# tiantianxuabc/ORB_SLAM2_Refactored

Hardware: AMD Instinct MI355X
Metric: frames/sec ORB extract+match (1280×720, 8 lvl, 1000 feat) + LocalBA iters/sec (higher is better)
Workload: dtype u8; 1 GPU; C2: 1280x720 mono, 8 levels, 2000 features, extract + brute-force Hamming top-2/ratio match of every frame vs its predecessor; width=1280, height=720, nlevels=8, nfeatures=2000, parallelism=8192-frame job sharded over 1 GPU(s), 8192 frames per GPU

## Files before the change

### include/orbslam2_amd.h

```cpp
#ifndef ORBSLAM2_AMD_H
#define ORBSLAM2_AMD_H

#include <stddef.h>
#include <stdint.h>

#ifdef __cplusplus
extern "C" {
#endif

#define ORB_OK          0
#define ORB_EINVAL     -1
#define ORB_EHIP       -2
#define ORB_ENOMEM     -3
#define ORB_ECAP       -4
#define ORB_EINTERNAL  -5


typedef struct orbx_params {
    int32_t nfeatures;
    float   scaleFactor;
    int32_t nlevels;
    int32_t iniThFAST;
    int32_t minThFAST;
} orbx_params;

typedef struct orbx_keypoint {
    float   x, y, size, angle, response;
    int32_t octave, class_id;
} orbx_keypoint;

typedef struct orbx_extractor orbx_extractor;

int orbx_create(const orbx_params* params, int device, orbx_extractor** out);
int orbx_destroy(orbx_extractor* h);

int orbx_scale_tables(const orbx_extractor* h, float* scale, float* inv_scale, float* sigma2,
                      float* inv_sigma2, int32_t* features_per_level);

int orbx_set_opencv_compat(orbx_extractor* h, int trig_mode, int resize_simd);
int orbx_get_opencv_compat(const orbx_extractor* h, int* trig_mode, int* resize_simd);

int orbx_max_keypoints(const orbx_extractor* h, int rows, int cols, int32_t* cap);

int orbx_extract(orbx_extractor* h, const uint8_t* img, int rows, int cols, size_t step,
                 orbx_keypoint* kps, uint8_t* desc, int cap, int* n);

int orbx_pyramid_level(const orbx_extractor* h, int level, uint8_t* dst, size_t dst_step,
                       int* rows, int* cols);

int orbx_extract_batch_device(orbx_extractor* h, const uint8_t* d_imgs, int n_frames, int rows,
                              int cols, size_t frame_stride, size_t step, orbx_keypoint* d_kps,
                              uint8_t* d_desc, int32_t* d_counts, int cap, void* stream);

int orbx_batch_status(orbx_extractor* h, void* stream, uint32_t* fault_mask);
int orbx_fault_word_device(orbx_extractor* h, uint32_t** d_fault);

int orbx_pyramid_device(const orbx_extractor* h, int frame, int level, const uint8_t** ptr,
                        int* rows, int* cols, size_t* step);


int orbm_descriptor_distance(const uint8_t* a, const uint8_t* b);

int orbm_hamming_top2_device(const uint8_t* d_A, int nA, const uint8_t* d_B, int nB,
                             int32_t* d_best_idx, int32_t* d_best, int32_t* d_second, void* stream);

int orbm_bf_match_batch_device(const uint8_t* d_A, const int32_t* d_nA, int strideA,
                               const uint8_t* d_B, const int32_t* d_nB, int strideB,
                               const int32_t* d_pair_b, int n_pairs, float nnratio, int th_low,
                               int32_t* d_best_idx, int32_t* d_best, int32_t* d_second,
                               int32_t* d_match, void* stream);

int orbm_bf_match(const uint8_t* A, int nA, const uint8_t* B, int nB, float nnratio, int th_low,
                  int32_t* best_idx, int32_t* best, int32_t* second, int32_t* match);

int orbm_check_orientation(const float* angleA, int nA, const float* angleB, int nB, int32_t* match,
                           int32_t* nmatches);

int orbm_check_orientation_batch_device(const float* d_angA, int kstrideA, int capA, const int32_t* d_nA,
                                        const float* d_angB, int kstrideB, int capB, const int32_t* d_pair_b,
                                        int n_pairs, int32_t* d_match, int strideM, int32_t* d_nmatches,
                                        void* stream);

typedef struct orbm_tri_frame {
    int32_t        n;
    const float*   kp_xy;
    const int32_t* octave;
    const float*   uright;
    const uint8_t* has_mappoint;
    const uint8_t* desc;
    int32_t        n_nodes;
    const uint32_t* node_id;
    const int32_t* node_off;
    const int32_t* indices;
} orbm_tri_frame;

int orbm_search_for_triangulation(const orbm_tri_frame* kf1, const orbm_tri_frame* kf2,
                                  const float* F12, const float* ep2, const float* scale2,
                                  const float* sigma2, int n_levels, int only_stereo,
                                  int32_t* match12, int32_t* nmatches);

#define ORBM_TRI_MAX_LEVELS 32
typedef struct orbm_tri_batch {
    int32_t n_pairs;
    int32_t cap1, cap2;
    const orbx_keypoint* kps1; const uint8_t* desc1; const int32_t* counts1;
    const float* uright1; const uint8_t* has_mappoint1;
    const orbx_keypoint* kps2; const uint8_t* desc2; const int32_t* counts2;
    const float* uright2; const uint8_t* has_mappoint2;
    const int32_t* frame1; const int32_t* frame2;
    const float* F12;
    const float* ep2;
    const uint32_t* fv_node1; const int32_t* fv_off1; const int32_t* fv_idx1; const int32_t* fv_n_nodes1;
    const uint32_t* fv_node2; const int32_t* fv_off2; const int32_t* fv_idx2; const int32_t* fv_n_nodes2;
    int32_t fv_cap1, fv_cap2;
    int32_t n_levels;
    const float* scale_factors2;
    const float* sigma2;
    int32_t only_stereo;
} orbm_tri_batch;

int orbm_search_for_triangulation_batch_device(const orbm_tri_batch* b, int32_t* d_match12, int32_t* d_nmatches,
                                               void* stream);

typedef struct orbm_bow_batch {
    int32_t n_pairs;
    int32_t cap1, cap2;
    const orbx_keypoint* kps1; const uint8_t* desc1; const uint8_t* mp_valid1;
    const int32_t* frame1;
    const orbx_keypoint* kps2; const uint8_t* desc2; const int32_t* counts2;
    const uint32_t* fv_node1; const int32_t* fv_off1; const int32_t* fv_idx1; const int32_t* fv_n_nodes1;
    const uint32_t* fv_node2; const int32_t* fv_off2; const int32_t* fv_idx2; const int32_t* fv_n_nodes2;
    int32_t fv_cap1, fv_cap2;
    float nnratio;
    int32_t check_orientation;
    const int32_t* counts1;
    const uint8_t* mp_valid2;
    const int32_t* frame2;
} orbm_bow_batch;

int orbm_search_by_bow_batch_device(const orbm_bow_batch* b, int32_t* d_match, int32_t* d_nmatches, void* stream);

int orbm_search_by_bow_kf_batch_device(const orbm_bow_batch* b, int32_t* d_match12, int32_t* d_nmatches,
                                       void* stream);

typedef struct orbm_stereo_view {
    int32_t n;
    const orbx_keypoint* kps;
    const uint8_t* desc;
    int32_t n_levels;
    const uint8_t* const* level;
    const int32_t* level_rows;
    const int32_t* level_cols;
    const int32_t* level_step;
} orbm_stereo_view;

int orbm_compute_stereo_matches(const orbm_stereo_view* left, const orbm_stereo_view* right,
                                const float* scale_factors, const float* inv_scale_factors, float bf,
                                float baseline, float* uright, float* depth);

int orbx_stereo_matches_batch_device(orbx_extractor* left, orbx_extractor* right, int n_frames,
                                     const orbx_keypoint* d_kps_l, const uint8_t* d_desc_l,
                                     const int32_t* d_counts_l, const orbx_keypoint* d_kps_r,
                                     const uint8_t* d_desc_r, const int32_t* d_counts_r, int cap,
                                     float bf, float baseline, float* d_uright, float* d_depth,
                                     void* stream);

int orbx_stereo_matches_last(orbx_extractor* left, orbx_extractor* right, float bf, float baseline, float* uright,
                             float* depth, int n_left);

#define ORBM_GRID_COLS 64
#define ORBM_GRID_ROWS 48
#define ORBM_PROJ_MAX_KP 8192

typedef struct orbm_proj_batch {
    int32_t        n_frames;
    int32_t        total_kp, total_mp;
    const int32_t* kp_begin;
    const float*   kp_xy;
    const int32_t* kp_octave;
    const float*   kp_uright;
    const uint8_t* kp_desc;
    const uint8_t* kp_claimed;
    const float*   bounds;
    const int32_t* mp_begin;
    const uint8_t* mp_valid;
    const float*   mp_proj;
    const float*   mp_view_cos;
    const int32_t* mp_level;
    const uint8_t* mp_desc;
    const uint8_t* mp_has_obs;
    int32_t        n_levels;
    const float*   scale_factors;
    float          th;
    float          nnratio;
} orbm_proj_batch;

int orbm_search_by_projection(const orbm_proj_batch* b, int32_t* kp_match, int32_t* n_matches, int device);
int orbm_search_by_projection_device(const orbm_proj_batch* b, int32_t* kp_match, int32_t* n_matches,
                                     void* stream);

typedef struct orbm_motion_batch {
    int32_t        n_frames, total_kp, total_mp;
    const int32_t* kp_begin;
    const float*   kp_xy;
    const int32_t* kp_octave;
    const float*   kp_uright;
    const uint8_t* kp_desc;
    const float*   kp_angle;
    const uint8_t* kp_claimed;
    const float*   bounds;
    const int32_t* mp_begin;
    const uint8_t* mp_valid;
    const float*   mp_proj;
    const int32_t* mp_octave;
    const uint8_t* mp_desc;
    const uint8_t* mp_has_obs;
    const float*   mp_angle;
    const int32_t* motion;
    int32_t        n_levels;
    const float*   scale_factors;
    float          th;
    int32_t        check_orientation;
} orbm_motion_batch;

int orbm_search_by_projection_motion_device(const orbm_motion_batch* b, int32_t* kp_match, int32_t* n_matches,
                                            void* stream);

typedef struct orbm_reloc_batch {
    int32_t        n_frames, total_kp, total_mp;
    const int32_t* kp_begin;
    const float*   kp_xy;
    const int32_t* kp_octave;
    const uint8_t* kp_desc;
    const float*   kp_angle;
    const uint8_t* kp_claimed;
    const float*   bounds;
    const float*   pose;
    const float*   camera;
    const int32_t* mp_begin;
    const uint8_t* mp_valid;
    const float*   mp_xw;
    const float*   mp_max_min;
    const uint8_t* mp_desc;
    const float*   mp_angle;
    int32_t        n_levels;
    const float*   scale_factors;
    float          log_scale_factor;
    float          th;
    int32_t        orb_dist;
    int32_t        check_orientation;
} orbm_reloc_batch;

int orbm_search_by_projection_reloc(const orbm_reloc_batch* b, int32_t* kp_match, int32_t* n_matches, int device);
int orbm_search_by_projection_reloc_device(const orbm_reloc_batch* b, int32_t* kp_match, int32_t* n_matches,
                                           void* stream);

typedef struct orbm_fuse_batch {
    int32_t        n_items, total_kp, total_mp;
    const int32_t* kp_begin;
    const float*   kp_xy;
    const int32_t* kp_octave;
    const float*   kp_uright;
    const uint8_t* kp_desc;
    const float*   bounds;
    const float*   pose;
    const float*   camera;
    const int32_t* mp_begin;
    const uint8_t* mp_valid;
    const float*   mp_xw;
    const float*   mp_max_min;
    const float*   mp_normal;
    const uint8_t* mp_desc;
    int32_t        n_levels;
    const float*   scale_factors;
    const float*   inv_sigma2;
    float          log_scale_factor;
    float          th;
    int32_t        chi2_gate;
} orbm_fuse_batch;

int orbm_fuse(const orbm_fuse_batch* b, int32_t* best_idx, int32_t* best_dist, int32_t* n_fused, int device);
int orbm_fuse_device(const orbm_fuse_batch* b, int32_t* best_idx, int32_t* best_dist, int32_t* n_fused, void* stream);

int orbm_search_by_projection_sim3(const orbm_fuse_batch* b, const uint8_t* kp_claimed, int32_t* kp_match,
                                   int32_t* n_matches, int device);
int orbm_search_by_projection_sim3_device(const orbm_fuse_batch* b, const uint8_t* kp_claimed, int32_t* kp_match,
                                          int32_t* n_matches, void* stream);

typedef struct orbm_sim3_batch {
    int32_t        n_pairs, total_kp1, total_kp2;
    const int32_t* kp1_begin;
    const int32_t* kp2_begin;
    const float*   kp1_xy;
    const int32_t* kp1_octave;
    const uint8_t* kp1_desc;
    const float*   kp2_xy;
    const int32_t* kp2_octave;
    const uint8_t* kp2_desc;
    const float*   bounds1;
    const float*   pose1;
    const float*   camera1;
    const float*   bounds2;
    const float*   pose2;
    const float*   camera2;
    const uint8_t* mp1_valid;
    const float*   mp1_xw;
    const float*   mp1_max_min;
    const uint8_t* mp1_desc;
    const uint8_t* mp2_valid;
    const float*   mp2_xw;
    const float*   mp2_max_min;
    const uint8_t* mp2_desc;
    const float*   s12;
    int32_t        n_levels;
    const float*   scale_factors;
    float          log_scale_factor;
    float          th;
} orbm_sim3_batch;

int orbm_search_by_sim3(const orbm_sim3_batch* b, int32_t* match12, int32_t* match1, int32_t* match2,
                        int32_t* n_found, int device);
int orbm_search_by_sim3_device(const orbm_sim3_batch* b, int32_t* match12, int32_t* match1, int32_t* match2,
                               int32_t* n_found, void* stream);

#define ORBM_DISTINCT_MAX_OBS 1024
int orbm_distinctive_descriptors(const uint8_t* desc , const int32_t* begin ,
                                 int32_t n_points, int32_t* best, int32_t* best_median ,
                                 uint8_t* out_desc , int device);
int orbm_distinctive_descriptors_device(const uint8_t* desc, const int32_t* begin, int32_t n_points, int32_t* best,
                                        int32_t* best_median, uint8_t* out_desc, void* stream);

typedef struct orbm_init_batch {
    int32_t        n_pairs, total_kp, total_q;
    const int32_t* kp_begin;
    const float*   kp_xy;
    const int32_t* kp_octave;
    const uint8_t* kp_desc;
    const float*   kp_angle;
    const float*   bounds;
    const int32_t* q_begin;
    const int32_t* q_octave;
    const uint8_t* q_desc;
    const float*   q_angle;
    float*         prev_matched;
    int32_t        window;
    float          nnratio;
    int32_t        check_orientation;
} orbm_init_batch;

int orbm_search_for_initialization(const orbm_init_batch* b, int32_t* matches12, int32_t* n_matches, int device);
int orbm_search_for_initialization_device(const orbm_init_batch* b, int32_t* matches12, int32_t* n_matches,
                                          void* stream);

typedef struct orbv_vocabulary orbv_vocabulary;
#define ORBV_MAX_FEATURES 4096

int orbv_load_text(const char* path, int device, orbv_vocabulary** out);
int orbv_create(int k, int L, int scoring, int weighting, int n_nodes, const int32_t* parent,
                const uint8_t* is_leaf, const uint8_t* desc, const double* weight, int device,
                orbv_vocabulary** out);
int orbv_destroy(orbv_vocabulary* v);
int orbv_info(const orbv_vocabulary* v, int* k, int* L, int* n_nodes, int* n_words, int* scoring,
              int* weighting);

int orbv_transform(orbv_vocabulary* v, const uint8_t* desc, int n, int levelsup, uint32_t* bow_word,
                   double* bow_weight, int* n_words, uint32_t* fv_node, int32_t* fv_off, int32_t* fv_idx,
                   int* n_nodes);
int orbv_transform_batch_device(orbv_vocabulary* v, const uint8_t* d_desc, const int32_t* d_counts, int cap,
                                int n_frames, int levelsup, uint32_t* d_bow_word, double* d_bow_weight,
                                int32_t* d_n_words, uint32_t* d_fv_node, int32_t* d_fv_off, int32_t* d_fv_idx,
                                int32_t* d_n_nodes, void* stream);

typedef struct orbba_problem {
    int32_t        n_poses;
    const double*  pose_R;
    const double*  pose_t;
    const uint8_t* pose_fixed;
    int32_t        n_points;
    const double*  points;
    int32_t        n_edges;
    const int32_t* edge_point;
    const int32_t* edge_pose;
    const double*  edge_obs;
    const double*  edge_inv_sigma2;
    const double*  edge_cam;
} orbba_problem;

typedef struct orbba_result {
    double*   pose_R;
    double*   pose_t;
    double*   pose_q;
    double*   points;
    uint8_t*  edge_outlier;
    double*   edge_chi2;
    int32_t   iterations[2];
    double    chi2[2];
    int32_t   ran;
} orbba_result;

#define ORBBA_MAX_FREE_KEYFRAMES 512

int orbba_local_ba(const orbba_problem* prob, orbba_result* res, const volatile int32_t* stop_flag,
                   int device);

#define ORBBA_POSE_MAX_EDGES 16384

typedef struct orbba_pose_batch {
    int32_t        n_frames;
    const int32_t* edge_begin;
    const double*  pose_R;
    const double*  pose_t;
    const double*  cam;
    const double*  xw;
    const double*  obs;
    const double*  inv_sigma2;
} orbba_pose_batch;

typedef struct orbba_pose_result {
    double*  pose_R;
    double*  pose_t;
    int32_t* n_inliers;
    uint8_t* outlier;
} orbba_pose_result;

int orbba_pose_optimization(const orbba_pose_batch* in, orbba_pose_result* out, int device);
int orbba_pose_optimization_device(const orbba_pose_batch* in, orbba_pose_result* out, void* stream);

#define ORBBA_SIM3_MAX_CORR ORBM_PROJ_MAX_KP

typedef struct orbba_sim3_batch {
    int32_t        n_pairs, total_kp1, total_kp2;
    const int32_t* kp1_begin;
    const int32_t* kp2_begin;
    const float*   kp1_xy;
    const int32_t* kp1_octave;
    const float*   kp2_xy;
    const int32_t* kp2_octave;
    const float*   pose1;
    const float*   camera1;
    const float*   pose2;
    const float*   camera2;
    const uint8_t* mp1_valid;
    const float*   mp1_xw;
    const uint8_t* mp2_valid;
    const float*   mp2_xw;
    const float*   s12;
    const int32_t* match12;
    int32_t        n_levels;
    const float*   inv_level_sigma2;
    float          max_chi2;
    int32_t        fix_scale;
} orbba_sim3_batch;

typedef struct orbba_sim3_result {
    float*   s12;
    double*  s12_g2o;
    int32_t* match12;
    int32_t* n_inliers;
    int32_t* iterations;
} orbba_sim3_result;

int orbba_optimize_sim3(const orbba_sim3_batch* in, orbba_sim3_result* out, int device);
int orbba_optimize_sim3_device(const orbba_sim3_batch* in, orbba_sim3_result* out, void* stream);

typedef struct orb_sim3solver_batch {
    int32_t        n_pairs, total_kp1, total_kp2;
    const int32_t* kp1_begin;
    const int32_t* kp2_begin;
    const float*   kp1_xy;
    const int32_t* kp1_octave;
    const float*   kp2_xy;
    const int32_t* kp2_octave;
    const float*   pose1;
    const float*   camera1;
    const float*   pose2;
    const float*   camera2;
    const uint8_t* mp1_valid;
    const float*   mp1_xw;
    const uint8_t* mp2_valid;
    const float*   mp2_xw;
    const float*   s12;
    const int32_t* match12;
    int32_t        n_levels;
    const float*   level_sigma2;
    int32_t        fix_scale;
    const int32_t* draws;
    int32_t        rand_max;
    double         probability;
    int32_t        min_inliers;
    int32_t        max_iterations;
    int32_t        maxk;
} orb_sim3solver_batch;

typedef struct orb_sim3solver_result {
    float*   s12;
    uint8_t* inlier;
    int32_t* match12;
    int32_t* found;
    int32_t* n_inliers;
    int32_t* iterations;
    int32_t* max_inliers;
    int32_t* terminate;
    int32_t* hyp_inliers;
} orb_sim3solver_result;

int orb_sim3solver_iterate(const orb_sim3solver_batch* in, orb_sim3solver_result* out, int device);
int orb_sim3solver_iterate_device(const orb_sim3solver_batch* in, orb_sim3solver_result* out, void* stream);

typedef struct orb_pnpsolver_batch {
    int32_t        n_frames, total_kp;
    const int32_t* kp_begin;
    const float*   kp_xy;
    const int32_t* kp_octave;
    const float*   camera;
    const uint8_t* mp_valid;
    const float*   mp_xw;
    int32_t        n_levels;
    const float*   level_sigma2;
    const int32_t* draws;
    int32_t        n_draws;
    int32_t        rand_max;
    double         probability;
    int32_t        min_inliers;
    int32_t        max_iterations;
    int32_t        min_set;
    float          epsilon;
    float          th2;
    int32_t        maxk;
} orb_pnpsolver_batch;

typedef struct orb_pnpsolver_result {
    float*   tcw;
    uint8_t* inlier;
    int32_t* found;
    int32_t* n_inliers;
    int32_t* terminate;
    int32_t* iterations;
    int32_t* best_inliers;
    uint8_t* best_mask;
    float*   best_tcw;
    int32_t* hyp_inliers;
} orb_pnpsolver_result;

int orb_pnpsolver_iterate(const orb_pnpsolver_batch* in, orb_pnpsolver_result* out, int device);
int orb_pnpsolver_iterate_device(const orb_pnpsolver_batch* in, orb_pnpsolver_result* out, void* stream);

typedef struct orb_initializer_batch {
    int32_t        n_pairs, total_kp1, total_kp2;
    const int32_t* kp1_begin;
    const int32_t* kp2_begin;
    const float*   kp1_xy;
    const float*   kp2_xy;
    const int32_t* matches12;
    const float*   camera;
    const int32_t* draws;
    int32_t        rand_max;
    float          sigma;
    int32_t        max_iterations;
    float          min_parallax;
    int32_t        min_triangulated;
    double         rh_threshold;
} orb_initializer_batch;

typedef struct orb_initializer_result {
    int32_t* found;
    int32_t* model;
    float*   r21t21;
    float*   p3d;
    uint8_t* triangulated;
    float*   score_h;
    float*   score_f;
    int32_t* best_h;
    int32_t* best_f;
    float*   h21;
    float*   f21;
    uint8_t* inlier_h;
    uint8_t* inlier_f;
    float*   hyp_score;
    int32_t* n_good;
    float*   parallax;
} orb_initializer_result;

int orb_initializer_initialize(const orb_initializer_batch* in, orb_initializer_result* out, int device);
int orb_initializer_initialize_device(const orb_initializer_batch* in, orb_initializer_result* out, void* stream);

const char* orb_last_error(void);
int orb_device_count(void);

int orbx_pack_descriptors(const uint8_t* desc, int32_t cap, const int32_t* counts, const int32_t* incl,
                          int32_t n_frames, uint8_t* out, int32_t out_rows, void* stream);

#define ORBX_NSTAGES 4
int orbx_profile_enable(orbx_extractor* h, int enable);
int orbx_profile_read(orbx_extractor* h, double* ms, int32_t* launches);

int orbx_debug_level_candidates(const orbx_extractor* h, int frame, int level, uint32_t* out, int cap, int* n);
int orbx_debug_qt_sort(const int32_t* sizes, int n, int32_t* perm);
int orbba_debug_po_wave(const double* in, double* scatter, double* sum);
int orbx_debug_level_selected(const orbx_extractor* h, int frame, int level, uint32_t* out, int cap, int* n);

#ifdef __cplusplus
}
#endif
#endif
```

### orb_slam2_refactored_amd/_lib.py

```python
import ctypes as C
import os
from pathlib import Path

import numpy as np

PKG = Path(__file__).resolve().parent
LIB_PATH = Path(os.environ.get("ORBSLAM2_AMD_LIB", PKG / "liborbslam2_amd.so"))


class OrbxParams(C.Structure):
    _fields_ = [("nfeatures", C.c_int32), ("scaleFactor", C.c_float), ("nlevels", C.c_int32),
                ("iniThFAST", C.c_int32), ("minThFAST", C.c_int32)]


class TriFrame(C.Structure):
    _fields_ = [("n", C.c_int32), ("kp_xy", C.c_void_p), ("octave", C.c_void_p), ("uright", C.c_void_p),
                ("has_mappoint", C.c_void_p), ("desc", C.c_void_p), ("n_nodes", C.c_int32),
                ("node_id", C.c_void_p), ("node_off", C.c_void_p), ("indices", C.c_void_p)]


class TriBatch(C.Structure):
    _fields_ = [("n_pairs", C.c_int32), ("cap1", C.c_int32), ("cap2", C.c_int32),
                ("kps1", C.c_void_p), ("desc1", C.c_void_p), ("counts1", C.c_void_p), ("uright1", C.c_void_p),
                ("has_mappoint1", C.c_void_p), ("kps2", C.c_void_p), ("desc2", C.c_void_p), ("counts2", C.c_void_p),
                ("uright2", C.c_void_p), ("has_mappoint2", C.c_void_p), ("frame1", C.c_void_p),
                ("frame2", C.c_void_p), ("F12", C.c_void_p), ("ep2", C.c_void_p),
                ("fv_node1", C.c_void_p), ("fv_off1", C.c_void_p), ("fv_idx1", C.c_void_p),
                ("fv_n_nodes1", C.c_void_p), ("fv_node2", C.c_void_p), ("fv_off2", C.c_void_p),
                ("fv_idx2", C.c_void_p), ("fv_n_nodes2", C.c_void_p), ("fv_cap1", C.c_int32),
                ("fv_cap2", C.c_int32), ("n_levels", C.c_int32), ("scale_factors2", C.c_void_p),
                ("sigma2", C.c_void_p), ("only_stereo", C.c_int32)]


class BowBatch(C.Structure):
    _fields_ = [("n_pairs", C.c_int32), ("cap1", C.c_int32), ("cap2", C.c_int32),
                ("kps1", C.c_void_p), ("desc1", C.c_void_p), ("mp_valid1", C.c_void_p), ("frame1", C.c_void_p),
                ("kps2", C.c_void_p), ("desc2", C.c_void_p), ("counts2", C.c_void_p),
                ("fv_node1", C.c_void_p), ("fv_off1", C.c_void_p), ("fv_idx1", C.c_void_p),
                ("fv_n_nodes1", C.c_void_p), ("fv_node2", C.c_void_p), ("fv_off2", C.c_void_p),
                ("fv_idx2", C.c_void_p), ("fv_n_nodes2", C.c_void_p), ("fv_cap1", C.c_int32),
                ("fv_cap2", C.c_int32), ("nnratio", C.c_float), ("check_orientation", C.c_int32),
                ("counts1", C.c_void_p), ("mp_valid2", C.c_void_p), ("frame2", C.c_void_p)]


class StereoView(C.Structure):
    _fields_ = [("n", C.c_int32), ("kps", C.c_void_p), ("desc", C.c_void_p), ("n_levels", C.c_int32),
                ("level", C.c_void_p), ("level_rows", C.c_void_p), ("level_cols", C.c_void_p),
                ("level_step", C.c_void_p)]


class BAProblem(C.Structure):
    _fields_ = [("n_poses", C.c_int32), ("pose_R", C.c_void_p), ("pose_t", C.c_void_p),
                ("pose_fixed", C.c_void_p), ("n_points", C.c_int32), ("points", C.c_void_p),
                ("n_edges", C.c_int32), ("edge_point", C.c_void_p), ("edge_pose", C.c_void_p),
                ("edge_obs", C.c_void_p), ("edge_inv_sigma2", C.c_void_p), ("edge_cam", C.c_void_p)]


class BAResult(C.Structure):
    _fields_ = [("pose_R", C.c_void_p), ("pose_t", C.c_void_p), ("pose_q", C.c_void_p),
                ("points", C.c_void_p), ("edge_outlier", C.c_void_p), ("edge_chi2", C.c_void_p),
                ("iterations", C.c_int32 * 2), ("chi2", C.c_double * 2), ("ran", C.c_int32)]


class ProjBatch(C.Structure):
    _fields_ = [("n_frames", C.c_int32), ("total_kp", C.c_int32), ("total_mp", C.c_int32),
                ("kp_begin", C.c_void_p), ("kp_xy", C.c_void_p), ("kp_octave", C.c_void_p), ("kp_uright", C.c_void_p),
                ("kp_desc", C.c_void_p), ("kp_claimed", C.c_void_p), ("bounds", C.c_void_p),
                ("mp_begin", C.c_void_p), ("mp_valid", C.c_void_p), ("mp_proj", C.c_void_p),
                ("mp_view_cos", C.c_void_p), ("mp_level", C.c_void_p), ("mp_desc", C.c_void_p),
                ("mp_has_obs", C.c_void_p), ("n_levels", C.c_int32), ("scale_factors", C.c_void_p),
                ("th", C.c_float), ("nnratio", C.c_float)]


class MotionBatch(C.Structure):
    _fields_ = [("n_frames", C.c_int32), ("total_kp", C.c_int32), ("total_mp", C.c_int32),
                ("kp_begin", C.c_void_p), ("kp_xy", C.c_void_p), ("kp_octave", C.c_void_p), ("kp_uright", C.c_void_p),
                ("kp_desc", C.c_void_p), ("kp_angle", C.c_void_p), ("kp_claimed", C.c_void_p), ("bounds", C.c_void_p),
                ("mp_begin", C.c_void_p), ("mp_valid", C.c_void_p), ("mp_proj", C.c_void_p), ("mp_octave", C.c_void_p),
                ("mp_desc", C.c_void_p), ("mp_has_obs", C.c_void_p), ("mp_angle", C.c_void_p), ("motion", C.c_void_p),
                ("n_levels", C.c_int32), ("scale_factors", C.c_void_p), ("th", C.c_float),
                ("check_orientation", C.c_int32)]


class RelocBatch(C.Structure):
    _fields_ = [("n_frames", C.c_int32), ("total_kp", C.c_int32), ("total_mp", C.c_int32),
                ("kp_begin", C.c_void_p), ("kp_xy", C.c_void_p), ("kp_octave", C.c_void_p), ("kp_desc", C.c_void_p),
                ("kp_angle", C.c_void_p), ("kp_claimed", C.c_void_p), ("bounds", C.c_void_p), ("pose", C.c_void_p),
                ("camera", C.c_void_p), ("mp_begin", C.c_void_p), ("mp_valid", C.c_void_p), ("mp_xw", C.c_void_p),
                ("mp_max_min", C.c_void_p), ("mp_desc", C.c_void_p), ("mp_angle", C.c_void_p), ("n_levels", C.c_int32),
                ("scale_factors", C.c_void_p), ("log_scale_factor", C.c_float), ("th", C.c_float),
                ("orb_dist", C.c_int32), ("check_orientation", C.c_int32)]


class FuseBatch(C.Structure):
    _fields_ = [("n_items", C.c_int32), ("total_kp", C.c_int32), ("total_mp", C.c_int32),
                ("kp_begin", C.c_void_p), ("kp_xy", C.c_void_p), ("kp_octave", C.c_void_p), ("kp_uright", C.c_void_p),
                ("kp_desc", C.c_void_p), ("bounds", C.c_void_p), ("pose", C.c_void_p), ("camera", C.c_void_p),
                ("mp_begin", C.c_void_p), ("mp_valid", C.c_void_p), ("mp_xw", C.c_void_p), ("mp_max_min", C.c_void_p),
                ("mp_normal", C.c_void_p), ("mp_desc", C.c_void_p), ("n_levels", C.c_int32),
                ("scale_factors", C.c_void_p), ("inv_sigma2", C.c_void_p), ("log_scale_factor", C.c_float),
                ("th", C.c_float), ("chi2_gate", C.c_int32)]


class Sim3Batch(C.Structure):
    _fields_ = [("n_pairs", C.c_int32), ("total_kp1", C.c_int32), ("total_kp2", C.c_int32),
                ("kp1_begin", C.c_void_p), ("kp2_begin", C.c_void_p),
                ("kp1_xy", C.c_void_p), ("kp1_octave", C.c_void_p), ("kp1_desc", C.c_void_p),
                ("kp2_xy", C.c_void_p), ("kp2_octave", C.c_void_p), ("kp2_desc", C.c_void_p),
                ("bounds1", C.c_void_p), ("pose1", C.c_void_p), ("camera1", C.c_void_p),
                ("bounds2", C.c_void_p), ("pose2", C.c_void_p), ("camera2", C.c_void_p),
                ("mp1_valid", C.c_void_p), ("mp1_xw", C.c_void_p), ("mp1_max_min", C.c_void_p), ("mp1_desc", C.c_void_p),
                ("mp2_valid", C.c_void_p), ("mp2_xw", C.c_void_p), ("mp2_max_min", C.c_void_p), ("mp2_desc", C.c_void_p),
                ("s12", C.c_void_p), ("n_levels", C.c_int32), ("scale_factors", C.c_void_p),
                ("log_scale_factor", C.c_float), ("th", C.c_float)]


class InitBatch(C.Structure):
    _fields_ = [("n_pairs", C.c_int32), ("total_kp", C.c_int32), ("total_q", C.c_int32),
                ("kp_begin", C.c_void_p), ("kp_xy", C.c_void_p), ("kp_octave", C.c_void_p), ("kp_desc", C.c_void_p),
                ("kp_angle", C.c_void_p), ("bounds", C.c_void_p), ("q_begin", C.c_void_p), ("q_octave", C.c_void_p),
                ("q_desc", C.c_void_p), ("q_angle", C.c_void_p), ("prev_matched", C.c_void_p), ("window", C.c_int32),
                ("nnratio", C.c_float), ("check_orientation", C.c_int32)]


class PoseBatch(C.Structure):
    _fields_ = [("n_frames", C.c_int32), ("edge_begin", C.c_void_p), ("pose_R", C.c_void_p), ("pose_t", C.c_void_p),
                ("cam", C.c_void_p), ("xw", C.c_void_p), ("obs", C.c_void_p), ("inv_sigma2", C.c_void_p)]


class PoseResult(C.Structure):
    _fields_ = [("pose_R", C.c_void_p), ("pose_t", C.c_void_p), ("n_inliers", C.c_void_p), ("outlier", C.c_void_p)]


class OptSim3Batch(C.Structure):
    _fields_ = [("n_pairs", C.c_int32), ("total_kp1", C.c_int32), ("total_kp2", C.c_int32),
                ("kp1_begin", C.c_void_p), ("kp2_begin", C.c_void_p),
                ("kp1_xy", C.c_void_p), ("kp1_octave", C.c_void_p), ("kp2_xy", C.c_void_p), ("kp2_octave", C.c_void_p),
                ("pose1", C.c_void_p), ("camera1", C.c_void_p), ("pose2", C.c_void_p), ("camera2", C.c_void_p),
                ("mp1_valid", C.c_void_p), ("mp1_xw", C.c_void_p), ("mp2_valid", C.c_void_p), ("mp2_xw", C.c_void_p),
                ("s12", C.c_void_p), ("match12", C.c_void_p), ("n_levels", C.c_int32),
                ("inv_level_sigma2", C.c_void_p), ("max_chi2", C.c_float), ("fix_scale", C.c_int32)]


class OptSim3Result(C.Structure):
    _fields_ = [("s12", C.c_void_p), ("s12_g2o", C.c_void_p), ("match12", C.c_void_p), ("n_inliers", C.c_void_p),
                ("iterations", C.c_void_p)]


class Sim3SolverBatch(C.Structure):
    _fields_ = [("n_pairs", C.c_int32), ("total_kp1", C.c_int32), ("total_kp2", C.c_int32),
                ("kp1_begin", C.c_void_p), ("kp2_begin", C.c_void_p),
                ("kp1_xy", C.c_void_p), ("kp1_octave", C.c_void_p), ("kp2_xy", C.c_void_p), ("kp2_octave", C.c_void_p),
                ("pose1", C.c_void_p), ("camera1", C.c_void_p), ("pose2", C.c_void_p), ("camera2", C.c_void_p),
                ("mp1_valid", C.c_void_p), ("mp1_xw", C.c_void_p), ("mp2_valid", C.c_void_p), ("mp2_xw", C.c_void_p),
                ("s12", C.c_void_p), ("match12", C.c_void_p), ("n_levels", C.c_int32),
                ("level_sigma2", C.c_void_p), ("fix_scale", C.c_int32), ("draws", C.c_void_p), ("rand_max", C.c_int32),
                ("probability", C.c_double), ("min_inliers", C.c_int32), ("max_iterations", C.c_int32),
                ("maxk", C.c_int32)]


class Sim3SolverResult(C.Structure):
    _fields_ = [("s12", C.c_void_p), ("inlier", C.c_void_p), ("match12", C.c_void_p), ("found", C.c_void_p),
                ("n_inliers", C.c_void_p), ("iterations", C.c_void_p), ("max_inliers", C.c_void_p),
                ("terminate", C.c_void_p), ("hyp_inliers", C.c_void_p)]


class PnPSolverBatch(C.Structure):
    _fields_ = [("n_frames", C.c_int32), ("total_kp", C.c_int32), ("kp_begin", C.c_void_p), ("kp_xy", C.c_void_p),
                ("kp_octave", C.c_void_p), ("camera", C.c_void_p), ("mp_valid", C.c_void_p), ("mp_xw", C.c_void_p),
                ("n_levels", C.c_int32), ("level_sigma2", C.c_void_p), ("draws", C.c_void_p), ("n_draws", C.c_int32),
                ("rand_max", C.c_int32), ("probability", C.c_double), ("min_inliers", C.c_int32),
                ("max_iterations", C.c_int32), ("min_set", C.c_int32), ("epsilon", C.c_float), ("th2", C.c_float),
                ("maxk", C.c_int32)]


class PnPSolverResult(C.Structure):
    _fields_ = [("tcw", C.c_void_p), ("inlier", C.c_void_p), ("found", C.c_void_p), ("n_inliers", C.c_void_p),
                ("terminate", C.c_void_p), ("iterations", C.c_void_p), ("best_inliers", C.c_void_p),
                ("best_mask", C.c_void_p), ("best_tcw", C.c_void_p), ("hyp_inliers", C.c_void_p)]


class InitializerBatch(C.Structure):
    _fields_ = [("n_pairs", C.c_int32), ("total_kp1", C.c_int32), ("total_kp2", C.c_int32),
                ("kp1_begin", C.c_void_p), ("kp2_begin", C.c_void_p), ("kp1_xy", C.c_void_p), ("kp2_xy", C.c_void_p),
                ("matches12", C.c_void_p), ("camera", C.c_void_p), ("draws", C.c_void_p), ("rand_max", C.c_int32),
                ("sigma", C.c_float), ("max_iterations", C.c_int32), ("min_parallax", C.c_float),
                ("min_triangulated", C.c_int32), ("rh_threshold", C.c_double)]


class InitializerResult(C.Structure):
    _fields_ = [("found", C.c_void_p), ("model", C.c_void_p), ("r21t21", C.c_void_p), ("p3d", C.c_void_p),
                ("triangulated", C.c_void_p), ("score_h", C.c_void_p), ("score_f", C.c_void_p), ("best_h", C.c_void_p),
                ("best_f", C.c_void_p), ("h21", C.c_void_p), ("f21", C.c_void_p), ("inlier_h", C.c_void_p),
                ("inlier_f", C.c_void_p), ("hyp_score", C.c_void_p), ("n_good", C.c_void_p), ("parallax", C.c_void_p)]


KP_DTYPE = np.dtype([("x", "<f4"), ("y", "<f4"), ("size", "<f4"), ("angle", "<f4"),
                     ("response", "<f4"), ("octave", "<i4"), ("class_id", "<i4")])

VP = C.c_void_p
I32 = C.c_int32
SZ = C.c_size_t

SIGNATURES = {
    "orbx_create": (C.c_int, [C.POINTER(OrbxParams), C.c_int, C.POINTER(VP)]),
    "orbx_destroy": (C.c_int, [VP]),
    "orbx_scale_tables": (C.c_int, [VP, VP, VP, VP, VP, VP]),
    "orbx_max_keypoints": (C.c_int, [VP, C.c_int, C.c_int, C.POINTER(I32)]),
    "orbx_set_opencv_compat": (C.c_int, [VP, C.c_int, C.c_int]),
    "orbx_get_opencv_compat": (C.c_int, [VP, C.POINTER(C.c_int), C.POINTER(C.c_int)]),
    "orbx_extract": (C.c_int, [VP, VP, C.c_int, C.c_int, SZ, VP, VP, C.c_int, C.POINTER(C.c_int)]),
    "orbx_pyramid_level": (C.c_int, [VP, C.c_int, VP, SZ, C.POINTER(C.c_int), C.POINTER(C.c_int)]),
    "orbx_extract_batch_device": (C.c_int, [VP, VP, C.c_int, C.c_int, C.c_int, SZ, SZ, VP, VP, VP, C.c_int, VP]),
    "orbx_batch_status": (C.c_int, [VP, VP, C.POINTER(C.c_uint32)]),
    "orbx_fault_word_device": (C.c_int, [VP, C.POINTER(VP)]),
    "orbx_pyramid_device": (C.c_int, [VP, C.c_int, C.c_int, C.POINTER(VP), C.POINTER(C.c_int),
                                      C.POINTER(C.c_int), C.POINTER(SZ)]),
    "orbm_descriptor_distance": (C.c_int, [VP, VP]),
    "orbm_hamming_top2_device": (C.c_int, [VP, C.c_int, VP, C.c_int, VP, VP, VP, VP]),
    "orbm_bf_match_batch_device": (C.c_int, [VP, VP, C.c_int, VP, VP, C.c_int, VP, C.c_int, C.c_float, C.c_int,
                                             VP, VP, VP, VP, VP]),
    "orbm_bf_match": (C.c_int, [VP, C.c_int, VP, C.c_int, C.c_float, C.c_int, VP, VP, VP, VP]),
    "orbm_check_orientation": (C.c_int, [VP, C.c_int, VP, C.c_int, VP, C.POINTER(I32)]),
    "orbm_check_orientation_batch_device": (C.c_int, [VP, C.c_int, C.c_int, VP, VP, C.c_int, C.c_int, VP, C.c_int,
                                                      VP, C.c_int, VP, VP]),
    "orbm_search_for_triangulation": (C.c_int, [C.POINTER(TriFrame), C.POINTER(TriFrame), VP, VP, VP, VP,
                                                C.c_int, C.c_int, VP, C.POINTER(I32)]),
    "orbm_search_for_triangulation_batch_device": (C.c_int, [C.POINTER(TriBatch), VP, VP, VP]),
    "orbm_search_by_bow_batch_device": (C.c_int, [C.POINTER(BowBatch), VP, VP, VP]),
    "orbm_search_by_bow_kf_batch_device": (C.c_int, [C.POINTER(BowBatch), VP, VP, VP]),
    "orbm_compute_stereo_matches": (C.c_int, [C.POINTER(StereoView), C.POINTER(StereoView), VP, VP, C.c_float,
                                              C.c_float, VP, VP]),
    "orbx_stereo_matches_batch_device": (C.c_int, [VP, VP, C.c_int, VP, VP, VP, VP, VP, VP, C.c_int, C.c_float,
                                                   C.c_float, VP, VP, VP]),
    "orbx_stereo_matches_last": (C.c_int, [VP, VP, C.c_float, C.c_float, VP, VP, C.c_int]),
    "orbm_search_by_projection": (C.c_int, [C.POINTER(ProjBatch), VP, VP, C.c_int]),
    "orbm_search_by_projection_device": (C.c_int, [C.POINTER(ProjBatch), VP, VP, VP]),
    "orbm_search_by_projection_motion_device": (C.c_int, [C.POINTER(MotionBatch), VP, VP, VP]),
    "orbm_search_for_initialization": (C.c_int, [C.POINTER(InitBatch), VP, VP, C.c_int]),
    "orbm_search_by_projection_reloc": (C.c_int, [C.POINTER(RelocBatch), VP, VP, C.c_int]),
    "orbm_search_by_projection_reloc_device": (C.c_int, [C.POINTER(RelocBatch), VP, VP, VP]),
    "orbm_search_for_initialization_device": (C.c_int, [C.POINTER(InitBatch), VP, VP, VP]),
    "orbm_fuse": (C.c_int, [C.POINTER(FuseBatch), VP, VP, VP, C.c_int]),
    "orbm_fuse_device": (C.c_int, [C.POINTER(FuseBatch), VP, VP, VP, VP]),
    "orbm_search_by_projection_sim3": (C.c_int, [C.POINTER(FuseBatch), VP, VP, VP, C.c_int]),
    "orbm_search_by_projection_sim3_device": (C.c_int, [C.POINTER(FuseBatch), VP, VP, VP, VP]),
    "orbm_search_by_sim3": (C.c_int, [C.POINTER(Sim3Batch), VP, VP, VP, VP, C.c_int]),
    "orbm_search_by_sim3_device": (C.c_int, [C.POINTER(Sim3Batch), VP, VP, VP, VP, VP]),
    "orbm_distinctive_descriptors": (C.c_int, [VP, VP, C.c_int32, VP, VP, VP, C.c_int]),
    "orbm_distinctive_descriptors_device": (C.c_int, [VP, VP, C.c_int32, VP, VP, VP, VP]),
    "orbv_load_text": (C.c_int, [C.c_char_p, C.c_int, C.POINTER(VP)]),
    "orbv_create": (C.c_int, [C.c_int, C.c_int, C.c_int, C.c_int, C.c_int, VP, VP, VP, VP, C.c_int, C.POINTER(VP)]),
    "orbv_destroy": (C.c_int, [VP]),
    "orbv_info": (C.c_int, [VP, C.POINTER(C.c_int), C.POINTER(C.c_int), C.POINTER(C.c_int), C.POINTER(C.c_int),
                            C.POINTER(C.c_int), C.POINTER(C.c_int)]),
    "orbv_transform": (C.c_int, [VP, VP, C.c_int, C.c_int, VP, VP, C.POINTER(C.c_int), VP, VP, VP,
                                 C.POINTER(C.c_int)]),
    "orbv_transform_batch_device": (C.c_int, [VP, VP, VP, C.c_int, C.c_int, C.c_int, VP, VP, VP, VP, VP, VP, VP, VP]),
    "orbba_local_ba": (C.c_int, [C.POINTER(BAProblem), C.POINTER(BAResult), VP, C.c_int]),
    "orbba_pose_optimization": (C.c_int, [C.POINTER(PoseBatch), C.POINTER(PoseResult), C.c_int]),
    "orbba_pose_optimization_device": (C.c_int, [C.POINTER(PoseBatch), C.POINTER(PoseResult), VP]),
    "orbba_optimize_sim3": (C.c_int, [C.POINTER(OptSim3Batch), C.POINTER(OptSim3Result), C.c_int]),
    "orbba_optimize_sim3_device": (C.c_int, [C.POINTER(OptSim3Batch), C.POINTER(OptSim3Result), VP]),
    "orb_sim3solver_iterate": (C.c_int, [C.POINTER(Sim3SolverBatch), C.POINTER(Sim3SolverResult), C.c_int]),
    "orb_sim3solver_iterate_device": (C.c_int, [C.POINTER(Sim3SolverBatch), C.POINTER(Sim3SolverResult), VP]),
    "orb_pnpsolver_iterate": (C.c_int, [C.POINTER(PnPSolverBatch), C.POINTER(PnPSolverResult), C.c_int]),
    "orb_pnpsolver_iterate_device": (C.c_int, [C.POINTER(PnPSolverBatch), C.POINTER(PnPSolverResult), VP]),
    "orb_initializer_initialize": (C.c_int, [C.POINTER(InitializerBatch), C.POINTER(InitializerResult), C.c_int]),
    "orb_initializer_initialize_device": (C.c_int, [C.POINTER(InitializerBatch), C.POINTER(InitializerResult), VP]),
    "orbx_pack_descriptors": (C.c_int,[VP, C.c_int, VP, VP, C.c_int, VP, C.c_int, VP]),
    "orbx_profile_enable": (C.c_int, [VP, C.c_int]),
    "orbx_profile_read": (C.c_int, [VP, VP, VP]),
    "orbx_debug_level_candidates": (C.c_int, [VP, C.c_int, C.c_int, VP, C.c_int, C.POINTER(C.c_int)]),
    "orbx_debug_qt_sort": (C.c_int, [VP, C.c_int, VP]),
    "orbba_debug_po_wave": (C.c_int, [VP, VP, VP]),
    "orbx_debug_level_selected": (C.c_int, [VP, C.c_int, C.c_int, VP, C.c_int, C.POINTER(C.c_int)]),
    "orb_last_error": (C.c_char_p, []),
    "orb_device_count": (C.c_int, []),
}

_lib = None


class OrbError(RuntimeError):
    pass


def lib():
    global _lib
    if _lib is None:
        if not LIB_PATH.exists():
            raise OrbError(f"{LIB_PATH} not found — build it with `python -c 'import __graft_entry__ as g; g.build()'`")
        l = C.CDLL(str(LIB_PATH))
        for name, (res, args) in SIGNATURES.items():
            if os.environ.get("ORBSLAM2_AMD_LIB") and not hasattr(l, name):
                continue
            fn = getattr(l, name)
            fn.restype = res
            fn.argtypes = args
        _lib = l
    return _lib


def check(rc: int, what: str = ""):
    if rc != 0:
        msg = lib().orb_last_error().decode(errors="replace")
        raise OrbError(f"{what} failed with status {rc}: {msg}")
    return rc


def ptr(a: np.ndarray):
    try:
        return VP(C.addressof(C.c_char.from_buffer(a)))
    except (TypeError, ValueError, BufferError):
        return VP(a.ctypes.data)


def tptr(t):
    return VP(t.data_ptr())


def stream_ptr(stream=None):
    import torch
    s = stream if stream is not None else torch.cuda.current_stream()
    return VP(s.cuda_stream)
```

### orb_slam2_refactored_amd/csrc/orbx.hip

```cpp
#include <algorithm>
#include <cfloat>
#include <cmath>
#include <cstring>
#include <mutex>
#include <type_traits>
#include <vector>

#include <hip/hip_ext.h>

#include "common.h"
#include "qt_sort.h"
#include "sincos_f.h"
#include "stereo.h"

#include "orbx_geom.h"
#include "orbx_pyramid.h"
#include "orbx_fast.h"
#include "orbx_quadtree.h"
#include "orbx_describe.h"

using namespace orbamd;

struct orbx_extractor {
    orbx_params p;
    int device = 0;
    hipStream_t stream = nullptr;
    std::vector<float> scale, inv_scale, sigma2, inv_sigma2;
    std::vector<int> quota;
    std::mutex mu;

    int g_rows = -1, g_cols = -1;
    Geom geom;
    std::vector<CellDev> cells;
    int NC = 0, PTC = 0;
    size_t qt_lds = 0;
    int qt_ptc0 = 0;
    size_t qt_lds0 = 0;
    int qt_wave = 0, qt_wave_wg = 2, qtw_l0 = 0, qtw_nc = 0, qtw_ptc = 0;
    size_t qtw_lds = 0;
    FastLds fl;
    size_t fast_lds = 0;
    int fast_cpw = 16;
    int fast_spec = 8;
    int fast_pair = 0;
    bool fast_pair_on = false;
    int fast_spec_first = 1;
    int nsub = 1;
    int debug_nc = 0;
    int debug_qt_block = 0;
    uint32_t fault_host = 0;
    int pyr_mfma = 0;
    std::vector<char> pyr_mfma_ok;
    std::vector<int> pyr_pair_np;
    DevBuf d_pyrmt, d_pyrkb;
    int pyr_pair = 2;
    int trig_float = 0;
    int resize_simd = 0;
    std::vector<std::pair<hipStream_t, hipEvent_t>> sub;
    hipEvent_t fork_ev = nullptr;
    bool lvl_overlap = false;
    hipStream_t lvl_side = nullptr;
    hipEvent_t lvl_fork = nullptr, lvl_join = nullptr;
    DevBuf d_cells, d_xtab, d_ytab;
    DevBuf d_strips;
    DevBuf d_slottab;
    DevBuf d_lvlpre;
    std::vector<int> strip_beg;

    int ws_frames = 0;
    DevBuf d_pyr, d_slots, d_cellcnt, d_P, d_T, d_sel, d_selcnt, d_fault;
    DevBuf d_img, d_kps, d_desc, d_counts;
    DevBuf d_stereo_sad;
    void release_buffers() {
        DevBuf* bufs[] = {&d_cells, &d_strips, &d_xtab, &d_ytab, &d_pyr, &d_slots, &d_cellcnt, &d_P,
                          &d_T, &d_sel, &d_selcnt, &d_fault, &d_img, &d_kps, &d_desc,
                          &d_counts, &d_stereo_sad, &d_pyrmt, &d_pyrkb, &d_slottab, &d_lvlpre,
                          &d_stereo_out, &d_dstat};
        for (DevBuf* b : bufs) b->release();
    }
    int prof = 0;
    std::vector<std::pair<hipEvent_t, hipEvent_t>> prof_ev[4];
    std::vector<hipEvent_t> ev_pool;
    const uint8_t* last_in = nullptr;
    long long last_fstride = 0;
    size_t last_step = 0;
    int last_frames = 0;
    int desc_dense = 0;
    int desc_force_c = 0;
    int desc_c = 0;
    DevBuf d_dstat;
    int32_t* h_dstat = nullptr;
    hipEvent_t dstat_ev = nullptr;
    bool dstat_pending = false;
    bool last_single = false;
    int last_kcap = 0;
    DevBuf d_stereo_out;
    std::vector<uint8_t> h_stage;
};

static int resize_tail_x(int w, int V) {
    if (V <= 0) return w;
    if (V == 1) return 0;
    int x = 0;
    for (; x <= w - V; x += V) {}
    for (; x < w - V / 2; x += V / 2) {}
    return x;
}

static int cv_round_d(double v) { return (int)std::lrint(v); }
static int cv_round_f(float v) { return (int)std::lrintf(v); }

static void compute_tables(orbx_extractor* h) {
    const orbx_params& p = h->p;
    const int L = p.nlevels;
    h->scale.resize(L); h->inv_scale.resize(L); h->sigma2.resize(L); h->inv_sigma2.resize(L);
    h->quota.resize(L);
    float s = 1.f;
    for (int l = 0; l < L; l++) {
        h->scale[l] = s;
        h->inv_scale[l] = 1.f / s;
        h->sigma2[l] = s * s;
        h->inv_sigma2[l] = 1.f / (s * s);
        s *= p.scaleFactor;
    }
    const double factor = 1 / p.scaleFactor;
    double nf = p.nfeatures * (1 - factor) / (1 - std::pow(factor, L));
    int sum = 0;
    for (int l = 0; l < L - 1; l++) {
        h->quota[l] = cv_round_d(nf);
        sum += h->quota[l];
        nf *= factor;
    }
    h->quota[L - 1] = std::max(p.nfeatures - sum, 0);
}

static int setup_geometry(orbx_extractor* h, int rows, int cols) {
    if (h->g_rows == rows && h->g_cols == cols) return ORB_OK;
    const int Lc = h->p.nlevels;
    Geom g;
    std::memset(&g, 0, sizeof(g));
    g.nlevels = Lc;
    for (int l = Lc; l < MAX_LEVELS; l++) g.lv[l].out_base = INT_MAX;
    std::vector<int2> xtab, ytab;
    std::vector<PyrMfmaLane> mt;
    std::vector<int> mkb;
    std::vector<CellDev> cells;
    long long pyr_off = 0, slot = 0, cand = 0;
    int out = 0, NC = 64;
    int prev_w = cols, prev_h = rows;
    for (int l = 0; l < Lc; l++) {
        LevelDev& L = g.lv[l];
        if (l == 0) {
            L.w = cols; L.h = rows; L.stride = cols; L.off = -1; L.tail_x = cols; L.mt_off = -1;
        } else {
            L.h = cv_round_f(h->inv_scale[l] * rows);
            L.w = cv_round_f(h->inv_scale[l] * cols);
            if (L.w <= 0 || L.h <= 0) {
                set_error("pyramid level collapses to zero size");
                return ORB_EINVAL;
            }
            L.stride = (int)align_up(L.w, 16);
            L.off = pyr_off;
            pyr_off += (long long)align_up((size_t)L.stride * L.h, 256);
            L.xtab_off = (int)xtab.size();
            L.ytab_off = (int)ytab.size();
            L.ssx = (double)prev_w / L.w;
            L.ssy = (double)prev_h / L.h;
            L.tail_x = resize_tail_x(L.w, h->resize_simd);
            pyr_resize_tables(prev_w, prev_h, L.w, L.h, xtab, ytab);
            L.mt_off = h->pyr_mfma ? pyr_mfma_tables(xtab.data() + L.xtab_off, L.w, mt, mkb) : -1;
        }
        if (l > 0) {
            const double sc = (double)prev_w / L.w, scy = (double)prev_h / L.h;
            if (sc * PYR_TW + 12 > PYR_SW || scy * PYR_TH + 6 > PYR_SH) {
                set_error("scaleFactor too large for the pyramid tile (max ~1.9)");
                return ORB_EINVAL;
            }
        }
        if (L.w >= 4096 || L.h >= 4096) {
            set_error("image dimensions must be < 4096");
            return ORB_EINVAL;
        }
        prev_w = L.w; prev_h = L.h;
        L.rx = 16; L.ry = 16; L.rw = L.w - 32; L.rh = L.h - 32;
        L.scale = h->scale[l];
        L.size = h->scale[l] * 31;
        L.quota = h->quota[l];
        L.cell_base = (int)cells.size();
        L.ncells = 0;
        L.cand_base = cand;
        L.cand_cap = 0;
        L.nroots = 0;
        L.out_base = out;
        L.out_cap = 0;
        if (L.rw > 0 && L.rh > 0) {
            const int gridw = L.rw / 30, gridh = L.rh / 30;
            if (gridw > 0 && gridh > 0) {
                const int cellw = (int)std::ceil(1. * L.rw / gridw), cellh = (int)std::ceil(1. * L.rh / gridh);
                const int maxx = L.rx + L.rw, maxy = L.ry + L.rh;
                for (int cy = 0, y0 = L.ry; cy < gridh && y0 + 6 < maxy; cy++, y0 += cellh)
                    for (int cx = 0, x0 = L.rx; cx < gridw && x0 + 6 < maxx; cx++, x0 += cellw) {
                        const int y1 = std::min(y0 + cellh + 6, maxy), x1 = std::min(x0 + cellw + 6, maxx);
                        const int zw = x1 - x0 - 6, zh = y1 - y0 - 6;
                        if (zw > MAX_ZONE || zh > MAX_ZONE) {
                            set_error("FAST cell larger than supported zone");
                            return ORB_EINVAL;
                        }
                        CellDev c;
                        c.level = l;
                        c.x0y0 = x0 | (y0 << 16);
                        c.zwzh = zw | (zh << 16);
                        c.slot = (int)slot;
                        const int cap = ((zw + 1) / 2) * ((zh + 1) / 2);
                        slot += cap;
                        L.cand_cap += cap;
                        cells.push_back(c);
                        L.ncells++;
                    }
                L.nroots = cv_round_d(1. * L.rw / L.rh);
                if (L.nroots <= 0 || L.nroots > MAX_ROOTS) {
                    set_error("unsupported aspect ratio (quadtree root count)");
                    return ORB_EINVAL;
                }
                L.hx = 1. * L.rw / L.nroots;
                L.out_cap = std::max(L.quota + 3, 4 * L.nroots) + 1;
                NC = std::max(NC, L.out_cap + 8);
            }
        }
        cand += L.cand_cap;
        out += L.out_cap;
    }
    g.ncells_total = (int)cells.size();
    g.pyr_frame_bytes = std::max<long long>(pyr_off, 256);
    g.slot_frame = std::max<long long>(slot, 1);
    g.cand_frame = std::max<long long>(cand, 1);
    g.out_frame = std::max(out, 1);
    if (g.out_frame >= 0x7fff) {
        set_error("ORBextractor: more than 32766 selection slots per frame (nfeatures too large)");
        return ORB_EINVAL;
    }
    for (int d = 0; d < MAX_LEVELS / 2; d++) g.lv_start[d] = 0x7fff7fffu;
    for (int l = 1; l < Lc; l++)
        g.lv_start[l >> 1] = (g.lv_start[l >> 1] & ~(0xffffu << (16 * (l & 1)))) | ((unsigned)g.lv[l].out_base << (16 * (l & 1)));
    {
        const unsigned d = (unsigned)g.out_frame;
        int lg = 0;
        while ((1ull << lg) < d) lg++;
        g.of_m = (unsigned)((((1ull << lg) - d) << 32) / d + 1);
        g.of_s1 = lg > 0 ? 1 : 0;
        g.of_s2 = lg > 0 ? lg - 1 : 0;
    }
    NC = (int)align_up(std::max(NC, 256), 64);
    if (h->debug_nc > 0) NC = (int)align_up(std::max(h->debug_nc, 256), 64);
    const size_t node_lds = (size_t)NC * (2 * sizeof(QtNode) + sizeof(int4) + 2 * sizeof(QtItem) + 2 * sizeof(int));
    int PTC = 2048;
    {
        hipFuncAttributes fa{};
        const size_t stat = hipFuncGetAttributes(&fa, (const void*)quadtree_kernel<false>) == hipSuccess ? fa.sharedSizeBytes : 1024;
        for (int t = QT_WAVES_DEF; t >= 2; t--) {
            const long long room = (long long)(160 * 1024 / t) - (long long)stat - (long long)node_lds;
            const int p = (int)std::min<long long>(2048, room / 8) & ~63;
            if (p >= 512) { PTC = p; break; }
        }
    }
    if (const char* e = getenv("ORBX_QT_PTC")) PTC = std::max(256, std::min(4096, atoi(e)));
    const size_t lds = node_lds + (size_t)PTC * 8;
    if (lds > 156 * 1024) {
        set_error("nfeatures too large for the quadtree LDS budget (per-level quota <= ~2100)");
        return ORB_EINVAL;
    }
    int PTC0 = 0;
    size_t lds0 = 0;
    if (const char* e = getenv("ORBX_QT_PTC0")) {
        PTC0 = std::max(256, std::min(8192, atoi(e))) & ~63;
        lds0 = node_lds + (size_t)PTC0 * 8;
        if (lds0 > 156 * 1024) { PTC0 = 0; lds0 = 0; }
    }
    if (std::max(lds, lds0) > 48 * 1024)
        ORB_HIP_TRY(hipFuncSetAttribute((const void*)quadtree_kernel<false>, hipFuncAttributeMaxDynamicSharedMemorySize,
                                        (int)std::max(lds, lds0)));
    h->qtw_l0 = g.nlevels;
    if (h->qt_wave) {
        int l0w = g.nlevels;
        while (l0w > 0 && g.lv[l0w - 1].ncells <= 4 * 64 && g.lv[l0w - 1].nroots <= 4) l0w--;
        int ncw = 64;
        for (int l = l0w; l < g.nlevels; l++) ncw = std::max(ncw, g.lv[l].out_cap + 8);
        ncw = (int)align_up(ncw, 64);
        hipFuncAttributes fa{};
        const size_t stat = hipFuncGetAttributes(&fa, (const void*)quadtree_kernel<true>) == hipSuccess ? fa.sharedSizeBytes : 2048;
        const long long per_wave = ((long long)(160 * 1024 / std::max(1, h->qt_wave_wg)) - (long long)stat) / 4;
        const int ptcw = (int)std::min<long long>(2048, (per_wave - (long long)ncw * QT_NODE_BYTES) / 8) & ~63;
        if (l0w < g.nlevels && ptcw >= 64) {
            h->qtw_l0 = l0w;
            h->qtw_nc = ncw;
            h->qtw_ptc = ptcw;
            h->qtw_lds = 4 * ((size_t)ncw * QT_NODE_BYTES + (size_t)ptcw * 8);
            if (h->qtw_lds > 48 * 1024)
                ORB_HIP_TRY(hipFuncSetAttribute((const void*)quadtree_kernel<true>, hipFuncAttributeMaxDynamicSharedMemorySize,
                                                (int)h->qtw_lds));
        }
    }
    int rc;
    if ((rc = h->d_cells.reserve(std::max<size_t>(1, cells.size()) * sizeof(CellDev)))) return rc;
    if ((rc = h->d_xtab.reserve(std::max<size_t>(1, xtab.size()) * sizeof(int2)))) return rc;
    if ((rc = h->d_ytab.reserve(std::max<size_t>(1, ytab.size()) * sizeof(int2)))) return rc;
    if (!cells.empty())
        ORB_HIP_TRY(hipMemcpy(h->d_cells.ptr, cells.data(), cells.size() * sizeof(CellDev), hipMemcpyHostToDevice));
    if (!xtab.empty())
        ORB_HIP_TRY(hipMemcpy(h->d_xtab.ptr, xtab.data(), xtab.size() * sizeof(int2), hipMemcpyHostToDevice));
    if (!ytab.empty())
        ORB_HIP_TRY(hipMemcpy(h->d_ytab.ptr, ytab.data(), ytab.size() * sizeof(int2), hipMemcpyHostToDevice));
    {
        std::vector<uint32_t> st((size_t)g.out_frame, 0u);
        for (int l = 0; l < Lc; l++)
            for (int i = 0; i < g.lv[l].out_cap; i++) st[(size_t)g.lv[l].out_base + i] = (uint32_t)l | ((uint32_t)i << 8);
        if ((rc = h->d_slottab.reserve(st.size() * sizeof(uint32_t)))) return rc;
        ORB_HIP_TRY(hipMemcpy(h->d_slottab.ptr, st.data(), st.size() * sizeof(uint32_t), hipMemcpyHostToDevice));
    }
    if (!mt.empty() && (rc = h->d_pyrmt.reserve(mt.size() * sizeof(PyrMfmaLane)))) return rc;
    if (!mkb.empty() && (rc = h->d_pyrkb.reserve(mkb.size() * sizeof(int)))) return rc;
    if (!mt.empty())
        ORB_HIP_TRY(hipMemcpy(h->d_pyrmt.ptr, mt.data(), mt.size() * sizeof(PyrMfmaLane), hipMemcpyHostToDevice));
    if (!mkb.empty())
        ORB_HIP_TRY(hipMemcpy(h->d_pyrkb.ptr, mkb.data(), mkb.size() * sizeof(int), hipMemcpyHostToDevice));
    h->pyr_mfma_ok.assign(Lc, 0);
    for (int l = 1; l + 1 < Lc; l++) h->pyr_mfma_ok[l] = h->pyr_mfma && pyr_mfma_pair_fits(g, l, mkb, ytab);
    h->pyr_pair_np.assign(Lc, 0);
    for (int l = 1; l + 1 < Lc; l++) h->pyr_pair_np[l] = pyr_pair_fits(g, l, xtab, ytab);
    h->geom = g;
    h->cells = cells;
    {
        std::vector<int2> strips;
        h->strip_beg.assign(g.nlevels + 1, 0);
        const int cpw = std::max(1, std::min(h->fast_cpw, 255));
        for (int l = 0; l < g.nlevels; l++) {
            h->strip_beg[l] = (int)strips.size();
            const LevelDev& L = g.lv[l];
            if (L.ncells <= 0) continue;
            const int x00 = cells[L.cell_base].x0y0 & 0xffff;
            int ncx = 0;
            while (ncx < L.ncells && (cells[L.cell_base + ncx].x0y0 >> 16) == (cells[L.cell_base].x0y0 >> 16)) ncx++;
            const int ncy = L.ncells / ncx;
            if (ncx * ncy != L.ncells || (cells[L.cell_base + ncx - 1].x0y0 & 0xffff) < x00) {
                set_error("FAST cell grid is not a rectangle");
                return ORB_EINTERNAL;
            }
            for (int rb = 0; rb < ncy; rb += cpw)
                for (int cx = 0; cx < ncx; cx++) {
                    const int c0 = L.cell_base + rb * ncx + cx, n = std::min(cpw, ncy - rb);
                    for (int k = 1; k < n; k++)
                        if ((cells[c0 + k * ncx].zwzh & 0xffff) != (cells[c0].zwzh & 0xffff)) {
                            set_error("FAST strip with unequal zone widths");
                            return ORB_EINTERNAL;
                        }
                    strips.push_back(make_int2(c0, n | (ncx << 8)));
                }
        }
        h->strip_beg[g.nlevels] = (int)strips.size();
        if ((rc = h->d_strips.reserve(std::max<size_t>(1, strips.size()) * sizeof(int2)))) return rc;
        if (!strips.empty())
            ORB_HIP_TRY(hipMemcpy(h->d_strips.ptr, strips.data(), strips.size() * sizeof(int2), hipMemcpyHostToDevice));
    }
    {
        int mzw = 1, mzh = 1;
        for (const CellDev& c : cells) { mzw = std::max(mzw, c.zwzh & 0xffff); mzh = std::max(mzh, c.zwzh >> 16); }
        if (mzw > 64 || mzh > (2 * GR_RING + FQ2_RING) / 8) {
            set_error("FAST cell larger than the kernel supports");
            return ORB_EINTERNAL;
        }
        h->fast_pair_on = false;
        if (h->fast_pair) {
            bool ok = 2 * mzh < 128 && 24 * ((2 * mzh + 1) / (mzw <= 32 ? 2 : 1) + 1) <= 2 * (2 * GR_RING + FQ2_RING);
            for (int l = 0; l < g.nlevels && ok; l++) {
                const LevelDev& L = g.lv[l];
                if (L.ncells <= 0) continue;
                int ncx = 0;
                while (ncx < L.ncells && (cells[L.cell_base + ncx].x0y0 >> 16) == (cells[L.cell_base].x0y0 >> 16)) ncx++;
                for (int c = L.cell_base; c + ncx < L.cell_base + L.ncells && ok; c++) {
                    const CellDev &A = cells[c], &B = cells[c + ncx];
                    ok = (A.x0y0 & 0xffff) == (B.x0y0 & 0xffff) && (B.x0y0 >> 16) == (A.x0y0 >> 16) + (A.zwzh >> 16);
                }
            }
            h->fast_pair_on = ok;
        }
        const int zrows = h->fast_pair_on ? 2 * mzh + 1 : mzh;
        FastLds fl;
        fl.CS = (int)align_up(mzw + 6 + 8, 4);
        if (fl.CS < 4 * ((mzw + 6 + 1 + 3) / 4)) fl.CS = 4 * ((mzw + 6 + 1 + 3) / 4);
        fl.ZS = (int)align_up(mzw + 2, 4);
        fl.crop_bytes = (int)align_up((size_t)fl.CS * std::max(zrows + 6 + FAST_CROP_SLACK, 4 * CROP_NG), 16);
        fl.mz_bytes = (int)align_up((size_t)fl.ZS * (zrows + 2), 16);
        fl.qcap = 2 * GR_RING + FQ2_RING;
        fl.ccap = std::min(FAST_CLIST_CAP, (int)align_up((size_t)mzw * mzh, 8));
        const int nbal = (fl.ccap + 63) / 64;
        h->fast_lds = (size_t)fl.crop_bytes + fl.mz_bytes + 2 * (size_t)(fl.qcap + fl.ccap) +
                      (h->fast_pair_on ? 24 : 16) * (size_t)nbal;
        h->fl = fl;
    }
    h->NC = NC;
    h->PTC = PTC;
    h->qt_lds = lds;
    h->qt_ptc0 = PTC0;
    h->qt_lds0 = lds0;
    h->g_rows = rows;
    h->g_cols = cols;
    h->ws_frames = 0;
    return ORB_OK;
}

static int max_keypoints(const Geom& g) {
    int c = 0;
    for (int l = 0; l < g.nlevels; l++) c += g.lv[l].out_cap;
    return c;
}

static int reserve_workspace(orbx_extractor* h, int frames) {
    if (frames <= h->ws_frames) return ORB_OK;
    const Geom& g = h->geom;
    int rc;
    if ((rc = h->d_pyr.reserve((size_t)frames * g.pyr_frame_bytes))) return rc;
    if ((rc = h->d_slots.reserve((size_t)frames * g.slot_frame * 4))) return rc;
    if ((rc = h->d_cellcnt.reserve((size_t)frames * std::max(1, g.ncells_total) * 4))) return rc;
    if ((rc = h->d_P.reserve((size_t)frames * g.cand_frame * 4))) return rc;
    if ((rc = h->d_T.reserve((size_t)frames * g.cand_frame * 4))) return rc;
    if ((rc = h->d_sel.reserve((size_t)frames * g.out_frame * 4))) return rc;
    if ((rc = h->d_selcnt.reserve((size_t)frames * g.nlevels * 4 + 64))) return rc;
    if ((rc = h->d_lvlpre.reserve((size_t)frames * LVP * 4))) return rc;
    if (!h->d_fault.ptr) {
        if ((rc = h->d_fault.reserve(16))) return rc;
        ORB_HIP_TRY(hipMemset(h->d_fault.ptr, 0, 16));
    }
    h->ws_frames = frames;
    return ORB_OK;
}

static hipEvent_t prof_event(orbx_extractor* h) {
    if (!h->ev_pool.empty()) {
        hipEvent_t e = h->ev_pool.back();
        h->ev_pool.pop_back();
        return e;
    }
    hipEvent_t e = nullptr;
    (void)hipEventCreate(&e);
    return e;
}

constexpr int ORBX_MIN_SUB_FRAMES = 16;

template <typename... KArgs, typename... Args>
static void launch_timed(orbx_extractor* h, int stage, void (*kernel)(KArgs...), dim3 grid, dim3 block,
                         uint32_t shmem, hipStream_t s, Args... args) {
    if (h->prof & (1 << stage)) {
        hipEvent_t a = prof_event(h), b = prof_event(h);
        hipExtLaunchKernelGGL(kernel, grid, block, shmem, s, a, b, 0, static_cast<KArgs>(args)...);
        h->prof_ev[stage].push_back({a, b});
    } else {
        hipLaunchKernelGGL(kernel, grid, block, shmem, s, static_cast<KArgs>(args)...);
    }
}

static auto fast_kernel_for(const FastLds& fl, bool pair) -> decltype(&fast_cells_kernel<0, 0, false>) {
    if (pair)
        return fl.CS == 48 && fl.ZS == 36   ? fast_cells_kernel<48, 36, true>
               : fl.CS == 52 && fl.ZS == 40 ? fast_cells_kernel<52, 40, true>
                                            : fast_cells_kernel<0, 0, true>;
    return fl.CS == 48 && fl.ZS == 36   ? fast_cells_kernel<48, 36, false>
           : fl.CS == 52 && fl.ZS == 40 ? fast_cells_kernel<52, 40, false>
                                        : fast_cells_kernel<0, 0, false>;
}

static void launch_chunk(orbx_extractor* h, int f0, const uint8_t* d_imgs, int F, long long fstride, int step,
                         orbx_keypoint* d_kps, uint8_t* d_desc, int32_t* d_counts, int cap, hipStream_t st,
                         hipStream_t side = nullptr) {
    const Geom& g = h->geom;
    uint8_t* pyr = h->d_pyr.as<uint8_t>() + (long long)f0 * g.pyr_frame_bytes;
    d_imgs += (long long)f0 * fstride;
    d_kps += (long long)f0 * cap;
    d_desc += (long long)f0 * cap * 32;
    d_counts += f0;
    uint32_t* slots = h->d_slots.as<uint32_t>() + (long long)f0 * g.slot_frame;
    int* cellcnt = h->d_cellcnt.as<int>() + (long long)f0 * g.ncells_total;
    uint32_t* Pb = h->d_P.as<uint32_t>() + (long long)f0 * g.cand_frame;
    uint32_t* Tb = h->d_T.as<uint32_t>() + (long long)f0 * g.cand_frame;
    uint32_t* sel = h->d_sel.as<uint32_t>() + (long long)f0 * g.out_frame;
    int* selcnt = h->d_selcnt.as<int>() + (long long)f0 * g.nlevels;
    uint32_t* fault = h->d_fault.as<uint32_t>();
    auto fast = [&](int l0, int l1, hipStream_t s) {
        const int sb = h->strip_beg[l0], ns = h->strip_beg[l1] - sb;
        if (ns <= 0) return;
        launch_timed(h, 1, fast_kernel_for(h->fl, h->fast_pair_on), dim3((unsigned)(ns * F)), dim3(64), (uint32_t)h->fast_lds, s,
                           g, h->d_cells.as<CellDev>(), h->d_strips.as<int2>(), d_imgs, fstride, step, pyr, h->p.iniThFAST,
                           h->p.minThFAST, slots, cellcnt, fault, h->fl, sb, ns,
                           h->fast_spec > 0 && h->fast_spec_first ? h->fast_spec | (1 << 29) : h->fast_spec);
    };
    const unsigned qt_block = h->debug_qt_block ? (unsigned)h->debug_qt_block : (unsigned)QT_THREADS;
    auto quadtree = [&](int l0, int nl, hipStream_t s) {
        if (nl <= 0) return;
        const int lw = std::max(l0, h->qtw_l0), nw_lv = l0 + nl - lw;
        if (nw_lv > 0) {
            launch_timed(h, 2, quadtree_kernel<true>, dim3((unsigned)F, (unsigned)((nw_lv + 3) / 4)), dim3(qt_block),
                         (uint32_t)h->qtw_lds, s, g, cellcnt, slots, h->d_cells.as<CellDev>(), Pb, Tb, sel, selcnt, h->qtw_nc,
                         h->qtw_ptc, fault, lw, nw_lv);
            nl -= nw_lv;
            if (nl <= 0) return;
        }
        if (h->qt_ptc0 > 0 && l0 == 0) {
            launch_timed(h, 2, quadtree_kernel<false>, dim3((unsigned)F, 1u), dim3(qt_block), (uint32_t)h->qt_lds0, s, g,
                         cellcnt, slots, h->d_cells.as<CellDev>(), Pb, Tb, sel, selcnt, h->NC, h->qt_ptc0, fault, 0, 1);
            l0 = 1;
            if (--nl <= 0) return;
        }
        launch_timed(h, 2, quadtree_kernel<false>, dim3((unsigned)F, (unsigned)nl), dim3(qt_block), (uint32_t)h->qt_lds, s,
                     g, cellcnt, slots, h->d_cells.as<CellDev>(), Pb, Tb, sel, selcnt, h->NC, h->PTC, fault, l0, nl);
    };
    auto pyramid = [&](int l) -> int {
        const int first = h->pyr_pair == 2 ? 1 : 2;
        const bool a16 = l > 1 || (((uintptr_t)d_imgs | (uintptr_t)fstride | (uintptr_t)step) & 15) == 0;
        const bool pair = h->pyr_pair && l >= first && (l - first) % 2 == 0 && l + 1 < g.nlevels && a16;
        auto tiles = [&](int lt) {
            return dim3((unsigned)((g.lv[lt].w + PYR_TW - 1) / PYR_TW), (unsigned)((g.lv[lt].h + PYR_TH - 1) / PYR_TH),
                        (unsigned)F);
        };
        if (pair && h->pyr_mfma && h->pyr_mfma_ok[l]) {
            launch_timed(h, 0, pyramid_pair_mfma_kernel, tiles(l + 1), dim3(256), 0u, st, g, l, d_imgs, fstride, step, pyr,
                         h->d_ytab.as<int2>(), h->d_pyrmt.as<PyrMfmaLane>(), h->d_pyrkb.as<int>());
            return 1;
        }
        if (pair && h->pyr_pair_np[l]) {
            launch_timed(h, 0, h->pyr_pair_np[l] <= 7 ? pyramid_pair_kernel<7> : pyramid_pair_kernel<PP_MAXP>, tiles(l + 1),
                         dim3(256), 0u, st, g, l, d_imgs, fstride, step, pyr, h->d_xtab.as<int2>(), h->d_ytab.as<int2>());
            return 1;
        }
        launch_timed(h, 0, pyramid_level_kernel, tiles(l), dim3(256), 0u, st, g, l, d_imgs, fstride, step, pyr,
                     h->d_xtab.as<int2>(), h->d_ytab.as<int2>());
        return 0;
    };
    const int nc0 = g.lv[0].ncells;
    if (side && nc0 > 0 && g.nlevels > 1) {
        (void)hipStreamWaitEvent(side, h->lvl_fork, 0);
        fast(0, 1, side);
        quadtree(0, 1, side);
        (void)hipEventRecord(h->lvl_join, side);
        {
            for (int l = 1; l < g.nlevels; l++) l += pyramid(l);
        }
        fast(1, g.nlevels, st);
        quadtree(1, g.nlevels - 1, st);
        (void)hipStreamWaitEvent(st, h->lvl_join, 0);
    } else {
        {
            for (int l = 1; l < g.nlevels; l++) l += pyramid(l);
        }
        fast(0, g.nlevels, st);
        quadtree(0, g.nlevels, st);
    }
    int* lvlpre = h->d_lvlpre.as<int>() + (long long)f0 * LVP;
    hipLaunchKernelGGL(describe_prefix_kernel, dim3((unsigned)((F + 255) / 256)), dim3(256), 0, st, (const int*)selcnt,
                       g.nlevels, F, lvlpre, d_counts, h->d_dstat.as<int>());
    const int rows_max = std::min(g.out_frame, cap);
    const int C = h->desc_dense ? std::max(1, std::min(h->desc_c > 0 ? h->desc_c : rows_max, rows_max)) : 0;
    DescGrid dg{};
    if (C > 0) {
        dg.C = C;
        const unsigned d = (unsigned)C;
        int lg = 0;
        while ((1ull << lg) < d) lg++;
        dg.m = (unsigned)((((1ull << lg) - d) << 32) / d + 1);
        dg.s1 = lg > 0 ? 1 : 0;
        dg.s2 = lg > 0 ? lg - 1 : 0;
    }
    launch_timed(h, 3, h->trig_float ? describe_kernel<1> : describe_kernel<0>,
                 dim3((unsigned)(C > 0 ? C : g.out_frame), (unsigned)F), dim3(64), 0u, st, g, d_imgs, fstride, step, pyr,
                 sel, selcnt, d_kps, d_desc, d_counts, cap, h->d_slottab.as<uint32_t>(), lvlpre, dg);
    if (C > 0 && C < rows_max)
        launch_timed(h, 3, h->trig_float ? describe_overflow_kernel<1> : describe_overflow_kernel<0>,
                     dim3((unsigned)std::min(F, 2048)), dim3(64), 0u, st, g, d_imgs, fstride, step, pyr, sel, d_kps, d_desc,
                     cap, (const int*)lvlpre, F, C);
}

static int launch_fast_hint(orbx_extractor* h, hipStream_t st) {
    if (!(h->fast_spec > 0 && h->fast_spec_first)) return ORB_OK;
    const int ns = h->strip_beg[h->geom.nlevels];
    if (ns <= 0) return ORB_OK;
    hipLaunchKernelGGL(fast_hint_kernel, dim3((unsigned)((ns + 255) / 256)), dim3(256), 0, st, h->d_strips.as<int2>(),
                       h->d_cellcnt.as<int>(), ns);
    ORB_HIP_TRY(hipGetLastError());
    return ORB_OK;
}

static int describe_grid_begin(orbx_extractor* h, hipStream_t st) {
    if (!h->dstat_ev) {
        ORB_HIP_TRY(hipEventCreateWithFlags(&h->dstat_ev, hipEventDisableTiming));
        ORB_HIP_TRY(hipHostMalloc((void**)&h->h_dstat, 64, hipHostMallocDefault));
        int rc;
        if ((rc = h->d_dstat.reserve(64))) return rc;
    }
    if (h->dstat_pending && hipEventQuery(h->dstat_ev) == hipSuccess) {
        const int mx = *h->h_dstat;
        h->desc_c = (int)align_up((size_t)std::max(mx + 32, 64), 64);
        h->dstat_pending = false;
    }
    if (h->desc_force_c > 0) h->desc_c = h->desc_force_c;
    ORB_HIP_TRY(hipMemsetAsync(h->d_dstat.ptr, 0, 4, st));
    return ORB_OK;
}
static int describe_grid_end(orbx_extractor* h, hipStream_t st) {
    if (h->dstat_pending) return ORB_OK;
    ORB_HIP_TRY(hipMemcpyAsync(h->h_dstat, h->d_dstat.ptr, 4, hipMemcpyDeviceToHost, st));
    ORB_HIP_TRY(hipEventRecord(h->dstat_ev, st));
    h->dstat_pending = true;
    return ORB_OK;
}

static int launch_batch(orbx_extractor* h, const uint8_t* d_imgs, int F, long long fstride, int step,
                        orbx_keypoint* d_kps, uint8_t* d_desc, int32_t* d_counts, int cap, hipStream_t st) {
    {
        const int rc = describe_grid_begin(h, st);
        if (rc) return rc;
    }
    int nsub = std::min(h->nsub, F / ORBX_MIN_SUB_FRAMES);
    if (nsub <= 1) {
        hipStream_t side = nullptr;
        if (h->lvl_overlap) {
            if (!h->lvl_side) {
                ORB_HIP_TRY(hipStreamCreateWithFlags(&h->lvl_side, hipStreamNonBlocking));
                ORB_HIP_TRY(hipEventCreateWithFlags(&h->lvl_fork, hipEventDisableTiming));
                ORB_HIP_TRY(hipEventCreateWithFlags(&h->lvl_join, hipEventDisableTiming));
            }
            ORB_HIP_TRY(hipEventRecord(h->lvl_fork, st));
            side = h->lvl_side;
        }
        launch_chunk(h, 0, d_imgs, F, fstride, step, d_kps, d_desc, d_counts, cap, st, side);
    } else {
        while ((int)h->sub.size() < nsub) {
            hipStream_t s2;
            ORB_HIP_TRY(hipStreamCreateWithFlags(&s2, hipStreamNonBlocking));
            hipEvent_t e;
            ORB_HIP_TRY(hipEventCreateWithFlags(&e, hipEventDisableTiming));
            h->sub.push_back({s2, e});
        }
        if (!h->fork_ev) ORB_HIP_TRY(hipEventCreateWithFlags(&h->fork_ev, hipEventDisableTiming));
        ORB_HIP_TRY(hipEventRecord(h->fork_ev, st));
        int f0 = 0;
        for (int i = 0; i < nsub; i++) {
            const int Fi = F / nsub + (i < F % nsub ? 1 : 0);
            ORB_HIP_TRY(hipStreamWaitEvent(h->sub[i].first, h->fork_ev, 0));
            launch_chunk(h, f0, d_imgs, Fi, fstride, step, d_kps, d_desc, d_counts, cap, h->sub[i].first);
            ORB_HIP_TRY(hipEventRecord(h->sub[i].second, h->sub[i].first));
            ORB_HIP_TRY(hipStreamWaitEvent(st, h->sub[i].second, 0));
            f0 += Fi;
        }
    }
    ORB_HIP_TRY(hipGetLastError());
    const int rc = describe_grid_end(h, st);
    return rc ? rc : launch_fast_hint(h, st);
}

static int check_fault(orbx_extractor* h) {
    uint32_t f = 0;
    ORB_HIP_TRY(hipMemcpy(&f, h->d_fault.ptr, 4, hipMemcpyDeviceToHost));
    if (f) {
        ORB_HIP_TRY(hipMemset(h->d_fault.ptr, 0, 4));
        set_error("device capacity check failed (fault mask " + std::to_string(f) + ")");
        return ORB_EINTERNAL;
    }
    return ORB_OK;
}

namespace orbamd {
__global__ __launch_bounds__(256) void pack_rows_kernel(const uint4* __restrict__ desc, int cap,
                                                        const int* __restrict__ counts, const int* __restrict__ incl,
                                                        uint4* __restrict__ out, int out_rows) {
    const int f = blockIdx.x;
    const int c = counts[f];
    const int n = min(max(c, 0), cap);
    const long long start = (long long)incl[f] - c;
    const long long r0 = max(start, 0ll), r1 = min(start + n, (long long)out_rows);
    const uint4* src = desc + (long long)f * cap * 2;
    for (long long i = 2 * r0 + threadIdx.x; i < 2 * r1; i += blockDim.x) out[i] = src[i - 2 * start];
}

}

extern "C" {

int orbx_create(const orbx_params* params, int device, orbx_extractor** out) {
    ORB_CHECK_ARG(params && out, "null argument");
    ORB_CHECK_ARG(params->nlevels >= 1 && params->nlevels <= MAX_LEVELS, "nlevels must be in [1,16]");
    ORB_CHECK_ARG(params->nfeatures >= 0 && params->scaleFactor > 1.0f, "bad nfeatures / scaleFactor");
    int ndev = 0;
    ORB_HIP_TRY(hipGetDeviceCount(&ndev));
    ORB_CHECK_ARG(device >= 0 && device < ndev, "no such HIP device");
    ORB_HIP_TRY(hipSetDevice(device));
    orbx_extractor* h = new orbx_extractor();
    h->p = *params;
    h->device = device;
    if (const char* e = getenv("ORBX_FAST_CPW")) h->fast_cpw = std::max(1, std::min(64, atoi(e)));
    if (const char* e = getenv("ORBX_FAST_SPEC")) h->fast_spec = std::max(-1, atoi(e));
    if (const char* e = getenv("ORBX_FAST_PAIR")) h->fast_pair = atoi(e) != 0;
    if (const char* e = getenv("ORBX_QT_WAVE")) h->qt_wave = atoi(e) != 0;
    if (const char* e = getenv("ORBX_QT_WAVE_WG")) h->qt_wave_wg = std::max(1, std::min(4, atoi(e)));
    if (const char* e = getenv("ORBX_FAST_SPEC_FIRST")) h->fast_spec_first = atoi(e) != 0;

    if (const char* e = getenv("ORBX_NSUB")) h->nsub = std::max(1, std::min(8, atoi(e)));
    if (const char* e = getenv("ORBX_PYR_PAIR")) h->pyr_pair = std::max(0, std::min(2, atoi(e)));
    if (const char* e = getenv("ORBX_PYR_MFMA")) h->pyr_mfma = atoi(e) != 0;
    if (const char* e = getenv("ORBX_LEVEL_OVERLAP")) h->lvl_overlap = atoi(e) != 0;
    if (const char* e = getenv("ORBX_DEBUG_NC")) h->debug_nc = atoi(e);
    if (const char* e = getenv("ORBX_DESC_DENSE")) h->desc_dense = atoi(e) != 0;
    if (const char* e = getenv("ORBX_DESC_C")) h->desc_force_c = std::max(0, atoi(e));
    if (const char* e = getenv("ORBX_DEBUG_QT_BLOCK")) {
        const int b = atoi(e);
        if (b >= 64 && b <= QT_THREADS && b % 64 == 0) h->debug_qt_block = b;
    }
    if (const char* e = getenv("ORBX_TRIG")) h->trig_float = (e[0] == 'f' || e[0] == '1') ? 1 : 0;
    if (const char* e = getenv("ORBX_RESIZE_TAIL")) {
        const int v = atoi(e);
        if (v == 0 || v == 1 || v == 8 || v == 16 || v == 32 || v == 64) h->resize_simd = v;
    }
    compute_tables(h);
    hipError_t e = hipStreamCreateWithFlags(&h->stream, hipStreamNonBlocking);
    if (e != hipSuccess) {
        delete h;
        set_error(std::string("hipStreamCreate: ") + hipGetErrorString(e));
        return ORB_EHIP;
    }
    *out = h;
    return ORB_OK;
}

int orbx_destroy(orbx_extractor* h) {
    if (!h) return ORB_OK;
    (void)hipSetDevice(h->device);
    h->release_buffers();
    for (auto& v : h->prof_ev)
        for (auto& pr : v) { (void)hipEventDestroy(pr.first); (void)hipEventDestroy(pr.second); }
    for (hipEvent_t e : h->ev_pool) (void)hipEventDestroy(e);
    if (h->stream) (void)hipStreamDestroy(h->stream);
    for (auto& se : h->sub) { (void)hipStreamDestroy(se.first); (void)hipEventDestroy(se.second); }
    if (h->fork_ev) (void)hipEventDestroy(h->fork_ev);
    if (h->lvl_side) (void)hipStreamDestroy(h->lvl_side);
    if (h->lvl_fork) (void)hipEventDestroy(h->lvl_fork);
    if (h->lvl_join) (void)hipEventDestroy(h->lvl_join);
    if (h->dstat_ev) (void)hipEventDestroy(h->dstat_ev);
    if (h->h_dstat) (void)hipHostFree(h->h_dstat);
    delete h;
    return ORB_OK;
}

int orbx_set_opencv_compat(orbx_extractor* h, int trig_mode, int resize_simd) {
    ORB_CHECK_ARG(h, "null extractor");
    ORB_CHECK_ARG(trig_mode >= -1 && trig_mode <= 1, "trig_mode must be -1 (keep), 0 (double) or 1 (float)");
    ORB_CHECK_ARG(resize_simd == -1 || resize_simd == 0 || resize_simd == 1 || resize_simd == 8 || resize_simd == 16 ||
                      resize_simd == 32 || resize_simd == 64,
                  "resize_simd must be -1 (keep), 0, 1, 8, 16, 32 or 64");
    std::lock_guard<std::mutex> lk(h->mu);
    if (trig_mode >= 0) h->trig_float = trig_mode;
    if (resize_simd >= 0 && resize_simd != h->resize_simd) {
        h->resize_simd = resize_simd;
        h->g_rows = h->g_cols = -1;
    }
    return ORB_OK;
}

int orbx_get_opencv_compat(const orbx_extractor* h, int* trig_mode, int* resize_simd) {
    ORB_CHECK_ARG(h, "null extractor");
    if (trig_mode) *trig_mode = h->trig_float;
    if (resize_simd) *resize_simd = h->resize_simd;
    return ORB_OK;
}

int orbx_scale_tables(const orbx_extractor* h, float* scale, float* inv_scale, float* sigma2, float* inv_sigma2,
                      int32_t* features_per_level) {
    ORB_CHECK_ARG(h, "null extractor");
    for (int l = 0; l < h->p.nlevels; l++) {
        if (scale) scale[l] = h->scale[l];
        if (inv_scale) inv_scale[l] = h->inv_scale[l];
        if (sigma2) sigma2[l] = h->sigma2[l];
        if (inv_sigma2) inv_sigma2[l] = h->inv_sigma2[l];
        if (features_per_level) features_per_level[l] = h->quota[l];
    }
    return ORB_OK;
}

int orbx_max_keypoints(const orbx_extractor* hc, int rows, int cols, int32_t* cap) {
    ORB_CHECK_ARG(hc && cap && rows > 0 && cols > 0, "bad argument");
    orbx_extractor* h = const_cast<orbx_extractor*>(hc);
    std::lock_guard<std::mutex> lk(h->mu);
    ORB_HIP_TRY(hipSetDevice(h->device));
    int rc = setup_geometry(h, rows, cols);
    if (rc) return rc;
    *cap = max_keypoints(h->geom);
    return ORB_OK;
}

int orbx_extract_batch_device(orbx_extractor* h, const uint8_t* d_imgs, int n_frames, int rows, int cols,
                              size_t frame_stride, size_t step, orbx_keypoint* d_kps, uint8_t* d_desc,
                              int32_t* d_counts, int cap, void* stream) {
    ORB_CHECK_ARG(h && d_imgs && d_kps && d_desc && d_counts, "null argument");
    ORB_CHECK_ARG(n_frames > 0 && n_frames <= 65535 && rows > 0 && cols > 0, "bad batch shape");
    ORB_CHECK_ARG(step >= (size_t)cols && step < (1u << 31), "bad row step");
    std::lock_guard<std::mutex> lk(h->mu);
    ORB_HIP_TRY(hipSetDevice(h->device));
    int rc = setup_geometry(h, rows, cols);
    if (rc) return rc;
    if (cap < max_keypoints(h->geom)) {
        set_error("cap < orbx_max_keypoints()");
        return ORB_ECAP;
    }
    if ((rc = reserve_workspace(h, n_frames))) return rc;
    hipStream_t st = (hipStream_t)stream;
    h->last_in = d_imgs;
    h->last_single = false;
    h->last_fstride = (long long)frame_stride;
    h->last_step = step;
    h->last_frames = n_frames;
    return launch_batch(h, d_imgs, n_frames, (long long)frame_stride, (int)step, d_kps, d_desc, d_counts, cap, st);
}

int orbx_extract(orbx_extractor* h, const uint8_t* img, int rows, int cols, size_t step, orbx_keypoint* kps,
                 uint8_t* desc, int cap, int* n) {
    ORB_CHECK_ARG(h && img && n, "null argument");
    ORB_CHECK_ARG(rows > 0 && cols > 0 && step >= (size_t)cols, "image must be a non-empty CV_8U matrix");
    std::lock_guard<std::mutex> lk(h->mu);
    ORB_HIP_TRY(hipSetDevice(h->device));
    int rc = setup_geometry(h, rows, cols);
    if (rc) return rc;
    const int kcap = max_keypoints(h->geom);
    if ((rc = reserve_workspace(h, 1))) return rc;
    if ((rc = h->d_img.reserve((size_t)rows * cols))) return rc;
    if ((rc = h->d_kps.reserve((size_t)kcap * sizeof(orbx_keypoint)))) return rc;
    if ((rc = h->d_desc.reserve((size_t)kcap * 32))) return rc;
    if ((rc = h->d_counts.reserve(16))) return rc;
    hipStream_t st = h->stream;
    if (step == (size_t)cols)
        ORB_HIP_TRY(hipMemcpyAsync(h->d_img.ptr, img, (size_t)rows * cols, hipMemcpyHostToDevice, st));
    else
        ORB_HIP_TRY(hipMemcpy2DAsync(h->d_img.ptr, cols, img, step, cols, rows, hipMemcpyHostToDevice, st));
    h->last_in = h->d_img.as<uint8_t>();
    h->last_fstride = (long long)rows * cols;
    h->last_step = cols;
    h->last_frames = 1;
    h->last_single = true;
    h->last_kcap = kcap;
    rc = launch_batch(h, h->d_img.as<uint8_t>(), 1, (long long)rows * cols, cols, h->d_kps.as<orbx_keypoint>(),
                      h->d_desc.as<uint8_t>(), h->d_counts.as<int32_t>(), kcap, st);
    if (rc) return rc;
    int32_t total = 0;
    ORB_HIP_TRY(hipMemcpyAsync(&total, h->d_counts.ptr, 4, hipMemcpyDeviceToHost, st));
    ORB_HIP_TRY(hipStreamSynchronize(st));
    if ((rc = check_fault(h))) return rc;
    *n = total;
    if (total == 0) return ORB_OK;
    if (total > cap) {
        set_error("output capacity too small");
        return ORB_ECAP;
    }
    ORB_CHECK_ARG(kps && desc, "null output");
    ORB_HIP_TRY(hipMemcpyAsync(kps, h->d_kps.ptr, (size_t)total * sizeof(orbx_keypoint), hipMemcpyDeviceToHost, st));
    ORB_HIP_TRY(hipMemcpyAsync(desc, h->d_desc.ptr, (size_t)total * 32, hipMemcpyDeviceToHost, st));
    ORB_HIP_TRY(hipStreamSynchronize(st));
    return ORB_OK;
}

int orbx_batch_status(orbx_extractor* h, void* stream, uint32_t* fault_mask) {
    ORB_CHECK_ARG(h && fault_mask, "null argument");
    std::lock_guard<std::mutex> lk(h->mu);
    ORB_HIP_TRY(hipSetDevice(h->device));
    *fault_mask = 0;
    if (!h->d_fault.ptr) return ORB_OK;
    hipStream_t st = (hipStream_t)stream;
    ORB_HIP_TRY(hipMemcpyAsync(&h->fault_host, h->d_fault.ptr, 4, hipMemcpyDeviceToHost, st));
    ORB_HIP_TRY(hipMemsetAsync(h->d_fault.ptr, 0, 4, st));
    ORB_HIP_TRY(hipStreamSynchronize(st));
    *fault_mask = h->fault_host;
    if (h->fault_host) {
        set_error("device capacity check failed in a batch (fault mask " + std::to_string(h->fault_host) + ")");
        return ORB_EINTERNAL;
    }
    return ORB_OK;
}

int orbx_fault_word_device(orbx_extractor* h, uint32_t** d_fault) {
    ORB_CHECK_ARG(h && d_fault, "null argument");
    std::lock_guard<std::mutex> lk(h->mu);
    ORB_HIP_TRY(hipSetDevice(h->device));
    int rc;
    if (!h->d_fault.ptr) {
        if ((rc = h->d_fault.reserve(16))) return rc;
        ORB_HIP_TRY(hipMemset(h->d_fault.ptr, 0, 16));
    }
    *d_fault = h->d_fault.as<uint32_t>();
    return ORB_OK;
}

int orbx_pyramid_device(const orbx_extractor* h, int frame, int level, const uint8_t** ptr, int* rows, int* cols,
                        size_t* step) {
    ORB_CHECK_ARG(h && ptr && h->last_in, "no extraction has run");
    ORB_CHECK_ARG(frame >= 0 && frame < h->last_frames && level >= 0 && level < h->geom.nlevels, "bad index");
    const LevelDev& L = h->geom.lv[level];
    if (level == 0) {
        *ptr = h->last_in + (long long)frame * h->last_fstride;
        if (step) *step = h->last_step;
    } else {
        *ptr = h->d_pyr.as<uint8_t>() + (long long)frame * h->geom.pyr_frame_bytes + L.off;
        if (step) *step = (size_t)L.stride;
    }
    if (rows) *rows = L.h;
    if (cols) *cols = L.w;
    return ORB_OK;
}

int orbx_pyramid_level(const orbx_extractor* h, int level, uint8_t* dst, size_t dst_step, int* rows, int* cols) {
    const uint8_t* p = nullptr;
    int r = 0, c = 0;
    size_t st = 0;
    int rc = orbx_pyramid_device(h, 0, level, &p, &r, &c, &st);
    if (rc) return rc;
    if (rows) *rows = r;
    if (cols) *cols = c;
    if (!dst) return ORB_OK;
    ORB_CHECK_ARG(dst_step >= (size_t)c, "dst_step too small");
    ORB_HIP_TRY(hipSetDevice(h->device));
    ORB_HIP_TRY(hipStreamSynchronize(h->stream));
    if (dst_step == st) {
        ORB_HIP_TRY(hipMemcpy(dst, p, (size_t)(r - 1) * st + c, hipMemcpyDeviceToHost));
    } else {
        std::vector<uint8_t>& tmp = const_cast<orbx_extractor*>(h)->h_stage;
        tmp.resize((size_t)(r - 1) * st + c);
        ORB_HIP_TRY(hipMemcpy(tmp.data(), p, tmp.size(), hipMemcpyDeviceToHost));
        for (int y = 0; y < r; y++) std::memcpy(dst + (size_t)y * dst_step, tmp.data() + (size_t)y * st, (size_t)c);
    }
    return ORB_OK;
}

int orbx_debug_level_candidates(const orbx_extractor* h, int frame, int level, uint32_t* out, int cap, int* n) {
    ORB_CHECK_ARG(h && n && h->last_frames > 0, "no extraction has run");
    ORB_CHECK_ARG(frame >= 0 && frame < h->last_frames && level >= 0 && level < h->geom.nlevels, "bad index");
    ORB_HIP_TRY(hipSetDevice(h->device));
    ORB_HIP_TRY(hipDeviceSynchronize());
    const Geom& g = h->geom;
    const LevelDev& L = g.lv[level];
    std::vector<int> cnt(std::max(1, L.ncells));
    if (L.ncells)
        ORB_HIP_TRY(hipMemcpy(cnt.data(), h->d_cellcnt.as<int>() + (long long)frame * g.ncells_total + L.cell_base,
                              4 * (size_t)L.ncells, hipMemcpyDeviceToHost));
    std::vector<uint32_t> slots((size_t)g.slot_frame);
    ORB_HIP_TRY(hipMemcpy(slots.data(), h->d_slots.as<uint32_t>() + (long long)frame * g.slot_frame,
                          4 * (size_t)g.slot_frame, hipMemcpyDeviceToHost));
    int m = 0;
    for (int c = 0; c < L.ncells; c++) {
        const CellDev& cd = h->cells[L.cell_base + c];
        for (int j = 0; j < (cnt[c] & CELL_CNT_MASK); j++) {
            if (out && m < cap) out[m] = slots[cd.slot + j];
            m++;
        }
    }
    *n = m;
    return ORB_OK;
}

int orbx_debug_level_selected(const orbx_extractor* h, int frame, int level, uint32_t* out, int cap, int* n) {
    ORB_CHECK_ARG(h && n && h->last_frames > 0, "no extraction has run");
    ORB_CHECK_ARG(frame >= 0 && frame < h->last_frames && level >= 0 && level < h->geom.nlevels, "bad index");
    ORB_HIP_TRY(hipSetDevice(h->device));
    ORB_HIP_TRY(hipDeviceSynchronize());
    const Geom& g = h->geom;
    int c = 0;
    ORB_HIP_TRY(hipMemcpy(&c, h->d_selcnt.as<int>() + frame * g.nlevels + level, 4, hipMemcpyDeviceToHost));
    *n = c;
    if (out && c > 0)
        ORB_HIP_TRY(hipMemcpy(out, h->d_sel.as<uint32_t>() + (long long)frame * g.out_frame + g.lv[level].out_base,
                              4 * (size_t)std::min(c, cap), hipMemcpyDeviceToHost));
    return ORB_OK;
}

int orbx_profile_enable(orbx_extractor* h, int enable) {
    ORB_CHECK_ARG(h, "null extractor");
    std::lock_guard<std::mutex> lk(h->mu);
    h->prof = enable > 0 ? 0xf : (-enable) & 0xf;

    return ORB_OK;
}

int orbx_pack_descriptors(const uint8_t* desc, int32_t cap, const int32_t* counts, const int32_t* incl,
                          int32_t n_frames, uint8_t* out, int32_t out_rows, void* stream) {
    ORB_CHECK_ARG(n_frames >= 0 && cap >= 0 && out_rows >= 0, "negative sizes");
    if (n_frames == 0 || out_rows == 0) return ORB_OK;
    ORB_CHECK_ARG(desc && counts && incl && out, "null argument");
    ORB_CHECK_ARG(((reinterpret_cast<uintptr_t>(desc) | reinterpret_cast<uintptr_t>(out)) & 15) == 0,
                  "desc / out must be 16-byte aligned");
    hipLaunchKernelGGL(orbamd::pack_rows_kernel, dim3((unsigned)n_frames), dim3(256), 0, (hipStream_t)stream,
                       reinterpret_cast<const uint4*>(desc), (int)cap, counts, incl, reinterpret_cast<uint4*>(out),
                       (int)out_rows);
    ORB_HIP_TRY(hipGetLastError());
    return ORB_OK;
}

int orbx_profile_read(orbx_extractor* h, double* ms, int32_t* launches) {
    ORB_CHECK_ARG(h, "null extractor");
    std::lock_guard<std::mutex> lk(h->mu);
    ORB_HIP_TRY(hipSetDevice(h->device));
    for (int k = 0; k < 4; k++) {
        double tot = 0;
        for (auto& pr : h->prof_ev[k]) {
            ORB_HIP_TRY(hipEventSynchronize(pr.second));
            float t = 0;
            ORB_HIP_TRY(hipEventElapsedTime(&t, pr.first, pr.second));
            tot += t;
            h->ev_pool.push_back(pr.first);
            h->ev_pool.push_back(pr.second);
        }
        if (ms) ms[k] = tot;
        if (launches) launches[k] = (int32_t)h->prof_ev[k].size();
        h->prof_ev[k].clear();
    }
    return ORB_OK;
}

int orbx_debug_qt_sort(const int32_t* sizes, int n, int32_t* perm) {
    ORB_CHECK_ARG(n >= 0 && (n == 0 || (sizes && perm)), "bad argument");
    if (n == 0) return ORB_OK;
    std::vector<QtItem> h(n);
    for (int i = 0; i < n; i++) h[i] = QtItem{sizes[i], i};
    DevBuf d;
    int rc;
    if ((rc = d.reserve((size_t)n * sizeof(QtItem) + ((size_t)n * 8 + 16) * sizeof(int) + 64))) return rc;
    QtItem* items = d.as<QtItem>();
    int* scratch = reinterpret_cast<int*>(items + n);
    ORB_HIP_TRY(hipMemcpy(items, h.data(), n * sizeof(QtItem), hipMemcpyHostToDevice));
    hipLaunchKernelGGL(qt_sort_test_kernel, dim3(1), dim3(256), 0, 0, items, n, scratch);
    ORB_HIP_TRY(hipGetLastError());
    ORB_HIP_TRY(hipMemcpy(h.data(), items, n * sizeof(QtItem), hipMemcpyDeviceToHost));
    d.release();
    for (int i = 0; i < n; i++) perm[i] = h[i].node;
    return ORB_OK;
}

static void stereo_side(const orbx_extractor* h, StereoSide& s) {
    std::memset(&s, 0, sizeof(s));
    const Geom& g = h->geom;
    s.nlevels = g.nlevels;
    s.lvl0 = h->last_in;
    s.fstride0 = h->last_fstride;
    s.step0 = (int)h->last_step;
    s.pyr = h->d_pyr.as<uint8_t>();
    s.pyr_frame = g.pyr_frame_bytes;
    for (int l = 0; l < g.nlevels; l++) {
        s.off[l] = g.lv[l].off;
        s.stride[l] = g.lv[l].stride;
        s.rows[l] = g.lv[l].h;
        s.cols[l] = g.lv[l].w;
    }
}

static int stereo_check_pair(const orbx_extractor* left, const orbx_extractor* right, bool same_cap) {
    ORB_CHECK_ARG(left->g_rows == right->g_rows && left->g_cols == right->g_cols &&
                      left->p.nlevels == right->p.nlevels && left->p.scaleFactor == right->p.scaleFactor && same_cap,
                  "left / right extractors differ in image size or pyramid parameters");
    ORB_CHECK_ARG(left->p.nlevels <= ST_MAX_LEVELS, "too many levels");
    return ORB_OK;
}

static int stereo_setup(orbx_extractor* left, const orbx_extractor* right, float bf, float baseline, int n_frames, int cap,
                        StereoSide& L, StereoSide& R, StereoParams& sp) {
    stereo_side(left, L);
    stereo_side(right, R);
    std::memset(&sp, 0, sizeof(sp));
    for (int l = 0; l < left->p.nlevels; l++) {
        sp.scale[l] = left->scale[l];
        sp.inv_scale[l] = left->inv_scale[l];
    }
    sp.bf = bf;
    sp.baseline = baseline;
    const size_t ints = stereo_scratch_ints(n_frames, cap, L.rows[0], stereo_row_span(sp, left->p.nlevels));
    return left->d_stereo_sad.reserve(ints * sizeof(int32_t));
}

int orbx_stereo_matches_batch_device(orbx_extractor* left, orbx_extractor* right, int n_frames,
                                     const orbx_keypoint* d_kps_l, const uint8_t* d_desc_l,
                                     const int32_t* d_counts_l, const orbx_keypoint* d_kps_r,
                                     const uint8_t* d_desc_r, const int32_t* d_counts_r, int cap, float bf,
                                     float baseline, float* d_uright, float* d_depth, void* stream) {
    ORB_CHECK_ARG(left && right && d_kps_l && d_desc_l && d_counts_l && d_kps_r && d_desc_r && d_counts_r && d_uright &&
                      d_depth, "null argument");
    ORB_CHECK_ARG(n_frames > 0 && cap > 0, "bad sizes");
    ORB_CHECK_ARG(left->last_in && right->last_in && left->last_frames >= n_frames && right->last_frames >= n_frames,
                  "both extractors need a batch of >= n_frames frames first");
    if (int rc = stereo_check_pair(left, right, true)) return rc;
    std::lock_guard<std::mutex> lk(left->mu);
    ORB_HIP_TRY(hipSetDevice(left->device));
    int rc;
    StereoSide L, R;
    StereoParams sp;
    if ((rc = stereo_setup(left, right, bf, baseline, n_frames, cap, L, R, sp))) return rc;
    return launch_stereo(L, R, sp, n_frames, d_kps_l, d_desc_l, d_counts_l, 0, d_kps_r, d_desc_r, d_counts_r, 0, cap,
                         d_uright, d_depth, left->d_stereo_sad.as<int32_t>(), (hipStream_t)stream);
}

int orbx_stereo_matches_last(orbx_extractor* left, orbx_extractor* right, float bf, float baseline, float* uright,
                             float* depth, int n_left) {
    ORB_CHECK_ARG(left && right && left != right && uright && depth, "null argument");
    ORB_CHECK_ARG(left->last_single && right->last_single, "both extractors need a single-frame orbx_extract first");
    if (int rc = stereo_check_pair(left, right, left->last_kcap == right->last_kcap)) return rc;
    std::unique_lock<std::mutex> la(left->mu, std::defer_lock), lb(right->mu, std::defer_lock);
    std::lock(la, lb);
    ORB_HIP_TRY(hipSetDevice(left->device));
    const int cap = left->last_kcap;
    int32_t nl = 0;
    ORB_HIP_TRY(hipMemcpy(&nl, left->d_counts.ptr, 4, hipMemcpyDeviceToHost));
    ORB_CHECK_ARG(n_left == nl, "n_left differs from the left extractor's keypoint count");
    if (nl == 0) return ORB_OK;
    int rc;
    StereoSide L, R;
    StereoParams sp;
    if ((rc = stereo_setup(left, right, bf, baseline, 1, cap, L, R, sp))) return rc;
    if ((rc = left->d_stereo_out.reserve(2 * (size_t)cap * sizeof(float)))) return rc;
    float* d_u = left->d_stereo_out.as<float>();
    float* d_d = d_u + cap;
    hipStream_t st = left->stream;
    if ((rc = launch_stereo(L, R, sp, 1, left->d_kps.as<orbx_keypoint>(), left->d_desc.as<uint8_t>(),
                            left->d_counts.as<int32_t>(), 0, right->d_kps.as<orbx_keypoint>(), right->d_desc.as<uint8_t>(),
                            right->d_counts.as<int32_t>(), 0, cap, d_u, d_d, left->d_stereo_sad.as<int32_t>(), st)))
        return rc;
    ORB_HIP_TRY(hipMemcpyAsync(uright, d_u, (size_t)nl * sizeof(float), hipMemcpyDeviceToHost, st));
    ORB_HIP_TRY(hipMemcpyAsync(depth, d_d, (size_t)nl * sizeof(float), hipMemcpyDeviceToHost, st));
    ORB_HIP_TRY(hipStreamSynchronize(st));
    return ORB_OK;
}

int orbx_debug_fast_stamps(unsigned long long* out, int n_words) {
#ifdef ORB_FAST_STAMPS
    ORB_CHECK_ARG(out && n_words > 0 && n_words <= FAST_NSAMP * 8, "bad stamp buffer");
    ORB_HIP_TRY(hipMemcpyFromSymbol(out, HIP_SYMBOL(g_fast_stamps), (size_t)n_words * 8));
    return ORB_OK;
#else
    (void)out;
    (void)n_words;
    set_error("built without ORB_FAST_STAMPS");
    return ORB_EINVAL;
#endif
}

int orbx_debug_qt_stamps(unsigned long long* out) {
#if defined(ORB_DESC_STAMPS)
    ORB_HIP_TRY(hipDeviceSynchronize());
    ORB_HIP_TRY(hipMemcpyFromSymbol(out + 64, HIP_SYMBOL(g_desc_stamps), 1024 * 8 * 8));
    return ORB_OK;
#elif defined(ORB_QT_STAMPS)
    ORB_HIP_TRY(hipDeviceSynchronize());
    ORB_HIP_TRY(hipMemcpyFromSymbol(out, HIP_SYMBOL(g_qt_stamps), 64 * 8));
    ORB_HIP_TRY(hipMemcpyFromSymbol(out + 64, HIP_SYMBOL(g_qt_wg), 4096 * 2 * 8));
    return ORB_OK;
#else
    (void)out;
    set_error("built without ORB_QT_STAMPS");
    return ORB_EINVAL;
#endif
}

}
```

### orb_slam2_refactored_amd/csrc/orbx_pyramid.h

```cpp
#pragma once
#include <cmath>
#include <type_traits>
#include <vector>

#include "orbx_geom.h"
#include "orbx_pyr_rect.h"

namespace orbamd {

typedef unsigned short us2 __attribute__((ext_vector_type(2)));

__device__ __forceinline__ uint32_t htap24(uint32_t h) { return h & 0xffff0u; }
__device__ __forceinline__ uint32_t mulhi24(uint32_t a, uint32_t b) {
    uint32_t r;
    asm("v_mul_hi_u32_u24 %0, %1, %2" : "=v"(r) : "v"(a), "v"(b));
    return r;
}
__device__ __forceinline__ uint32_t vcoef24(int b) { return ((uint32_t)b & 0xfffu) << 12; }
__device__ __forceinline__ uint32_t vtail(uint32_t h0, uint32_t h1, uint32_t b0_24, uint32_t b1_24) {
    return (__umul24(h0, b0_24 >> 12) + __umul24(h1, b1_24 >> 12) + (1u << 21)) >> 22;
}

__device__ __forceinline__ us2 pyr_tap(uint32_t hi, uint32_t lo, uint32_t sel) {
    const uint32_t r = __builtin_amdgcn_perm(hi, lo, sel);
    return *reinterpret_cast<const us2*>(&r);
}

struct PyrRecipTab { unsigned m[PYR_RECIP_N]; };
constexpr PyrRecipTab pyr_recip_tab() {
    PyrRecipTab t{};
    for (int n = 1; n < PYR_RECIP_N; n++) t.m[n] = pyr_recip20(n);
    return t;
}
__constant__ PyrRecipTab c_pyr_recip = pyr_recip_tab();
static_assert(PYR_SW / 16 < PYR_RECIP_N, "the staging piece counts are in the table");

__device__ __forceinline__ int4 pyr_row_taps(int2 yv, int sy_lo) {
    return make_int4(((yv.x & 0xffff) - sy_lo) * PYR_SW, ((yv.x >> 16) - sy_lo) * PYR_SW, (int)vcoef24(yv.y),
                     (int)vcoef24(yv.y >> 16));
}

__device__ __forceinline__ void pyr_tile_compute(const Geom& g, const LevelDev& L, int f, uint8_t* pyr,
                                                 const uint8_t* S, const int2* xs_t, const int4* ys_t, int tx0,
                                                 int ty0, int tw, int th, int xa) {
    {
        const int q0 = (threadIdx.x & 15) * 4;
        uint32_t sel0[2], sel1[2];
        int wdb[2];
        us2 a0[2], a1[2];
        bool fits = true;
#pragma unroll
        for (int j = 0; j < 2; j++) {
            const int2 xv0 = xs_t[min(q0 + 2 * j, tw - 1)], xv1 = xs_t[min(q0 + 2 * j + 1, tw - 1)];
            const int s00 = (xv0.x & 0xffff) - xa, s01 = (xv0.x >> 16) - xa;
            const int s10 = (xv1.x & 0xffff) - xa, s11 = (xv1.x >> 16) - xa;
            const int wd = s00 >> 2;
            const int e00 = s00 - 4 * wd, e01 = s01 - 4 * wd, e10 = s10 - 4 * wd, e11 = s11 - 4 * wd;
            fits = fits && max(e01, e11) <= 7 && min(e00, e10) >= 0;
            sel0[j] = (uint32_t)e00 | 0x0c00u | ((uint32_t)e01 << 16) | 0x0c000000u;
            sel1[j] = (uint32_t)e10 | 0x0c00u | ((uint32_t)e11 << 16) | 0x0c000000u;
            wdb[j] = 4 * wd;
            a0[j] = *reinterpret_cast<const us2*>(&xv0.y);
            a1[j] = *reinterpret_cast<const us2*>(&xv1.y);
        }
        if (!__syncthreads_or(!fits)) {
            if (q0 >= tw) return;
            const bool full = q0 + 3 < tw;
            uint8_t* dst = pyr + (long long)f * g.pyr_frame_bytes + L.off + tx0 + q0 +
                           (long long)(ty0 + (int)(threadIdx.x >> 4)) * L.stride;
            const long long dstep = 16ll * L.stride;
            const int tcol = L.tail_x - (tx0 + q0);
            auto rows = [&](auto tail_c) {
                constexpr bool TAIL = decltype(tail_c)::value;
                for (int ty = threadIdx.x >> 4; ty < th; ty += 16, dst += dstep) {
                    const int4 yv = ys_t[ty];
                    const uint32_t b0 = (uint32_t)yv.z, b1 = (uint32_t)yv.w;
                    uint32_t out = 0;
#pragma unroll
                    for (int j = 0; j < 2; j++) {
                        const uint32_t* s0 = reinterpret_cast<const uint32_t*>(S + yv.x + wdb[j]);
                        const uint32_t* s1 = reinterpret_cast<const uint32_t*>(S + yv.y + wdb[j]);
                        const uint32_t w00 = s0[0], w01 = s0[1], w10 = s1[0], w11 = s1[1];
                        const uint32_t r0a = __builtin_amdgcn_udot2(pyr_tap(w01, w00, sel0[j]), a0[j], 0u, false);
                        const uint32_t r1a = __builtin_amdgcn_udot2(pyr_tap(w11, w10, sel0[j]), a0[j], 0u, false);
                        const uint32_t r0b = __builtin_amdgcn_udot2(pyr_tap(w01, w00, sel1[j]), a1[j], 0u, false);
                        const uint32_t r1b = __builtin_amdgcn_udot2(pyr_tap(w11, w10, sel1[j]), a1[j], 0u, false);
                        uint32_t va = (mulhi24(htap24(r0a), b0) + mulhi24(htap24(r1a), b1) + 2) >> 2;
                        uint32_t vb = (mulhi24(htap24(r0b), b0) + mulhi24(htap24(r1b), b1) + 2) >> 2;
                        if (TAIL) {
                            va = 2 * j >= tcol ? vtail(r0a, r1a, b0, b1) : va;
                            vb = 2 * j + 1 >= tcol ? vtail(r0b, r1b, b0, b1) : vb;
                        }
                        out |= (va | (vb << 8)) << (16 * j);
                    }
                    if (full) {
                        *reinterpret_cast<uint32_t*>(dst) = out;
                    } else {
                        for (int k = 0; k < 3; k++)
                            if (q0 + k < tw) dst[k] = (uint8_t)(out >> (8 * k));
                    }
                }
            };
            if (tx0 + tw > L.tail_x) rows(std::true_type{});
            else
                rows(std::false_type{});
            return;
        }
    }
    const int q0 = (threadIdx.x & 15) * 4;
    if (q0 >= tw) return;
    uint8_t* dbase = pyr + (long long)f * g.pyr_frame_bytes + L.off + tx0 + q0;
#pragma nounroll
    for (int ty = threadIdx.x >> 4; ty < th; ty += 16) {
        const int4 yv = ys_t[ty];
        const int r0 = yv.x, r1 = yv.y;
        const int b0 = yv.z >> 12, b1 = yv.w >> 12;
        uint32_t packed = 0;
#pragma nounroll
        for (int k = 0; k < 4; k++) {
            const int2 xv = xs_t[min(q0 + k, tw - 1)];
            const int sx0 = (xv.x & 0xffff) - xa, sx1 = (xv.x >> 16) - xa, a0 = xv.y & 0xffff, a1 = xv.y >> 16;
            const int h0 = S[r0 + sx0] * a0 + S[r0 + sx1] * a1;
            const int h1 = S[r1 + sx0] * a0 + S[r1 + sx1] * a1;
            const int s0 = min(h0 >> 4, 32767), s1 = min(h1 >> 4, 32767);
            int v = (((s0 * b0) >> 16) + ((s1 * b1) >> 16) + 2) >> 2;
            if (tx0 + q0 + k >= L.tail_x) v = (h0 * b0 + h1 * b1 + (1 << 21)) >> 22;
            packed |= (uint32_t)(v > 255 ? 255 : v) << (8 * k);
        }
        uint8_t* dst = dbase + (long long)(ty0 + ty) * L.stride;
        if (q0 + 3 < tw) *reinterpret_cast<uint32_t*>(dst) = packed;
        else {
            dst[0] = (uint8_t)packed;
            if (q0 + 1 < tw) dst[1] = (uint8_t)(packed >> 8);
            if (q0 + 2 < tw) dst[2] = (uint8_t)(packed >> 16);
        }
    }
}


struct PyrTile {
    int f, tx0, ty0, tw, th, sy_lo, xa, nc, items, mul;
    const uint8_t* src;
    int sstep;
};

__device__ __forceinline__ PyrTile pyr_tile_geom(const Geom& g, int l, int t, int ntx, int nty, PyrSpan sx, PyrSpan sy,
                                                 const uint8_t* in, long long in_fstride, int in_step, uint8_t* pyr) {
    const LevelDev& L = g.lv[l];
    PyrTile T;
    const int per = ntx * nty;
    T.f = t / per;
    const int r = t - T.f * per;
    T.ty0 = (r / ntx) * PYR_TH;
    T.tx0 = (r - (r / ntx) * ntx) * PYR_TW;
    T.tw = min(PYR_TW, L.w - T.tx0);
    T.th = min(PYR_TH, L.h - T.ty0);
    T.sy_lo = sy.lo;
    T.xa = sx.lo & ~15;
    T.nc = ((sx.hi - T.xa) >> 4) + 1;
    T.items = (sy.hi - sy.lo + 1) * T.nc;
    T.mul = (int)c_pyr_recip.m[T.nc];
    T.src = level_base(g, l - 1, T.f, in, in_fstride, in_step, pyr, &T.sstep);
    auto u = [](int x) { return __builtin_amdgcn_readfirstlane(x); };
    T.f = u(T.f), T.tx0 = u(T.tx0), T.ty0 = u(T.ty0), T.tw = u(T.tw), T.th = u(T.th), T.sy_lo = u(T.sy_lo);
    T.xa = u(T.xa), T.nc = u(T.nc), T.items = u(T.items), T.mul = u(T.mul), T.sstep = u(T.sstep);
    const unsigned long long sp = (unsigned long long)(uintptr_t)T.src;
    T.src = (const uint8_t*)(uintptr_t)(((unsigned long long)(unsigned)u((int)(sp >> 32)) << 32) |
                                        (unsigned)u((int)(unsigned)sp));
    return T;
}

__device__ __forceinline__ int pyr_piece_row(const PyrTile& T, int i) {
    return (int)(__umulhi(((unsigned)i & 0x7ffu) << 12, (unsigned)T.mul & 0xffffffu) & 0x7ffu);
}
__device__ __forceinline__ int mul12(int a, int b) {
    return (int)(((unsigned)a & 0xfffu) * ((unsigned)b & 0xfffu));
}
__device__ __forceinline__ void pyr_piece_load(const PyrTile& T, int i, uint4& v) {
    if (i < T.items) {
        const int rr = pyr_piece_row(T, i), c = i - mul12(rr, T.nc);
        v = *reinterpret_cast<const uint4*>(T.src + __mul24(T.sy_lo + rr, T.sstep) + T.xa + 16 * c);
    }
}

__device__ __forceinline__ void pyr_fetch(const PyrTile& T, int tid, uint4& v0, uint4& v1, uint4& v2, uint4& v3,
                                          uint4& v4) {
    static_assert(PYR_PF == 5, "five pieces per thread");
    pyr_piece_load(T, tid, v0);
    pyr_piece_load(T, tid + 256, v1);
    pyr_piece_load(T, tid + 512, v2);
    pyr_piece_load(T, tid + 768, v3);
    pyr_piece_load(T, tid + 1024, v4);
}

__device__ __forceinline__ void pyr_stage(const PyrTile& T, int tid, uint8_t* S, const uint4& v, int k) {
    const int i = tid + 256 * k;
    if (i < T.items) {
        const int rr = pyr_piece_row(T, i), c = i - mul12(rr, T.nc);
        *reinterpret_cast<uint4*>(&S[mul12(rr, PYR_SW) + 16 * c]) = v;
    }
}

__global__ __launch_bounds__(256) void pyramid_level_kernel(Geom g, int l, const uint8_t* __restrict__ in,
                                                            long long in_fstride, int in_step, uint8_t* pyr,
                                                            const int2* __restrict__ xtab,
                                                            const int2* __restrict__ ytab) {
    __shared__ __attribute__((aligned(16))) uint8_t S[PYR_SH * PYR_SW + 16];
    __shared__ int2 xs_t[PYR_TW];
    __shared__ int4 ys_t[PYR_TH];
    const LevelDev& L = g.lv[l];
    const LevelDev& Ls = g.lv[l - 1];
    const int gx = gridDim.x, gxy = gridDim.x * gridDim.y;
    const int lb = xcd_swizzle(blockIdx.x + gx * blockIdx.y + gxy * blockIdx.z, gxy * gridDim.z);
    const int f = lb / gxy;
    const int tx0 = (lb % gx) * PYR_TW, ty0 = ((lb % gxy) / gx) * PYR_TH;
    const int tw = min(PYR_TW, L.w - tx0), th = min(PYR_TH, L.h - ty0);
    int sstep;
    const uint8_t* src = level_base(g, l - 1, f, in, in_fstride, in_step, pyr, &sstep);
    const int2* xt = xtab + L.xtab_off;
    const int2* yt = ytab + L.ytab_off;
    const int sw = Ls.w;
    const PyrSpan sx = pyr_tap_span(xt, tx0, tx0 + tw - 1), sy = pyr_tap_span(yt, ty0, ty0 + th - 1);
    const int sx_lo = __builtin_amdgcn_readfirstlane(sx.lo), sx_hi = __builtin_amdgcn_readfirstlane(sx.hi);
    const int sy_lo = __builtin_amdgcn_readfirstlane(sy.lo), sy_hi = __builtin_amdgcn_readfirstlane(sy.hi);
    if ((int)threadIdx.x < tw) xs_t[threadIdx.x] = xt[tx0 + threadIdx.x];
    if ((int)threadIdx.x >= 64 && (int)threadIdx.x - 64 < th)
        ys_t[threadIdx.x - 64] = pyr_row_taps(yt[ty0 + threadIdx.x - 64], sy_lo);
    const int xa = sx_lo & ~3;
    const int nd = (sx_hi - xa + 4) >> 2;
    const int nr = sy_hi - sy_lo + 1;
    const bool aligned = ((reinterpret_cast<uintptr_t>(src) | (uintptr_t)sstep) & 3) == 0;
    if (((reinterpret_cast<uintptr_t>(src) | (uintptr_t)sstep) & 15) == 0 && sx_hi - (sx_lo & ~15) < PYR_SW) {
        const PyrTile T = pyr_tile_geom(g, l, lb, gx, gridDim.y, PyrSpan{sx_lo, sx_hi}, PyrSpan{sy_lo, sy_hi}, in,
                                        in_fstride, in_step, pyr);
        uint4 v0, v1, v2, v3, v4;
        pyr_fetch(T, threadIdx.x, v0, v1, v2, v3, v4);
        pyr_stage(T, threadIdx.x, S, v0, 0);
        pyr_stage(T, threadIdx.x, S, v1, 1);
        pyr_stage(T, threadIdx.x, S, v2, 2);
        pyr_stage(T, threadIdx.x, S, v3, 3);
        pyr_stage(T, threadIdx.x, S, v4, 4);
        __syncthreads();
        pyr_tile_compute(g, L, f, pyr, S, xs_t, ys_t, tx0, ty0, tw, th, T.xa);
        return;
    }
    if (aligned) {
        constexpr int RPW = PYR_SH / 4;
        const int wv = __builtin_amdgcn_readfirstlane((int)(threadIdx.x >> 6));
        const int ln = threadIdx.x & 63;
        const int col = min(xa + 4 * ln, (sw - 1) & ~3);
        const uint8_t* rbase = src + (long long)sy_lo * sstep + col;
        uint32_t v[RPW];
#pragma unroll
        for (int k = 0; k < RPW; k++) {
            const int rk = min(wv + 4 * k, nr - 1);
            v[k] = *reinterpret_cast<const uint32_t*>(rbase + (long long)rk * sstep);
        }
        if (ln < nd) {
            uint32_t* drow = reinterpret_cast<uint32_t*>(S) + wv * (PYR_SW / 4) + ln;
#pragma unroll
            for (int k = 0; k < RPW; k++)
                if (wv + 4 * k < nr) drow[k * PYR_SW] = v[k];
        }
    } else {
        for (int i = threadIdx.x; i < nd * nr; i += blockDim.x) {
            const int r = i / nd, d = i - r * nd;
            const uint8_t* rowp = src + (long long)(sy_lo + r) * sstep;
            const int x = xa + 4 * d;
            uint32_t v = 0;
            for (int q = 0; q < 4; q++)
                if (x + q < sw) v |= (uint32_t)rowp[x + q] << (8 * q);
            *reinterpret_cast<uint32_t*>(&S[r * PYR_SW + 4 * d]) = v;
        }
    }
    __syncthreads();
    pyr_tile_compute(g, L, f, pyr, S, xs_t, ys_t, tx0, ty0, tw, th, xa);
}


__device__ __forceinline__ uint32_t pyr_px_generic(const uint8_t* S, int2 xv, int4 yv, int xa, bool tail) {
    const int r0 = yv.x, r1 = yv.y;
    const int sx0 = (xv.x & 0xffff) - xa, sx1 = (xv.x >> 16) - xa, a0 = xv.y & 0xffff, a1 = xv.y >> 16;
    const int b0 = yv.z >> 12, b1 = yv.w >> 12;
    const int h0 = S[r0 + sx0] * a0 + S[r0 + sx1] * a1;
    const int h1 = S[r1 + sx0] * a0 + S[r1 + sx1] * a1;
    const int s0 = min(h0 >> 4, 32767), s1 = min(h1 >> 4, 32767);
    int v = (((s0 * b0) >> 16) + ((s1 * b1) >> 16) + 2) >> 2;
    if (tail) v = (h0 * b0 + h1 * b1 + (1 << 21)) >> 22;
    return (uint32_t)(v > 255 ? 255 : v);
}

template <int NP>
__global__ __launch_bounds__(256) void pyramid_pair_kernel(Geom g, int l, const uint8_t* __restrict__ in,
                                                           long long in_fstride, int in_step, uint8_t* pyr,
                                                           const int2* __restrict__ xtab,
                                                           const int2* __restrict__ ytab) {
    __shared__ __attribute__((aligned(16))) uint8_t S[PYR_SH * PYR_SW + 16];
    __shared__ int2 xs1[PP_MAXC], xs2[PYR_TW];
    __shared__ int4 ys1[PP_MAXR], ys2[PYR_TH];
    const LevelDev& L1 = g.lv[l];
    const LevelDev& L2 = g.lv[l + 1];
    const int tid = threadIdx.x;
    const int gx = gridDim.x, gxy = gridDim.x * gridDim.y;
    const int lb = xcd_swizzle(blockIdx.x + gx * blockIdx.y + gxy * blockIdx.z, gxy * gridDim.z);
    const int f = lb / gxy;
    const int tx0 = (lb % gx) * PYR_TW, ty0 = ((lb % gxy) / gx) * PYR_TH;
    const int tw = min(PYR_TW, L2.w - tx0), th = min(PYR_TH, L2.h - ty0);
    auto u = [](int x) { return __builtin_amdgcn_readfirstlane(x); };
    const PyrPairRect R = pyr_pair_rect(xtab + L1.xtab_off, ytab + L1.ytab_off, xtab + L2.xtab_off,
                                        ytab + L2.ytab_off, tx0, ty0, tw, th);
    const int c0 = u(R.c0), c1 = u(R.c1), ay0 = u(R.ay0), ay1 = u(R.ay1);
    const int ncol = c1 - c0 + 1, nrow = ay1 - ay0 + 1;
    PyrTile T;
    T.sy_lo = u(R.by0);
    T.xa = u(R.xa);
    T.nc = u(((R.bx1 - R.xa) >> 4) + 1);
    T.items = u((R.by1 - R.by0 + 1) * T.nc);
    T.mul = u((int)c_pyr_recip.m[T.nc]);
    T.src = level_base(g, l - 1, f, in, in_fstride, in_step, pyr, &T.sstep);
    {
        uint4 v0, v1, v2, v3, v4;
        pyr_fetch(T, tid, v0, v1, v2, v3, v4);
        if (tid < ncol) xs1[tid] = xtab[L1.xtab_off + c0 + tid];
        if (tid < nrow) ys1[tid] = pyr_row_taps(ytab[L1.ytab_off + ay0 + tid], T.sy_lo);
        if (tid < tw) xs2[tid] = xtab[L2.xtab_off + tx0 + tid];
        if (tid < th) ys2[tid] = pyr_row_taps(ytab[L2.ytab_off + ty0 + tid], ay0);
        pyr_stage(T, tid, S, v0, 0);
        pyr_stage(T, tid, S, v1, 1);
        pyr_stage(T, tid, S, v2, 2);
        pyr_stage(T, tid, S, v3, 3);
        pyr_stage(T, tid, S, v4, 4);
    }
    __syncthreads();
    const int ncq = (ncol + 3) >> 2;
    const unsigned m20 = (unsigned)u((int)c_pyr_recip.m[ncq]);
    const int rpp = (int)(m20 >> 12);
    const int r0 = (int)(__umul24((unsigned)tid, m20) >> 20), q = tid - __mul24(r0, ncq);
    const bool act = r0 < rpp;
    uint32_t out[NP];
    if (act) {
        uint32_t sel0[2], sel1[2], wdv[2];
        us2 a0[2], a1[2];
        int2 xv[4];
        bool fits = true;
#pragma unroll
        for (int k = 0; k < 4; k++) xv[k] = xs1[min(4 * q + k, ncol - 1)];
#pragma unroll
        for (int j = 0; j < 2; j++) {
            const int2 xv0 = xv[2 * j], xv1 = xv[2 * j + 1];
            const int s00 = (xv0.x & 0xffff) - T.xa, s01 = (xv0.x >> 16) - T.xa;
            const int s10 = (xv1.x & 0xffff) - T.xa, s11 = (xv1.x >> 16) - T.xa;
            const int wd = s00 >> 2;
            const int e00 = s00 - 4 * wd, e01 = s01 - 4 * wd, e10 = s10 - 4 * wd, e11 = s11 - 4 * wd;
            fits = fits && max(e01, e11) <= 7 && min(e00, e10) >= 0;
            sel0[j] = (uint32_t)e00 | 0x0c00u | ((uint32_t)e01 << 16) | 0x0c000000u;
            sel1[j] = (uint32_t)e10 | 0x0c00u | ((uint32_t)e11 << 16) | 0x0c000000u;
            wdv[j] = (uint32_t)wd;
            a0[j] = *reinterpret_cast<const us2*>(&xv0.y);
            a1[j] = *reinterpret_cast<const us2*>(&xv1.y);
        }
        const int tcol = L1.tail_x - (c0 + 4 * q);
        auto rows = [&](auto tail_c) {
            constexpr bool TAIL = decltype(tail_c)::value;
#pragma unroll
            for (int pp = 0; pp < NP; pp++) {
                const int r = r0 + pp * rpp;
                out[pp] = 0;
                if (pp * rpp >= nrow) break;
                if ((pp + 1) * rpp > nrow && r >= nrow) break;
                const int4 yv = ys1[r];
                if (fits) {
                    const uint32_t b0 = (uint32_t)yv.z, b1 = (uint32_t)yv.w;
#pragma unroll
                    for (int j = 0; j < 2; j++) {
                        const uint32_t* s0 = reinterpret_cast<const uint32_t*>(S + yv.x + 4 * (int)wdv[j]);
                        const uint32_t* s1 = reinterpret_cast<const uint32_t*>(S + yv.y + 4 * (int)wdv[j]);
                        const uint32_t w00 = s0[0], w01 = s0[1], w10 = s1[0], w11 = s1[1];
                        const uint32_t r0a = __builtin_amdgcn_udot2(pyr_tap(w01, w00, sel0[j]), a0[j], 0u, false);
                        const uint32_t r1a = __builtin_amdgcn_udot2(pyr_tap(w11, w10, sel0[j]), a0[j], 0u, false);
                        const uint32_t r0b = __builtin_amdgcn_udot2(pyr_tap(w01, w00, sel1[j]), a1[j], 0u, false);
                        const uint32_t r1b = __builtin_amdgcn_udot2(pyr_tap(w11, w10, sel1[j]), a1[j], 0u, false);
                        uint32_t va = (mulhi24(htap24(r0a), b0) + mulhi24(htap24(r1a), b1) + 2) >> 2;
                        uint32_t vb = (mulhi24(htap24(r0b), b0) + mulhi24(htap24(r1b), b1) + 2) >> 2;
                        if (TAIL) {
                            va = 2 * j >= tcol ? vtail(r0a, r1a, b0, b1) : va;
                            vb = 2 * j + 1 >= tcol ? vtail(r0b, r1b, b0, b1) : vb;
                        }
                        out[pp] |= (va | (vb << 8)) << (16 * j);
                    }
                } else {
#pragma unroll
                    for (int k = 0; k < 4; k++) out[pp] |= pyr_px_generic(S, xv[k], yv, T.xa, k >= tcol) << (8 * k);
                }
            }
        };
        if (c1 >= L1.tail_x) rows(std::true_type{});
        else
            rows(std::false_type{});
    }
    __syncthreads();
    if (act) {
        uint8_t* lrow = pyr + (long long)f * g.pyr_frame_bytes + L1.off + c0 + 4 * q;
        const bool full = c0 + 4 * q + 3 <= c1;
#pragma unroll
        for (int pp = 0; pp < NP; pp++) {
            const int r = r0 + pp * rpp;
            if (pp * rpp >= nrow) break;
            if ((pp + 1) * rpp > nrow && r >= nrow) break;
            *reinterpret_cast<uint32_t*>(&S[r * PYR_SW + 4 * q]) = out[pp];
            uint8_t* dst = lrow + __mul24(ay0 + r, L1.stride);
            if (full) {
                *reinterpret_cast<uint32_t*>(dst) = out[pp];
            } else {
                for (int k = 0; k < 3; k++)
                    if (c0 + 4 * q + k <= c1) dst[k] = (uint8_t)(out[pp] >> (8 * k));
            }
        }
    }
    __syncthreads();
    pyr_tile_compute(g, L2, f, pyr, S, xs2, ys2, tx0, ty0, tw, th, c0);
}

static int pyr_pair_fits(const Geom& g, int l, const std::vector<int2>& xtab, const std::vector<int2>& ytab) {
    const LevelDev &L0 = g.lv[l - 1], &L1 = g.lv[l], &L2 = g.lv[l + 1];
    const PyrPairPlan P = pyr_pair_plan(L0.w, L0.h, L1.w, L1.h, L2.w, L2.h, xtab.data() + L1.xtab_off,
                                        ytab.data() + L1.ytab_off, xtab.data() + L2.xtab_off, ytab.data() + L2.ytab_off);
    if (!P.ok) return 0;
    return P.passes <= 7 ? 7 : PP_MAXP;
}

typedef _Float16 h8v __attribute__((ext_vector_type(8)));
typedef float pf4v __attribute__((ext_vector_type(4)));
struct PyrMfmaLane { uint32_t a[4]; float c[4]; };
constexpr int PM_MAXB1 = 6;
constexpr int PM_TAB = PYR_SH;
constexpr int PM_MAXU1 = 12;


template <bool TAIL>
__device__ __forceinline__ uint32_t pyr_mfma_unit(const uint8_t* sp, int k, const h8v& A, const pf4v& C, const int4& t,
                                                  int tcol) {
    const int g = lane_id() >> 4;
    constexpr uint32_t hmask = TAIL ? 0xfffffu : 0xffff0u;
    const uint2 w = *reinterpret_cast<const uint2*>(sp + k * (15 * PYR_SW));
    const uint4 bu = make_uint4(__builtin_amdgcn_perm(0x64646464u, w.x, 0x04010400u),
                                __builtin_amdgcn_perm(0x64646464u, w.x, 0x04030402u),
                                __builtin_amdgcn_perm(0x64646464u, w.y, 0x04010400u),
                                __builtin_amdgcn_perm(0x64646464u, w.y, 0x04030402u));
    const pf4v d = __builtin_amdgcn_mfma_f32_16x16x32_f16(A, __builtin_bit_cast(h8v, bu), C, 0, 0, 0);
    const uint32_t b0 = (uint32_t)t.y, b1 = (uint32_t)t.z;
    uint32_t out = 0;
#pragma unroll
    for (int j = 0; j < 4; j++) {
        const uint32_t h0 = __float_as_uint(d[j]) & hmask;
        const uint32_t h1 = (uint32_t)__builtin_amdgcn_mov_dpp((int)h0, 0x101, 0xf, 0xf, true);
        uint32_t v;
        if (!TAIL) {
            v = (mulhi24(h0, b0) + mulhi24(h1, b1) + 2) >> 2;
        } else {
            v = (mulhi24(h0 & 0xffff0u, b0) + mulhi24(h1 & 0xffff0u, b1) + 2) >> 2;
            v = 4 * g + j >= tcol ? vtail(h0, h1, b0, b1) : v;
        }
        out |= v << (8 * j);
    }
    return out;
}

__device__ __forceinline__ void pyr_mfma_frag(const PyrMfmaLane* tab, h8v& A, pf4v& C) {
    const PyrMfmaLane t = tab[lane_id()];
    A = __builtin_bit_cast(h8v, make_uint4(t.a[0], t.a[1], t.a[2], t.a[3]));
    C = pf4v{t.c[0], t.c[1], t.c[2], t.c[3]};
}

__device__ __forceinline__ void pyr_mfma_tab(const int2* ytab, int r0, int nrow, int sy_lo, int ostride, int4* tab) {
    const int y = threadIdx.x;
    if (y < nrow) {
        const int2 v = ytab[r0 + y];
        const int s0 = (v.x & 0xffff) - sy_lo;
        const int s0n = y + 1 < nrow ? (ytab[r0 + y + 1].x & 0xffff) - sy_lo : PM_TAB;
        if (y == 0)
            for (int r = 0; r < s0; r++) tab[r] = make_int4(-1, 0, 0, -1);
        tab[s0] = make_int4((r0 + y) * ostride, (int)vcoef24(v.y), (int)vcoef24(v.y >> 16), y);
        for (int r = s0 + 1; r < min(s0n, PM_TAB); r++) tab[r] = make_int4(-1, 0, 0, -1);
    }
}

__device__ __forceinline__ void pyr_store4(uint8_t* dst, uint32_t o, int col, int last) {
    if (col + 3 <= last) *reinterpret_cast<uint32_t*>(dst) = o;
    else
        for (int k = 0; k < 3; k++)
            if (col + k <= last) dst[k] = (uint8_t)(o >> (8 * k));
}

__global__ __launch_bounds__(256) void pyramid_pair_mfma_kernel(Geom g, int l, const uint8_t* __restrict__ in,
                                                                long long in_fstride, int in_step, uint8_t* pyr,
                                                                const int2* __restrict__ ytab,
                                                                const PyrMfmaLane* __restrict__ mt,
                                                                const int* __restrict__ mkb) {
    __shared__ __attribute__((aligned(16))) uint8_t S[PYR_SH * PYR_SW + 16];
    __shared__ int4 tab1[PM_TAB], tab2[PM_TAB];
    const LevelDev& L0 = g.lv[l - 1];
    const LevelDev& L1 = g.lv[l];
    const LevelDev& L2 = g.lv[l + 1];
    const int tid = threadIdx.x;
    const int w = __builtin_amdgcn_readfirstlane(tid >> 6);
    const int gx = gridDim.x, gxy = gridDim.x * gridDim.y;
    const int lb = xcd_swizzle(blockIdx.x + gx * blockIdx.y + gxy * blockIdx.z, gxy * gridDim.z);
    const int f = lb / gxy;
    const int tx0 = (lb % gx) * PYR_TW, ty0 = ((lb % gxy) / gx) * PYR_TH;
    const int tw = min(PYR_TW, L2.w - tx0), th = min(PYR_TH, L2.h - ty0);
    auto u = [](int x) { return __builtin_amdgcn_readfirstlane(x); };
    const int ax0 = max(0, (int)floor((tx0 + 0.5) * L2.ssx - 0.5) - 2);
    const int c1 = u(min(L1.w - 1, (int)floor((tx0 + tw - 0.5) * L2.ssx - 0.5) + 2));
    const int ay0 = u(max(0, (int)floor((ty0 + 0.5) * L2.ssy - 0.5) - 2));
    const int ay1 = u(min(L1.h - 1, (int)floor((ty0 + th - 0.5) * L2.ssy - 0.5) + 2));
    const int c0 = u(ax0 & ~15);
    const int ncol = c1 - c0 + 1, nrow = ay1 - ay0 + 1;
    PyrTile T;
    const int bx0 = max(0, (int)floor((c0 + 0.5) * L1.ssx - 0.5) - 2);
    const int bx1 = min(L0.w - 1, (int)floor((c1 + 0.5) * L1.ssx - 0.5) + 2);
    T.sy_lo = u(max(0, (int)floor((ay0 + 0.5) * L1.ssy - 0.5) - 2));
    const int by1 = u(min(L0.h - 1, (int)floor((ay1 + 0.5) * L1.ssy - 0.5) + 2));
    T.xa = u(bx0 & ~15);
    T.nc = u(((bx1 - T.xa) >> 4) + 1);
    T.items = u((by1 - T.sy_lo + 1) * T.nc);
    T.mul = u(((1 << 20) + T.nc - 1) / T.nc);
    T.src = level_base(g, l - 1, f, in, in_fstride, in_step, pyr, &T.sstep);
    const int rep1 = by1 == L0.h - 1 ? by1 - T.sy_lo : -1;
    {
        uint4 v0, v1, v2, v3, v4;
        pyr_fetch(T, tid, v0, v1, v2, v3, v4);
        pyr_mfma_tab(ytab + L1.ytab_off, ay0, nrow, T.sy_lo, (int)L1.stride, tab1);
        pyr_mfma_tab(ytab + L2.ytab_off, ty0, th, ay0, (int)L2.stride, tab2);
        auto stage = [&](const uint4& v, int k) {
            const int i = tid + 256 * k;
            if (i < T.items) {
                const int rr = pyr_piece_row(T, i), c = i - mul12(rr, T.nc);
                *reinterpret_cast<uint4*>(&S[mul12(rr, PYR_SW) + 16 * c]) = v;
                if (rr == rep1) *reinterpret_cast<uint4*>(&S[mul12(rr + 1, PYR_SW) + 16 * c]) = v;
            }
        };
        stage(v0, 0);
        stage(v1, 1);
        stage(v2, 2);
        stage(v3, 3);
        stage(v4, 4);
    }
    __syncthreads();
    const int n = tid & 15, q = (tid >> 4) & 3;
    const int nb1 = (ncol + 15) >> 4;
    const int g1 = u(((ytab[L1.ytab_off + ay1].x & 0xffff) - T.sy_lo) / 15 + 1);
    const int nu1 = nb1 * g1;
    const int ub = (nu1 * w) >> 2, ue = (nu1 * (w + 1)) >> 2;
    uint32_t o1[PM_MAXU1];
    uint8_t* lbase = pyr + (long long)f * g.pyr_frame_bytes + L1.off + c0 + 4 * q;
    {
        int cur = -1;
        h8v A;
        pf4v C;
        const uint8_t* sp = S;
        int tcol = 16;
#pragma unroll
        for (int i = 0; i < PM_MAXU1; i++) {
            const int un = ub + i;
            if (un >= ue) break;
            const int b = un / g1, k = un - b * g1;
            if (b != cur) {
                cur = b;
                const int blk = L1.mt_off + ((c0 >> 4) + b);
                pyr_mfma_frag(mt + (long long)blk * 64, A, C);
                sp = S + (mkb[blk] - T.xa + 8 * q + n * PYR_SW);
                tcol = L1.tail_x - (c0 + 16 * b);
            }
            const int4 t = tab1[15 * k + n];
            o1[i] = tcol < 16 ? pyr_mfma_unit<true>(sp, k, A, C, t, tcol) : pyr_mfma_unit<false>(sp, k, A, C, t, tcol);
            const int col = c0 + 16 * b + 4 * q;
            if (t.x >= 0 && n < 15 && col <= c1) pyr_store4(lbase + 16 * b + t.x, o1[i], col, c1);
        }
    }
    __syncthreads();
    const int rep2 = ay1 == L1.h - 1 ? nrow - 1 : -1;
#pragma unroll
    for (int i = 0; i < PM_MAXU1; i++) {
        const int un = ub + i;
        if (un >= ue) break;
        const int b = un / g1, k = un - b * g1;
        const int4 t = tab1[15 * k + n];
        if (t.x >= 0 && n < 15) {
            *reinterpret_cast<uint32_t*>(&S[t.w * PYR_SW + 16 * b + 4 * q]) = o1[i];
            if (t.w == rep2) *reinterpret_cast<uint32_t*>(&S[(t.w + 1) * PYR_SW + 16 * b + 4 * q]) = o1[i];
        }
    }
    __syncthreads();
    if (16 * w < tw) {
        const int bc = tx0 + 16 * w;
        const int blk = L2.mt_off + (bc >> 4);
        h8v A;
        pf4v C;
        pyr_mfma_frag(mt + (long long)blk * 64, A, C);
        const uint8_t* sp = S + (mkb[blk] - c0 + 8 * q + n * PYR_SW);
        const int col = bc + 4 * q;
        const int tcol = L2.tail_x - bc;
        const int g2 = u(((ytab[L2.ytab_off + ty0 + th - 1].x & 0xffff) - ay0) / 15 + 1);
        uint8_t* dbase = pyr + (long long)f * g.pyr_frame_bytes + L2.off + col;
        const int last = tx0 + tw - 1;
        auto run = [&](auto tail_c) {
            constexpr bool TAIL = decltype(tail_c)::value;
            for (int k = 0; k < g2; k++) {
                const int4 t = tab2[15 * k + n];
                const uint32_t o = pyr_mfma_unit<TAIL>(sp, k, A, C, t, tcol);
                if (t.x >= 0 && n < 15 && col <= last) pyr_store4(dbase + t.x, o, col, last);
            }
        };
        if (tcol < 16) run(std::true_type{});
        else run(std::false_type{});
    }
}

static uint16_t f16_of_int(int v) {
    if (v <= 0) return 0;
    int e = 0;
    while ((2 << e) <= v) e++;
    const int m = e >= 10 ? (v - (1 << e)) >> (e - 10) : (v - (1 << e)) << (10 - e);
    return (uint16_t)(((e + 15) << 10) | m);
}

static int pyr_mfma_tables(const int2* xt, int dw, std::vector<PyrMfmaLane>& mt, std::vector<int>& mkb) {
    const int nb = (dw + 15) / 16;
    std::vector<PyrMfmaLane> lanes((size_t)nb * 64);
    std::vector<int> kbs(nb);
    for (int j = 0; j < nb; j++) {
        const int kb = (xt[16 * j].x & 0xffff) & ~7;
        kbs[j] = kb;
        for (int ln = 0; ln < 64; ln++) {
            PyrMfmaLane& t = lanes[(size_t)j * 64 + ln];
            const int c = 16 * j + (ln & 15), gq = ln >> 4;
            uint16_t hv[8] = {0, 0, 0, 0, 0, 0, 0, 0};
            if (c < dw) {
                const int sx0 = xt[c].x & 0xffff, sx1 = xt[c].x >> 16, a0 = xt[c].y & 0xffff, a1 = xt[c].y >> 16;
                const int e0 = sx0 - kb, e1 = sx1 - kb;
                if (e0 < 0 || e1 < e0 || e1 > 31 || a0 < 0 || a1 < 0 || a0 + a1 > 4096) return -1;
                for (int k = 0; k < 8; k++) {
                    const int kk = 8 * gq + k;
                    const int wv = (kk == e0 ? a0 : 0) + (kk == e1 ? a1 : 0);
                    if (wv > 2048) return -1;
                    hv[k] = f16_of_int(wv);
                }
            }
            for (int k = 0; k < 4; k++) t.a[k] = (uint32_t)hv[2 * k] | ((uint32_t)hv[2 * k + 1] << 16);
            for (int r = 0; r < 4; r++) {
                const int cm = 16 * j + 4 * gq + r;
                const int sum = cm < dw ? (xt[cm].y & 0xffff) + (xt[cm].y >> 16) : 0;
                t.c[r] = (float)(8388608 - 1024 * sum);
            }
        }
    }
    const int off = (int)mkb.size();
    mt.insert(mt.end(), lanes.begin(), lanes.end());
    mkb.insert(mkb.end(), kbs.begin(), kbs.end());
    return off;
}

static bool pyr_mfma_pair_fits(const Geom& g, int l, const std::vector<int>& mkb, const std::vector<int2>& ytab) {
    const LevelDev &L0 = g.lv[l - 1], &L1 = g.lv[l], &L2 = g.lv[l + 1];
    if (L1.mt_off < 0 || L2.mt_off < 0) return false;
    auto fl = [](double v) { return (int)std::floor(v); };
    int max_rows = 0, max_nc = 0, max_nb1 = 0, max_g1 = 0;
    for (int ty0 = 0; ty0 < L2.h; ty0 += PYR_TH) {
        const int th = std::min(PYR_TH, L2.h - ty0);
        const int ay0 = std::max(0, fl((ty0 + 0.5) * L2.ssy - 0.5) - 2);
        const int ay1 = std::min(L1.h - 1, fl((ty0 + th - 0.5) * L2.ssy - 0.5) + 2);
        const int nrow = ay1 - ay0 + 1;
        const int sy_lo = std::max(0, fl((ay0 + 0.5) * L1.ssy - 0.5) - 2);
        const int by1 = std::min(L0.h - 1, fl((ay1 + 0.5) * L1.ssy - 0.5) + 2);
        if (nrow > PP_MAXR || by1 - sy_lo + 1 > PYR_SH) return false;
        max_rows = std::max(max_rows, by1 - sy_lo + 1);
        max_g1 = std::max(max_g1, ((ytab[L1.ytab_off + ay1].x & 0xffff) - sy_lo) / 15 + 1);
        auto rows_ok = [&](const LevelDev& L, const LevelDev& Ls, int r0, int nr, int lo, int staged) {
            int prev = -1;
            for (int y = 0; y < nr; y++) {
                const int2 v = ytab[L.ytab_off + r0 + y];
                const int s0 = (v.x & 0xffff) - lo, s1 = (v.x >> 16) - lo;
                if (s0 <= prev || s0 < 0 || !(s1 == s0 + 1 || (s1 == s0 && (v.x >> 16) == Ls.h - 1))) return false;
                if (s1 >= staged) return false;
                prev = s0;
            }
            const int groups = prev / 15 + 1;
            return 15 * groups < PM_TAB && 15 * groups < PYR_SH && staged + 1 <= PYR_SH;
        };
        if (!rows_ok(L1, L0, ay0, nrow, sy_lo, by1 - sy_lo + 1) || !rows_ok(L2, L1, ty0, th, ay0, nrow)) return false;
    }
    for (int tx0 = 0; tx0 < L2.w; tx0 += PYR_TW) {
        const int tw = std::min(PYR_TW, L2.w - tx0);
        const int ax0 = std::max(0, fl((tx0 + 0.5) * L2.ssx - 0.5) - 2);
        const int c1 = std::min(L1.w - 1, fl((tx0 + tw - 0.5) * L2.ssx - 0.5) + 2);
        const int c0 = ax0 & ~15;
        const int ncol = c1 - c0 + 1;
        const int bx0 = std::max(0, fl((c0 + 0.5) * L1.ssx - 0.5) - 2);
        const int bx1 = std::min(L0.w - 1, fl((c1 + 0.5) * L1.ssx - 0.5) + 2);
        const int xa = bx0 & ~15, nc = ((bx1 - xa) >> 4) + 1;
        if (ncol > 16 * PM_MAXB1 || 16 * nc > PYR_SW) return false;
        max_nb1 = std::max(max_nb1, (ncol + 15) / 16);
        max_nc = std::max(max_nc, nc);
        for (int b = 0; b < (ncol + 15) / 16; b++) {
            const int kbrel = mkb[L1.mt_off + (c0 >> 4) + b] - xa;
            if (kbrel < 0 || kbrel + 32 > PYR_SW) return false;
        }
        for (int b = 0; 16 * b < tw; b++) {
            const int kbrel = mkb[L2.mt_off + (tx0 >> 4) + b] - c0;
            if (kbrel < 0 || kbrel + 32 > PYR_SW) return false;
        }
    }
    return max_rows * max_nc <= PYR_PF * 256 && max_nb1 * max_g1 <= 4 * PM_MAXU1;
}

}
```

Measured before the change: 177,100 frames/s.

## Group multiple frames per pyramid workgroup to reuse tile setup

Pyramid level and pair kernels now process K frames per workgroup, looping over frames with the next frame's source pieces prefetched while the current one is computed. Per-tile column tables, tap selectors and lane geometry are computed once and reused across frames. K is chosen from the workgroup count relative to the CU count times a residency factor, capped by default at 2. This cuts redundant per-block setup and launch overhead, but grouping reduces grid parallelism and adds extra barriers per frame. A debug entry point for querying pair-plan passes is also added.

```diff
diff --git a/include/orbslam2_amd.h b/include/orbslam2_amd.h
--- a/include/orbslam2_amd.h
+++ b/include/orbslam2_amd.h
@@ -57,6 +57,8 @@
 
 int orbx_pyramid_device(const orbx_extractor* h, int frame, int level, const uint8_t** ptr,
                         int* rows, int* cols, size_t* step);
+
+int orbx_debug_pyramid_pairs(orbx_extractor* h, int rows, int cols, int32_t* np, int n);
 
 
 int orbm_descriptor_distance(const uint8_t* a, const uint8_t* b);
diff --git a/orb_slam2_refactored_amd/_lib.py b/orb_slam2_refactored_amd/_lib.py
--- a/orb_slam2_refactored_amd/_lib.py
+++ b/orb_slam2_refactored_amd/_lib.py
@@ -216,6 +216,7 @@
     "orbx_fault_word_device": (C.c_int, [VP, C.POINTER(VP)]),
     "orbx_pyramid_device": (C.c_int, [VP, C.c_int, C.c_int, C.POINTER(VP), C.POINTER(C.c_int),
                                       C.POINTER(C.c_int), C.POINTER(SZ)]),
+    "orbx_debug_pyramid_pairs": (C.c_int, [VP, C.c_int, C.c_int, VP, C.c_int]),
     "orbm_descriptor_distance": (C.c_int, [VP, VP]),
     "orbm_hamming_top2_device": (C.c_int, [VP, C.c_int, VP, C.c_int, VP, VP, VP, VP]),
     "orbm_bf_match_batch_device": (C.c_int, [VP, VP, C.c_int, VP, VP, C.c_int, VP, C.c_int, C.c_float, C.c_int,
diff --git a/orb_slam2_refactored_amd/csrc/orbx.hip b/orb_slam2_refactored_amd/csrc/orbx.hip
--- a/orb_slam2_refactored_amd/csrc/orbx.hip
+++ b/orb_slam2_refactored_amd/csrc/orbx.hip
@@ -54,6 +54,7 @@
     std::vector<int> pyr_pair_np;
     DevBuf d_pyrmt, d_pyrkb;
     int pyr_pair = 2;
+    int pyr_k = 0, pyr_k_cap = 2, pyr_k_sets = 4, pyr_resident = 256 * 7;
     int trig_float = 0;
     int resize_simd = 0;
     std::vector<std::pair<hipStream_t, hipEvent_t>> sub;
@@ -526,13 +527,25 @@
                          h->d_ytab.as<int2>(), h->d_pyrmt.as<PyrMfmaLane>(), h->d_pyrkb.as<int>());
             return 1;
         }
+        auto grouped = [&](int lt, int* K) {
+            dim3 gr = tiles(lt);
+            const long long wgs = (long long)gr.x * gr.y * F;
+            *K = h->pyr_k > 0 ? h->pyr_k : (int)std::max(1ll, std::min((long long)h->pyr_k_cap, wgs / ((long long)h->pyr_k_sets * h->pyr_resident)));
+            *K = std::min(*K, F);
+            gr.z = (unsigned)((F + *K - 1) / *K);
+            return gr;
+        };
+        int K = 1;
         if (pair && h->pyr_pair_np[l]) {
-            launch_timed(h, 0, h->pyr_pair_np[l] <= 7 ? pyramid_pair_kernel<7> : pyramid_pair_kernel<PP_MAXP>, tiles(l + 1),
-                         dim3(256), 0u, st, g, l, d_imgs, fstride, step, pyr, h->d_xtab.as<int2>(), h->d_ytab.as<int2>());
+            const bool np7 = h->pyr_pair_np[l] <= 7;
+            const dim3 gr = grouped(l + 1, &K);
+            launch_timed(h, 0, np7 ? pyramid_pair_kernel<7> : pyramid_pair_kernel<PP_MAXP>, gr, dim3(256), 0u, st, g, l, d_imgs, fstride, step, pyr, h->d_xtab.as<int2>(), h->d_ytab.as<int2>(),
+                         F, K);
             return 1;
         }
-        launch_timed(h, 0, pyramid_level_kernel, tiles(l), dim3(256), 0u, st, g, l, d_imgs, fstride, step, pyr,
-                     h->d_xtab.as<int2>(), h->d_ytab.as<int2>());
+        const dim3 gr = grouped(l, &K);
+        launch_timed(h, 0, pyramid_level_kernel, gr, dim3(256), 0u, st, g, l, d_imgs, fstride, step, pyr,
+                     h->d_xtab.as<int2>(), h->d_ytab.as<int2>(), F, K);
         return 0;
     };
     const int nc0 = g.lv[0].ncells;
@@ -705,6 +718,14 @@
     if (const char* e = getenv("ORBX_NSUB")) h->nsub = std::max(1, std::min(8, atoi(e)));
     if (const char* e = getenv("ORBX_PYR_PAIR")) h->pyr_pair = std::max(0, std::min(2, atoi(e)));
     if (const char* e = getenv("ORBX_PYR_MFMA")) h->pyr_mfma = atoi(e) != 0;
+    if (const char* e = getenv("ORBX_PYR_K")) h->pyr_k = std::max(0, std::min(65535, atoi(e)));
+    if (const char* e = getenv("ORBX_PYR_K_CAP")) h->pyr_k_cap = std::max(1, std::min(65535, atoi(e)));
+    if (const char* e = getenv("ORBX_PYR_K_SETS")) h->pyr_k_sets = std::max(1, std::min(4096, atoi(e)));
+    {
+        int cus = 0;
+        if (hipDeviceGetAttribute(&cus, hipDeviceAttributeMultiprocessorCount, device) == hipSuccess && cus > 0)
+            h->pyr_resident = cus * 7;
+    }
     if (const char* e = getenv("ORBX_LEVEL_OVERLAP")) h->lvl_overlap = atoi(e) != 0;
     if (const char* e = getenv("ORBX_DEBUG_NC")) h->debug_nc = atoi(e);
     if (const char* e = getenv("ORBX_DESC_DENSE")) h->desc_dense = atoi(e) != 0;
@@ -911,6 +932,16 @@
     return ORB_OK;
 }
 
+int orbx_debug_pyramid_pairs(orbx_extractor* h, int rows, int cols, int32_t* np, int n) {
+    ORB_CHECK_ARG(h && np && rows > 0 && cols > 0, "bad argument");
+    std::lock_guard<std::mutex> lk(h->mu);
+    ORB_HIP_TRY(hipSetDevice(h->device));
+    int rc = setup_geometry(h, rows, cols);
+    if (rc) return rc;
+    for (int l = 0; l < n; l++) np[l] = l < (int)h->pyr_pair_np.size() ? h->pyr_pair_np[l] : 0;
+    return ORB_OK;
+}
+
 int orbx_pyramid_level(const orbx_extractor* h, int level, uint8_t* dst, size_t dst_step, int* rows, int* cols) {
     const uint8_t* p = nullptr;
     int r = 0, c = 0;
diff --git a/orb_slam2_refactored_amd/csrc/orbx_pyramid.h b/orb_slam2_refactored_amd/csrc/orbx_pyramid.h
--- a/orb_slam2_refactored_amd/csrc/orbx_pyramid.h
+++ b/orb_slam2_refactored_amd/csrc/orbx_pyramid.h
@@ -40,243 +40,63 @@
                      (int)vcoef24(yv.y >> 16));
 }
 
-__device__ __forceinline__ void pyr_tile_compute(const Geom& g, const LevelDev& L, int f, uint8_t* pyr,
-                                                 const uint8_t* S, const int2* xs_t, const int4* ys_t, int tx0,
-                                                 int ty0, int tw, int th, int xa) {
-    {
-        const int q0 = (threadIdx.x & 15) * 4;
-        uint32_t sel0[2], sel1[2];
-        int wdb[2];
-        us2 a0[2], a1[2];
-        bool fits = true;
-#pragma unroll
-        for (int j = 0; j < 2; j++) {
-            const int2 xv0 = xs_t[min(q0 + 2 * j, tw - 1)], xv1 = xs_t[min(q0 + 2 * j + 1, tw - 1)];
-            const int s00 = (xv0.x & 0xffff) - xa, s01 = (xv0.x >> 16) - xa;
-            const int s10 = (xv1.x & 0xffff) - xa, s11 = (xv1.x >> 16) - xa;
-            const int wd = s00 >> 2;
-            const int e00 = s00 - 4 * wd, e01 = s01 - 4 * wd, e10 = s10 - 4 * wd, e11 = s11 - 4 * wd;
-            fits = fits && max(e01, e11) <= 7 && min(e00, e10) >= 0;
-            sel0[j] = (uint32_t)e00 | 0x0c00u | ((uint32_t)e01 << 16) | 0x0c000000u;
-            sel1[j] = (uint32_t)e10 | 0x0c00u | ((uint32_t)e11 << 16) | 0x0c000000u;
-            wdb[j] = 4 * wd;
-            a0[j] = *reinterpret_cast<const us2*>(&xv0.y);
-            a1[j] = *reinterpret_cast<const us2*>(&xv1.y);
-        }
-        if (!__syncthreads_or(!fits)) {
-            if (q0 >= tw) return;
-            const bool full = q0 + 3 < tw;
-            uint8_t* dst = pyr + (long long)f * g.pyr_frame_bytes + L.off + tx0 + q0 +
-                           (long long)(ty0 + (int)(threadIdx.x >> 4)) * L.stride;
-            const long long dstep = 16ll * L.stride;
-            const int tcol = L.tail_x - (tx0 + q0);
-            auto rows = [&](auto tail_c) {
-                constexpr bool TAIL = decltype(tail_c)::value;
-                for (int ty = threadIdx.x >> 4; ty < th; ty += 16, dst += dstep) {
-                    const int4 yv = ys_t[ty];
-                    const uint32_t b0 = (uint32_t)yv.z, b1 = (uint32_t)yv.w;
-                    uint32_t out = 0;
-#pragma unroll
-                    for (int j = 0; j < 2; j++) {
-                        const uint32_t* s0 = reinterpret_cast<const uint32_t*>(S + yv.x + wdb[j]);
-                        const uint32_t* s1 = reinterpret_cast<const uint32_t*>(S + yv.y + wdb[j]);
-                        const uint32_t w00 = s0[0], w01 = s0[1], w10 = s1[0], w11 = s1[1];
-                        const uint32_t r0a = __builtin_amdgcn_udot2(pyr_tap(w01, w00, sel0[j]), a0[j], 0u, false);
-                        const uint32_t r1a = __builtin_amdgcn_udot2(pyr_tap(w11, w10, sel0[j]), a0[j], 0u, false);
-                        const uint32_t r0b = __builtin_amdgcn_udot2(pyr_tap(w01, w00, sel1[j]), a1[j], 0u, false);
-                        const uint32_t r1b = __builtin_amdgcn_udot2(pyr_tap(w11, w10, sel1[j]), a1[j], 0u, false);
-                        uint32_t va = (mulhi24(htap24(r0a), b0) + mulhi24(htap24(r1a), b1) + 2) >> 2;
-                        uint32_t vb = (mulhi24(htap24(r0b), b0) + mulhi24(htap24(r1b), b1) + 2) >> 2;
-                        if (TAIL) {
-                            va = 2 * j >= tcol ? vtail(r0a, r1a, b0, b1) : va;
-                            vb = 2 * j + 1 >= tcol ? vtail(r0b, r1b, b0, b1) : vb;
-                        }
-                        out |= (va | (vb << 8)) << (16 * j);
-                    }
-                    if (full) {
-                        *reinterpret_cast<uint32_t*>(dst) = out;
-                    } else {
-                        for (int k = 0; k < 3; k++)
-                            if (q0 + k < tw) dst[k] = (uint8_t)(out >> (8 * k));
-                    }
-                }
-            };
-            if (tx0 + tw > L.tail_x) rows(std::true_type{});
-            else
-                rows(std::false_type{});
-            return;
-        }
-    }
-    const int q0 = (threadIdx.x & 15) * 4;
-    if (q0 >= tw) return;
-    uint8_t* dbase = pyr + (long long)f * g.pyr_frame_bytes + L.off + tx0 + q0;
-#pragma nounroll
-    for (int ty = threadIdx.x >> 4; ty < th; ty += 16) {
-        const int4 yv = ys_t[ty];
-        const int r0 = yv.x, r1 = yv.y;
-        const int b0 = yv.z >> 12, b1 = yv.w >> 12;
-        uint32_t packed = 0;
-#pragma nounroll
-        for (int k = 0; k < 4; k++) {
-            const int2 xv = xs_t[min(q0 + k, tw - 1)];
-            const int sx0 = (xv.x & 0xffff) - xa, sx1 = (xv.x >> 16) - xa, a0 = xv.y & 0xffff, a1 = xv.y >> 16;
-            const int h0 = S[r0 + sx0] * a0 + S[r0 + sx1] * a1;
-            const int h1 = S[r1 + sx0] * a0 + S[r1 + sx1] * a1;
-            const int s0 = min(h0 >> 4, 32767), s1 = min(h1 >> 4, 32767);
-            int v = (((s0 * b0) >> 16) + ((s1 * b1) >> 16) + 2) >> 2;
-            if (tx0 + q0 + k >= L.tail_x) v = (h0 * b0 + h1 * b1 + (1 << 21)) >> 22;
-            packed |= (uint32_t)(v > 255 ? 255 : v) << (8 * k);
-        }
-        uint8_t* dst = dbase + (long long)(ty0 + ty) * L.stride;
-        if (q0 + 3 < tw) *reinterpret_cast<uint32_t*>(dst) = packed;
-        else {
-            dst[0] = (uint8_t)packed;
-            if (q0 + 1 < tw) dst[1] = (uint8_t)(packed >> 8);
-            if (q0 + 2 < tw) dst[2] = (uint8_t)(packed >> 16);
-        }
-    }
-}
-
-
-struct PyrTile {
-    int f, tx0, ty0, tw, th, sy_lo, xa, nc, items, mul;
-    const uint8_t* src;
-    int sstep;
+
+__device__ __forceinline__ int pyr_keep_v(int x) {
+    asm volatile("" : "+v"(x));
+    return x;
+}
+__device__ __forceinline__ int pyr_keep_s(int x) {
+    asm volatile("" : "+s"(x));
+    return x;
+}
+
+struct PyrCols {
+    uint32_t sel0[2], sel1[2];
+    int wdb[2];
+    us2 a0[2], a1[2];
 };
-
-__device__ __forceinline__ PyrTile pyr_tile_geom(const Geom& g, int l, int t, int ntx, int nty, PyrSpan sx, PyrSpan sy,
-                                                 const uint8_t* in, long long in_fstride, int in_step, uint8_t* pyr) {
-    const LevelDev& L = g.lv[l];
-    PyrTile T;
-    const int per = ntx * nty;
-    T.f = t / per;
-    const int r = t - T.f * per;
-    T.ty0 = (r / ntx) * PYR_TH;
-    T.tx0 = (r - (r / ntx) * ntx) * PYR_TW;
-    T.tw = min(PYR_TW, L.w - T.tx0);
-    T.th = min(PYR_TH, L.h - T.ty0);
-    T.sy_lo = sy.lo;
-    T.xa = sx.lo & ~15;
-    T.nc = ((sx.hi - T.xa) >> 4) + 1;
-    T.items = (sy.hi - sy.lo + 1) * T.nc;
-    T.mul = (int)c_pyr_recip.m[T.nc];
-    T.src = level_base(g, l - 1, T.f, in, in_fstride, in_step, pyr, &T.sstep);
-    auto u = [](int x) { return __builtin_amdgcn_readfirstlane(x); };
-    T.f = u(T.f), T.tx0 = u(T.tx0), T.ty0 = u(T.ty0), T.tw = u(T.tw), T.th = u(T.th), T.sy_lo = u(T.sy_lo);
-    T.xa = u(T.xa), T.nc = u(T.nc), T.items = u(T.items), T.mul = u(T.mul), T.sstep = u(T.sstep);
-    const unsigned long long sp = (unsigned long long)(uintptr_t)T.src;
-    T.src = (const uint8_t*)(uintptr_t)(((unsigned long long)(unsigned)u((int)(sp >> 32)) << 32) |
-                                        (unsigned)u((int)(unsigned)sp));
-    return T;
-}
-
-__device__ __forceinline__ int pyr_piece_row(const PyrTile& T, int i) {
-    return (int)(__umulhi(((unsigned)i & 0x7ffu) << 12, (unsigned)T.mul & 0xffffffu) & 0x7ffu);
-}
-__device__ __forceinline__ int mul12(int a, int b) {
-    return (int)(((unsigned)a & 0xfffu) * ((unsigned)b & 0xfffu));
-}
-__device__ __forceinline__ void pyr_piece_load(const PyrTile& T, int i, uint4& v) {
-    if (i < T.items) {
-        const int rr = pyr_piece_row(T, i), c = i - mul12(rr, T.nc);
-        v = *reinterpret_cast<const uint4*>(T.src + __mul24(T.sy_lo + rr, T.sstep) + T.xa + 16 * c);
-    }
-}
-
-__device__ __forceinline__ void pyr_fetch(const PyrTile& T, int tid, uint4& v0, uint4& v1, uint4& v2, uint4& v3,
-                                          uint4& v4) {
-    static_assert(PYR_PF == 5, "five pieces per thread");
-    pyr_piece_load(T, tid, v0);
-    pyr_piece_load(T, tid + 256, v1);
-    pyr_piece_load(T, tid + 512, v2);
-    pyr_piece_load(T, tid + 768, v3);
-    pyr_piece_load(T, tid + 1024, v4);
-}
-
-__device__ __forceinline__ void pyr_stage(const PyrTile& T, int tid, uint8_t* S, const uint4& v, int k) {
-    const int i = tid + 256 * k;
-    if (i < T.items) {
-        const int rr = pyr_piece_row(T, i), c = i - mul12(rr, T.nc);
-        *reinterpret_cast<uint4*>(&S[mul12(rr, PYR_SW) + 16 * c]) = v;
-    }
-}
-
-__global__ __launch_bounds__(256) void pyramid_level_kernel(Geom g, int l, const uint8_t* __restrict__ in,
-                                                            long long in_fstride, int in_step, uint8_t* pyr,
-                                                            const int2* __restrict__ xtab,
-                                                            const int2* __restrict__ ytab) {
-    __shared__ __attribute__((aligned(16))) uint8_t S[PYR_SH * PYR_SW + 16];
-    __shared__ int2 xs_t[PYR_TW];
-    __shared__ int4 ys_t[PYR_TH];
-    const LevelDev& L = g.lv[l];
-    const LevelDev& Ls = g.lv[l - 1];
-    const int gx = gridDim.x, gxy = gridDim.x * gridDim.y;
-    const int lb = xcd_swizzle(blockIdx.x + gx * blockIdx.y + gxy * blockIdx.z, gxy * gridDim.z);
-    const int f = lb / gxy;
-    const int tx0 = (lb % gx) * PYR_TW, ty0 = ((lb % gxy) / gx) * PYR_TH;
-    const int tw = min(PYR_TW, L.w - tx0), th = min(PYR_TH, L.h - ty0);
-    int sstep;
-    const uint8_t* src = level_base(g, l - 1, f, in, in_fstride, in_step, pyr, &sstep);
-    const int2* xt = xtab + L.xtab_off;
-    const int2* yt = ytab + L.ytab_off;
-    const int sw = Ls.w;
-    const PyrSpan sx = pyr_tap_span(xt, tx0, tx0 + tw - 1), sy = pyr_tap_span(yt, ty0, ty0 + th - 1);
-    const int sx_lo = __builtin_amdgcn_readfirstlane(sx.lo), sx_hi = __builtin_amdgcn_readfirstlane(sx.hi);
-    const int sy_lo = __builtin_amdgcn_readfirstlane(sy.lo), sy_hi = __builtin_amdgcn_readfirstlane(sy.hi);
-    if ((int)threadIdx.x < tw) xs_t[threadIdx.x] = xt[tx0 + threadIdx.x];
-    if ((int)threadIdx.x >= 64 && (int)threadIdx.x - 64 < th)
-        ys_t[threadIdx.x - 64] = pyr_row_taps(yt[ty0 + threadIdx.x - 64], sy_lo);
-    const int xa = sx_lo & ~3;
-    const int nd = (sx_hi - xa + 4) >> 2;
-    const int nr = sy_hi - sy_lo + 1;
-    const bool aligned = ((reinterpret_cast<uintptr_t>(src) | (uintptr_t)sstep) & 3) == 0;
-    if (((reinterpret_cast<uintptr_t>(src) | (uintptr_t)sstep) & 15) == 0 && sx_hi - (sx_lo & ~15) < PYR_SW) {
-        const PyrTile T = pyr_tile_geom(g, l, lb, gx, gridDim.y, PyrSpan{sx_lo, sx_hi}, PyrSpan{sy_lo, sy_hi}, in,
-                                        in_fstride, in_step, pyr);
-        uint4 v0, v1, v2, v3, v4;
-        pyr_fetch(T, threadIdx.x, v0, v1, v2, v3, v4);
-        pyr_stage(T, threadIdx.x, S, v0, 0);
-        pyr_stage(T, threadIdx.x, S, v1, 1);
-        pyr_stage(T, threadIdx.x, S, v2, 2);
-        pyr_stage(T, threadIdx.x, S, v3, 3);
-        pyr_stage(T, threadIdx.x, S, v4, 4);
-        __syncthreads();
-        pyr_tile_compute(g, L, f, pyr, S, xs_t, ys_t, tx0, ty0, tw, th, T.xa);
-        return;
-    }
-    if (aligned) {
-        constexpr int RPW = PYR_SH / 4;
-        const int wv = __builtin_amdgcn_readfirstlane((int)(threadIdx.x >> 6));
-        const int ln = threadIdx.x & 63;
-        const int col = min(xa + 4 * ln, (sw - 1) & ~3);
-        const uint8_t* rbase = src + (long long)sy_lo * sstep + col;
-        uint32_t v[RPW];
-#pragma unroll
-        for (int k = 0; k < RPW; k++) {
-            const int rk = min(wv + 4 * k, nr - 1);
-            v[k] = *reinterpret_cast<const uint32_t*>(rbase + (long long)rk * sstep);
-        }
-        if (ln < nd) {
-            uint32_t* drow = reinterpret_cast<uint32_t*>(S) + wv * (PYR_SW / 4) + ln;
-#pragma unroll
-            for (int k = 0; k < RPW; k++)
-                if (wv + 4 * k < nr) drow[k * PYR_SW] = v[k];
-        }
-    } else {
-        for (int i = threadIdx.x; i < nd * nr; i += blockDim.x) {
-            const int r = i / nd, d = i - r * nd;
-            const uint8_t* rowp = src + (long long)(sy_lo + r) * sstep;
-            const int x = xa + 4 * d;
-            uint32_t v = 0;
-            for (int q = 0; q < 4; q++)
-                if (x + q < sw) v |= (uint32_t)rowp[x + q] << (8 * q);
-            *reinterpret_cast<uint32_t*>(&S[r * PYR_SW + 4 * d]) = v;
-        }
-    }
-    __syncthreads();
-    pyr_tile_compute(g, L, f, pyr, S, xs_t, ys_t, tx0, ty0, tw, th, xa);
-}
-
+__device__ __forceinline__ bool pyr_cols(const int2* xs_t, int q0, int n, int xa, PyrCols& C) {
+    bool fits = true;
+#pragma unroll
+    for (int j = 0; j < 2; j++) {
+        const int2 xv0 = xs_t[min(q0 + 2 * j, n - 1)], xv1 = xs_t[min(q0 + 2 * j + 1, n - 1)];
+        const int s00 = (xv0.x & 0xffff) - xa, s01 = (xv0.x >> 16) - xa;
+        const int s10 = (xv1.x & 0xffff) - xa, s11 = (xv1.x >> 16) - xa;
+        const int wd = s00 >> 2;
+        const int e00 = s00 - 4 * wd, e01 = s01 - 4 * wd, e10 = s10 - 4 * wd, e11 = s11 - 4 * wd;
+        fits = fits && max(e01, e11) <= 7 && min(e00, e10) >= 0;
+        C.sel0[j] = (uint32_t)e00 | 0x0c00u | ((uint32_t)e01 << 16) | 0x0c000000u;
+        C.sel1[j] = (uint32_t)e10 | 0x0c00u | ((uint32_t)e11 << 16) | 0x0c000000u;
+        C.wdb[j] = 4 * wd;
+        C.a0[j] = *reinterpret_cast<const us2*>(&xv0.y);
+        C.a1[j] = *reinterpret_cast<const us2*>(&xv1.y);
+    }
+    return fits;
+}
+
+template <bool TAIL>
+__device__ __forceinline__ uint32_t pyr_row4(const uint8_t* S, const int4& yv, const PyrCols& C, int tcol) {
+    const uint32_t b0 = (uint32_t)yv.z, b1 = (uint32_t)yv.w;
+    uint32_t out = 0;
+#pragma unroll
+    for (int j = 0; j < 2; j++) {
+        const uint32_t* s0 = reinterpret_cast<const uint32_t*>(S + yv.x + C.wdb[j]);
+        const uint32_t* s1 = reinterpret_cast<const uint32_t*>(S + yv.y + C.wdb[j]);
+        const uint32_t w00 = s0[0], w01 = s0[1], w10 = s1[0], w11 = s1[1];
+        const uint32_t r0a = __builtin_amdgcn_udot2(pyr_tap(w01, w00, C.sel0[j]), C.a0[j], 0u, false);
+        const uint32_t r1a = __builtin_amdgcn_udot2(pyr_tap(w11, w10, C.sel0[j]), C.a0[j], 0u, false);
+        const uint32_t r0b = __builtin_amdgcn_udot2(pyr_tap(w01, w00, C.sel1[j]), C.a1[j], 0u, false);
+        const uint32_t r1b = __builtin_amdgcn_udot2(pyr_tap(w11, w10, C.sel1[j]), C.a1[j], 0u, false);
+        uint32_t va = (mulhi24(htap24(r0a), b0) + mulhi24(htap24(r1a), b1) + 2) >> 2;
+        uint32_t vb = (mulhi24(htap24(r0b), b0) + mulhi24(htap24(r1b), b1) + 2) >> 2;
+        if (TAIL) {
+            va = 2 * j >= tcol ? vtail(r0a, r1a, b0, b1) : va;
+            vb = 2 * j + 1 >= tcol ? vtail(r0b, r1b, b0, b1) : vb;
+        }
+        out |= (va | (vb << 8)) << (16 * j);
+    }
+    return out;
+}
 
 __device__ __forceinline__ uint32_t pyr_px_generic(const uint8_t* S, int2 xv, int4 yv, int xa, bool tail) {
     const int r0 = yv.x, r1 = yv.y;
@@ -290,135 +110,362 @@
     return (uint32_t)(v > 255 ? 255 : v);
 }
 
+struct PyrTilePrep {
+    PyrCols C;
+    uint32_t doff;
+    int tcol;
+    int rem;
+    bool fits;
+    bool tail;
+};
+__device__ __forceinline__ void pyr_tile_lane(const LevelDev& L, int tx0, int ty0, int tw, int tid, PyrTilePrep& P) {
+    const int q0 = (tid & 15) * 4;
+    P.rem = tw - 1 - q0;
+    P.doff = (uint32_t)(tx0 + q0 + (ty0 + (tid >> 4)) * L.stride);
+    P.tcol = L.tail_x - (tx0 + q0);
+}
+__device__ __forceinline__ PyrTilePrep pyr_tile_prep(const LevelDev& L, const int2* xs_t, int tx0, int ty0, int tw,
+                                                     int xa) {
+    PyrTilePrep P;
+    P.fits = !__syncthreads_or(!pyr_cols(xs_t, (threadIdx.x & 15) * 4, tw, xa, P.C));
+    pyr_tile_lane(L, tx0, ty0, tw, threadIdx.x, P);
+    P.tail = tx0 + tw > L.tail_x;
+    return P;
+}
+
+__device__ __forceinline__ void pyr_tile_rows(const LevelDev& L, uint8_t* lvl, const uint8_t* S, const int2* xs_t,
+                                              const int4* ys_t, const PyrTilePrep& P, const PyrCols& C, int tx0, int tw,
+                                              int th, int xa) {
+    const int rem = pyr_keep_v(P.rem), tcol = pyr_keep_v(P.tcol);
+    if (rem < 0) return;
+    const bool full = rem >= 3;
+    uint32_t doff = P.doff;
+    const uint32_t dstep = 16u * (uint32_t)L.stride;
+    if (P.fits) {
+        auto rows = [&](auto tail_c) {
+            constexpr bool TAIL = decltype(tail_c)::value;
+            for (int ty = threadIdx.x >> 4; ty < th; ty += 16, doff += dstep) {
+                uint8_t* dst = lvl + doff;
+                const uint32_t out = pyr_row4<TAIL>(S, ys_t[ty], C, tcol);
+                if (full) {
+                    *reinterpret_cast<uint32_t*>(dst) = out;
+                } else {
+                    for (int k = 0; k < 3; k++)
+                        if (k <= rem) dst[k] = (uint8_t)(out >> (8 * k));
+                }
+            }
+        };
+        if (P.tail) rows(std::true_type{});
+        else
+            rows(std::false_type{});
+        return;
+    }
+    const int q0 = (pyr_keep_v((int)threadIdx.x) & 15) * 4;
+#pragma nounroll
+    for (int ty = threadIdx.x >> 4; ty < th; ty += 16, doff += dstep) {
+        uint8_t* dst = lvl + doff;
+        const int4 yv = ys_t[ty];
+        uint32_t packed = 0;
+#pragma nounroll
+        for (int k = 0; k < 4; k++)
+            packed |= pyr_px_generic(S, xs_t[min(q0 + k, tw - 1)], yv, xa, tx0 + q0 + k >= L.tail_x) << (8 * k);
+        if (full) *reinterpret_cast<uint32_t*>(dst) = packed;
+        else {
+            dst[0] = (uint8_t)packed;
+            if (rem >= 1) dst[1] = (uint8_t)(packed >> 8);
+            if (rem >= 2) dst[2] = (uint8_t)(packed >> 16);
+        }
+    }
+}
+
+
+struct PyrTile {
+    int sy_lo, xa, nc, items, mul;
+    const uint8_t* src;
+    int sstep;
+};
+
+__device__ __forceinline__ int pyr_piece_row(const PyrTile& T, int i) {
+    return (int)(__umulhi(((unsigned)i & 0x7ffu) << 12, (unsigned)T.mul & 0xffffffu) & 0x7ffu);
+}
+__device__ __forceinline__ int mul12(int a, int b) {
+    return (int)(((unsigned)a & 0xfffu) * ((unsigned)b & 0xfffu));
+}
+__device__ __forceinline__ void pyr_piece_load(const PyrTile& T, int i, uint4& v) {
+    if (i < T.items) {
+        const int rr = pyr_piece_row(T, i), c = i - mul12(rr, T.nc);
+        v = *reinterpret_cast<const uint4*>(T.src + __mul24(T.sy_lo + rr, T.sstep) + T.xa + 16 * c);
+    }
+}
+
+__device__ __forceinline__ void pyr_fetch(const PyrTile& T, int tid, uint4& v0, uint4& v1, uint4& v2, uint4& v3,
+                                          uint4& v4) {
+    static_assert(PYR_PF == 5, "five pieces per thread");
+    pyr_piece_load(T, tid, v0);
+    pyr_piece_load(T, tid + 256, v1);
+    pyr_piece_load(T, tid + 512, v2);
+    pyr_piece_load(T, tid + 768, v3);
+    pyr_piece_load(T, tid + 1024, v4);
+}
+
+struct PyrPieces { uint32_t g0, g1, g2, g3, g4; int l01, l23, l4; };
+__device__ __forceinline__ int pyr_lo16(int x) { return (int)(short)x; }
+__device__ __forceinline__ int pyr_hi16(int x) { return x >> 16; }
+typedef uint32_t pyr_u4 __attribute__((ext_vector_type(4)));
+struct PyrPix { pyr_u4 v0, v1, v2, v3, v4; };
+__device__ __forceinline__ PyrPieces pyr_pieces(const PyrTile& T, int tid) {
+    static_assert(PYR_PF == 5, "five pieces per thread");
+    PyrPieces P;
+    auto one = [&](int k, uint32_t& goff, int& loff) {
+        const int i = tid + 256 * k;
+        const int rr = pyr_piece_row(T, i), c = i - mul12(rr, T.nc);
+        goff = (uint32_t)(__mul24(T.sy_lo + rr, T.sstep) + T.xa + 16 * c);
+        loff = i < T.items ? mul12(rr, PYR_SW) + 16 * c : -1;
+    };
+    int l0, l1, l2, l3;
+    one(0, P.g0, l0), one(1, P.g1, l1), one(2, P.g2, l2), one(3, P.g3, l3), one(4, P.g4, P.l4);
+    P.l01 = (l0 & 0xffff) | (l1 << 16), P.l23 = (l2 & 0xffff) | (l3 << 16);
+    return P;
+}
+__device__ __forceinline__ void pyr_piece_get(const uint8_t* src, uint32_t goff, int loff, pyr_u4& x) {
+    x = pyr_u4{0, 0, 0, 0};
+    if (loff >= 0) x = *reinterpret_cast<const pyr_u4*>(src + (uint32_t)pyr_keep_v((int)goff));
+}
+__device__ __forceinline__ void pyr_piece_put(uint8_t* S, int loff, const pyr_u4& x) {
+    if (loff >= 0) *reinterpret_cast<pyr_u4*>(S + loff) = x;
+}
+__device__ __forceinline__ void pyr_pieces_load(const PyrPieces& P, const uint8_t* src, PyrPix& v) {
+    const int l01 = pyr_keep_v(P.l01), l23 = pyr_keep_v(P.l23), l4 = pyr_keep_v(P.l4);
+    pyr_piece_get(src, P.g0, pyr_lo16(l01), v.v0);
+    pyr_piece_get(src, P.g1, pyr_hi16(l01), v.v1);
+    pyr_piece_get(src, P.g2, pyr_lo16(l23), v.v2);
+    pyr_piece_get(src, P.g3, pyr_hi16(l23), v.v3);
+    pyr_piece_get(src, P.g4, l4, v.v4);
+}
+__device__ __forceinline__ void pyr_pieces_stage(const PyrPieces& P, uint8_t* S, const PyrPix& v) {
+    const int l01 = pyr_keep_v(P.l01), l23 = pyr_keep_v(P.l23), l4 = pyr_keep_v(P.l4);
+    pyr_piece_put(S, pyr_lo16(l01), v.v0);
+    pyr_piece_put(S, pyr_hi16(l01), v.v1);
+    pyr_piece_put(S, pyr_lo16(l23), v.v2);
+    pyr_piece_put(S, pyr_hi16(l23), v.v3);
+    pyr_piece_put(S, l4, v.v4);
+}
+
+struct PyrBlock { int fbeg, fend, tx0, ty0; };
+__device__ __forceinline__ PyrBlock pyr_block(int F, int K) {
+    const int gx = gridDim.x, gxy = gridDim.x * gridDim.y;
+    const int lb = xcd_swizzle(blockIdx.x + gx * blockIdx.y + gxy * blockIdx.z, gxy * gridDim.z);
+    PyrBlock B;
+    B.fbeg = (lb / gxy) * K;
+    B.fend = min(F, B.fbeg + K);
+    B.tx0 = (lb % gx) * PYR_TW;
+    B.ty0 = ((lb % gxy) / gx) * PYR_TH;
+    return B;
+}
+
+__global__ __launch_bounds__(256) __attribute__((amdgpu_waves_per_eu(7))) void pyramid_level_kernel(Geom g, int l, const uint8_t* __restrict__ in,
+                                                            long long in_fstride, int in_step, uint8_t* pyr,
+                                                            const int2* __restrict__ xtab,
+                                                            const int2* __restrict__ ytab, int F, int K) {
+    __shared__ __attribute__((aligned(16))) uint8_t S[PYR_SH * PYR_SW + 16];
+    __shared__ int2 xs_t[PYR_TW];
+    __shared__ int4 ys_t[PYR_TH];
+    const LevelDev& L = g.lv[l];
+    const LevelDev& Ls = g.lv[l - 1];
+    const int tid = threadIdx.x;
+    const PyrBlock B = pyr_block(F, K);
+    const int tx0 = B.tx0, ty0 = B.ty0;
+    const int tw = min(PYR_TW, L.w - tx0), th = min(PYR_TH, L.h - ty0);
+    const int2* xt = xtab + L.xtab_off;
+    const int2* yt = ytab + L.ytab_off;
+    const int sw = Ls.w;
+    const PyrSpan sx = pyr_tap_span(xt, tx0, tx0 + tw - 1), sy = pyr_tap_span(yt, ty0, ty0 + th - 1);
+    const int sx_lo = __builtin_amdgcn_readfirstlane(sx.lo), sx_hi = __builtin_amdgcn_readfirstlane(sx.hi);
+    const int sy_lo = __builtin_amdgcn_readfirstlane(sy.lo), sy_hi = __builtin_amdgcn_readfirstlane(sy.hi);
+    if (tid < tw) xs_t[tid] = xt[tx0 + tid];
+    if (tid >= 64 && tid - 64 < th) ys_t[tid - 64] = pyr_row_taps(yt[ty0 + tid - 64], sy_lo);
+    int sstep;
+    const uint8_t* src = level_base(g, l - 1, B.fbeg, in, in_fstride, in_step, pyr, &sstep);
+    const long long sfs = l == 1 ? in_fstride : g.pyr_frame_bytes;
+    uint8_t* lvl = pyr + (long long)B.fbeg * g.pyr_frame_bytes + L.off;
+    const int xa16 = sx_lo & ~15;
+    const uintptr_t algn = reinterpret_cast<uintptr_t>(src) | (uintptr_t)sstep | (B.fend - B.fbeg > 1 ? (uintptr_t)sfs : 0);
+    if ((algn & 15) == 0 && sx_hi - xa16 < PYR_SW) {
+        PyrTile T{};
+        T.sy_lo = sy_lo, T.xa = xa16, T.sstep = __builtin_amdgcn_readfirstlane(sstep);
+        T.nc = ((sx_hi - xa16) >> 4) + 1;
+        T.items = (sy_hi - sy_lo + 1) * T.nc;
+        T.mul = __builtin_amdgcn_readfirstlane((int)c_pyr_recip.m[T.nc]);
+        const PyrPieces P = pyr_pieces(T, tid);
+        PyrPix v;
+        pyr_pieces_load(P, src, v);
+        __syncthreads();
+        const PyrTilePrep O = pyr_tile_prep(L, xs_t, tx0, ty0, tw, xa16);
+        for (int f = B.fbeg;;) {
+            pyr_pieces_stage(P, S, v);
+            __syncthreads();
+            const int df = pyr_keep_s(f - B.fbeg);
+            const bool more = ++f < B.fend;
+            if (more) pyr_pieces_load(P, src + (df + 1) * sfs, v);
+            pyr_tile_rows(L, lvl + df * g.pyr_frame_bytes, S, xs_t, ys_t, O, O.C, tx0, tw, th, xa16);
+            if (!more) break;
+            __syncthreads();
+        }
+        return;
+    }
+    const int xa = sx_lo & ~3;
+    const int nd = (sx_hi - xa + 4) >> 2;
+    const int nr = sy_hi - sy_lo + 1;
+    for (int f = B.fbeg; f < B.fend; f++, src += sfs, lvl += g.pyr_frame_bytes) {
+        if (f > B.fbeg) __syncthreads();
+        if (((reinterpret_cast<uintptr_t>(src) | (uintptr_t)sstep) & 3) == 0) {
+            constexpr int RPW = PYR_SH / 4;
+            const int wv = __builtin_amdgcn_readfirstlane((int)(threadIdx.x >> 6));
+            const int ln = threadIdx.x & 63;
+            const int col = min(xa + 4 * ln, (sw - 1) & ~3);
+            const uint8_t* rbase = src + (long long)sy_lo * sstep + col;
+            uint32_t v[RPW];
+#pragma unroll
+            for (int k = 0; k < RPW; k++) {
+                const int rk = min(wv + 4 * k, nr - 1);
+                v[k] = *reinterpret_cast<const uint32_t*>(rbase + (long long)rk * sstep);
+            }
+            if (ln < nd) {
+                uint32_t* drow = reinterpret_cast<uint32_t*>(S) + wv * (PYR_SW / 4) + ln;
+#pragma unroll
+                for (int k = 0; k < RPW; k++)
+                    if (wv + 4 * k < nr) drow[k * PYR_SW] = v[k];
+            }
+        } else {
+            for (int i = threadIdx.x; i < nd * nr; i += blockDim.x) {
+                const int r = i / nd, d = i - r * nd;
+                const uint8_t* rowp = src + (long long)(sy_lo + r) * sstep;
+                const int x = xa + 4 * d;
+                uint32_t v = 0;
+                for (int q = 0; q < 4; q++)
+                    if (x + q < sw) v |= (uint32_t)rowp[x + q] << (8 * q);
+                *reinterpret_cast<uint32_t*>(&S[r * PYR_SW + 4 * d]) = v;
+            }
+        }
+        __syncthreads();
+        const PyrTilePrep O = pyr_tile_prep(L, xs_t, tx0, ty0, tw, xa);
+        pyr_tile_rows(L, lvl, S, xs_t, ys_t, O, O.C, tx0, tw, th, xa);
+    }
+}
+
 template <int NP>
-__global__ __launch_bounds__(256) void pyramid_pair_kernel(Geom g, int l, const uint8_t* __restrict__ in,
+__global__ __launch_bounds__(256) __attribute__((amdgpu_waves_per_eu(7))) void pyramid_pair_kernel(Geom g, int l, const uint8_t* __restrict__ in,
                                                            long long in_fstride, int in_step, uint8_t* pyr,
                                                            const int2* __restrict__ xtab,
-                                                           const int2* __restrict__ ytab) {
+                                                           const int2* __restrict__ ytab, int F, int K) {
     __shared__ __attribute__((aligned(16))) uint8_t S[PYR_SH * PYR_SW + 16];
     __shared__ int2 xs1[PP_MAXC], xs2[PYR_TW];
     __shared__ int4 ys1[PP_MAXR], ys2[PYR_TH];
     const LevelDev& L1 = g.lv[l];
     const LevelDev& L2 = g.lv[l + 1];
     const int tid = threadIdx.x;
-    const int gx = gridDim.x, gxy = gridDim.x * gridDim.y;
-    const int lb = xcd_swizzle(blockIdx.x + gx * blockIdx.y + gxy * blockIdx.z, gxy * gridDim.z);
-    const int f = lb / gxy;
-    const int tx0 = (lb % gx) * PYR_TW, ty0 = ((lb % gxy) / gx) * PYR_TH;
+    const PyrBlock B = pyr_block(F, K);
+    const int tx0 = B.tx0, ty0 = B.ty0;
     const int tw = min(PYR_TW, L2.w - tx0), th = min(PYR_TH, L2.h - ty0);
     auto u = [](int x) { return __builtin_amdgcn_readfirstlane(x); };
     const PyrPairRect R = pyr_pair_rect(xtab + L1.xtab_off, ytab + L1.ytab_off, xtab + L2.xtab_off,
                                         ytab + L2.ytab_off, tx0, ty0, tw, th);
     const int c0 = u(R.c0), c1 = u(R.c1), ay0 = u(R.ay0), ay1 = u(R.ay1);
     const int ncol = c1 - c0 + 1, nrow = ay1 - ay0 + 1;
-    PyrTile T;
+    const uint8_t* src;
+    PyrTile T{};
     T.sy_lo = u(R.by0);
     T.xa = u(R.xa);
     T.nc = u(((R.bx1 - R.xa) >> 4) + 1);
     T.items = u((R.by1 - R.by0 + 1) * T.nc);
     T.mul = u((int)c_pyr_recip.m[T.nc]);
-    T.src = level_base(g, l - 1, f, in, in_fstride, in_step, pyr, &T.sstep);
-    {
-        uint4 v0, v1, v2, v3, v4;
-        pyr_fetch(T, tid, v0, v1, v2, v3, v4);
-        if (tid < ncol) xs1[tid] = xtab[L1.xtab_off + c0 + tid];
-        if (tid < nrow) ys1[tid] = pyr_row_taps(ytab[L1.ytab_off + ay0 + tid], T.sy_lo);
-        if (tid < tw) xs2[tid] = xtab[L2.xtab_off + tx0 + tid];
-        if (tid < th) ys2[tid] = pyr_row_taps(ytab[L2.ytab_off + ty0 + tid], ay0);
-        pyr_stage(T, tid, S, v0, 0);
-        pyr_stage(T, tid, S, v1, 1);
-        pyr_stage(T, tid, S, v2, 2);
-        pyr_stage(T, tid, S, v3, 3);
-        pyr_stage(T, tid, S, v4, 4);
-    }
+    src = level_base(g, l - 1, B.fbeg, in, in_fstride, in_step, pyr, &T.sstep);
+    const long long sfs = l == 1 ? in_fstride : g.pyr_frame_bytes;
+    uint8_t* slab0 = pyr + (long long)B.fbeg * g.pyr_frame_bytes;
+    const PyrPieces P = pyr_pieces(T, tid);
+    PyrPix v;
+    pyr_pieces_load(P, src, v);
+    if (tid < ncol) xs1[tid] = xtab[L1.xtab_off + c0 + tid];
+    if (tid < nrow) ys1[tid] = pyr_row_taps(ytab[L1.ytab_off + ay0 + tid], T.sy_lo);
+    if (tid < tw) xs2[tid] = xtab[L2.xtab_off + tx0 + tid];
+    if (tid < th) ys2[tid] = pyr_row_taps(ytab[L2.ytab_off + ty0 + tid], ay0);
     __syncthreads();
     const int ncq = (ncol + 3) >> 2;
     const unsigned m20 = (unsigned)u((int)c_pyr_recip.m[ncq]);
-    const int rpp = (int)(m20 >> 12);
-    const int r0 = (int)(__umul24((unsigned)tid, m20) >> 20), q = tid - __mul24(r0, ncq);
-    const bool act = r0 < rpp;
-    uint32_t out[NP];
-    if (act) {
-        uint32_t sel0[2], sel1[2], wdv[2];
-        us2 a0[2], a1[2];
-        int2 xv[4];
-        bool fits = true;
-#pragma unroll
-        for (int k = 0; k < 4; k++) xv[k] = xs1[min(4 * q + k, ncol - 1)];
-#pragma unroll
-        for (int j = 0; j < 2; j++) {
-            const int2 xv0 = xv[2 * j], xv1 = xv[2 * j + 1];
-            const int s00 = (xv0.x & 0xffff) - T.xa, s01 = (xv0.x >> 16) - T.xa;
-            const int s10 = (xv1.x & 0xffff) - T.xa, s11 = (xv1.x >> 16) - T.xa;
-            const int wd = s00 >> 2;
-            const int e00 = s00 - 4 * wd, e01 = s01 - 4 * wd, e10 = s10 - 4 * wd, e11 = s11 - 4 * wd;
-            fits = fits && max(e01, e11) <= 7 && min(e00, e10) >= 0;
-            sel0[j] = (uint32_t)e00 | 0x0c00u | ((uint32_t)e01 << 16) | 0x0c000000u;
-            sel1[j] = (uint32_t)e10 | 0x0c00u | ((uint32_t)e11 << 16) | 0x0c000000u;
-            wdv[j] = (uint32_t)wd;
-            a0[j] = *reinterpret_cast<const us2*>(&xv0.y);
-            a1[j] = *reinterpret_cast<const us2*>(&xv1.y);
-        }
-        const int tcol = L1.tail_x - (c0 + 4 * q);
-        auto rows = [&](auto tail_c) {
-            constexpr bool TAIL = decltype(tail_c)::value;
+    const int rppw = (int)(m20 >> 12);
+    const int r0w = (int)(__umul24((unsigned)tid, m20) >> 20), q = tid - __mul24(r0w, ncq);
+    const bool act = r0w < rppw;
+    PyrCols C1;
+    const bool fits1 = pyr_cols(xs1, 4 * q, ncol, T.xa, C1);
+    const int c4qw = c0 + 4 * q;
+    const bool tail1 = c1 >= L1.tail_x;
+    const PyrTilePrep O2 = pyr_tile_prep(L2, xs2, tx0, ty0, tw, c0);
+    for (int f = B.fbeg;;) {
+        pyr_pieces_stage(P, S, v);
+        __syncthreads();
+        const int df = pyr_keep_s(f - B.fbeg);
+        uint8_t* slab = slab0 + df * g.pyr_frame_bytes;
+        const int r0 = pyr_keep_v(r0w), rpp = pyr_keep_s(rppw), c4q = pyr_keep_v(c4qw);
+        const int tcol1 = L1.tail_x - c4q, rem1 = c1 - c4q;
+        const int soff1 = r0 * PYR_SW + (c4q - c0);
+        const uint32_t doff1 = (uint32_t)(c4q + (ay0 + r0) * L1.stride);
+        uint32_t out[NP];
+        if (act) {
+            auto rows = [&](auto tail_c) {
+                constexpr bool TAIL = decltype(tail_c)::value;
+#pragma unroll
+                for (int pp = 0; pp < NP; pp++) {
+                    const int r = r0 + pp * rpp;
+                    out[pp] = 0;
+                    if (pp * rpp >= nrow) break;
+                    if ((pp + 1) * rpp > nrow && r >= nrow) break;
+                    const int4 yv = ys1[r];
+                    if (fits1) {
+                        out[pp] = pyr_row4<TAIL>(S, yv, C1, tcol1);
+                    } else {
+                        const int qg = pyr_keep_v(q), tg = pyr_keep_v(tcol1);
+#pragma unroll
+                        for (int k = 0; k < 4; k++)
+                            out[pp] |= pyr_px_generic(S, xs1[min(4 * qg + k, ncol - 1)], yv, T.xa, k >= tg) << (8 * k);
+                    }
+                }
+            };
+            if (tail1) rows(std::true_type{});
+            else
+                rows(std::false_type{});
+        }
+        __syncthreads();
+        if (act) {
+            uint8_t* lvl1 = slab + L1.off;
+            const uint32_t dstep = (uint32_t)(rpp * L1.stride);
 #pragma unroll
             for (int pp = 0; pp < NP; pp++) {
+                uint8_t* lrow = lvl1 + (doff1 + (uint32_t)pp * dstep);
                 const int r = r0 + pp * rpp;
-                out[pp] = 0;
                 if (pp * rpp >= nrow) break;
                 if ((pp + 1) * rpp > nrow && r >= nrow) break;
-                const int4 yv = ys1[r];
-                if (fits) {
-                    const uint32_t b0 = (uint32_t)yv.z, b1 = (uint32_t)yv.w;
-#pragma unroll
-                    for (int j = 0; j < 2; j++) {
-                        const uint32_t* s0 = reinterpret_cast<const uint32_t*>(S + yv.x + 4 * (int)wdv[j]);
-                        const uint32_t* s1 = reinterpret_cast<const uint32_t*>(S + yv.y + 4 * (int)wdv[j]);
-                        const uint32_t w00 = s0[0], w01 = s0[1], w10 = s1[0], w11 = s1[1];
-                        const uint32_t r0a = __builtin_amdgcn_udot2(pyr_tap(w01, w00, sel0[j]), a0[j], 0u, false);
-                        const uint32_t r1a = __builtin_amdgcn_udot2(pyr_tap(w11, w10, sel0[j]), a0[j], 0u, false);
-                        const uint32_t r0b = __builtin_amdgcn_udot2(pyr_tap(w01, w00, sel1[j]), a1[j], 0u, false);
-                        const uint32_t r1b = __builtin_amdgcn_udot2(pyr_tap(w11, w10, sel1[j]), a1[j], 0u, false);
-                        uint32_t va = (mulhi24(htap24(r0a), b0) + mulhi24(htap24(r1a), b1) + 2) >> 2;
-                        uint32_t vb = (mulhi24(htap24(r0b), b0) + mulhi24(htap24(r1b), b1) + 2) >> 2;
-                        if (TAIL) {
-                            va = 2 * j >= tcol ? vtail(r0a, r1a, b0, b1) : va;
-                            vb = 2 * j + 1 >= tcol ? vtail(r0b, r1b, b0, b1) : vb;
-                        }
-                        out[pp] |= (va | (vb << 8)) << (16 * j);
-                    }
+                *reinterpret_cast<uint32_t*>(&S[soff1 + pp * rpp * PYR_SW]) = out[pp];
+                if (rem1 >= 3) {
+                    *reinterpret_cast<uint32_t*>(lrow) = out[pp];
                 } else {
-#pragma unroll
-                    for (int k = 0; k < 4; k++) out[pp] |= pyr_px_generic(S, xv[k], yv, T.xa, k >= tcol) << (8 * k);
+                    for (int k = 0; k < 3; k++)
+                        if (k <= rem1) lrow[k] = (uint8_t)(out[pp] >> (8 * k));
                 }
             }
-        };
-        if (c1 >= L1.tail_x) rows(std::true_type{});
-        else
-            rows(std::false_type{});
-    }
-    __syncthreads();
-    if (act) {
-        uint8_t* lrow = pyr + (long long)f * g.pyr_frame_bytes + L1.off + c0 + 4 * q;
-        const bool full = c0 + 4 * q + 3 <= c1;
-#pragma unroll
-        for (int pp = 0; pp < NP; pp++) {
-            const int r = r0 + pp * rpp;
-            if (pp * rpp >= nrow) break;
-            if ((pp + 1) * rpp > nrow && r >= nrow) break;
-            *reinterpret_cast<uint32_t*>(&S[r * PYR_SW + 4 * q]) = out[pp];
-            uint8_t* dst = lrow + __mul24(ay0 + r, L1.stride);
-            if (full) {
-                *reinterpret_cast<uint32_t*>(dst) = out[pp];
-            } else {
-                for (int k = 0; k < 3; k++)
-                    if (c0 + 4 * q + k <= c1) dst[k] = (uint8_t)(out[pp] >> (8 * k));
-            }
-        }
-    }
-    __syncthreads();
-    pyr_tile_compute(g, L2, f, pyr, S, xs2, ys2, tx0, ty0, tw, th, c0);
+        }
+        __syncthreads();
+        const bool more = ++f < B.fend;
+        PyrCols C2;
+        const int tidf = pyr_keep_v(tid);
+        pyr_cols(xs2, (tidf & 15) * 4, tw, c0, C2);
+        PyrTilePrep O2f;
+        O2f.fits = O2.fits, O2f.tail = O2.tail;
+        pyr_tile_lane(L2, tx0, ty0, tw, tidf, O2f);
+        pyr_tile_rows(L2, slab + L2.off, S, xs2, ys2, O2f, C2, tx0, tw, th, c0);
+        if (!more) break;
+        pyr_pieces_load(P, src + (df + 1) * sfs, v);
+        __syncthreads();
+    }
 }
 
 static int pyr_pair_fits(const Geom& g, int l, const std::vector<int2>& xtab, const std::vector<int2>& ytab) {
```

After: 178,400 frames/s (median of 6 runs). About the same (+0.8%).
